# NickTravers/NeuralNetworkLibrary

Hardware: AMD Instinct MI355X
Metric: ResNet-34 224x224 training throughput (Learner.train1minibatch, fwd+loss+bwd+optimizer) (higher is better)
Workload: dtype f32; 1 GPU; DogsCats ResNet-34 classifier, 224x224, bs=64 per GPU, SGD momentum 0.9, fp32; global_batch=64, image_size=224, parallelism=dp1

## Files before the change

include/nnl.h:

```cpp
#ifndef NNL_H_
#define NNL_H_

#include <stddef.h>
#include <stdint.h>

#ifdef __cplusplus
extern "C" {
#endif

typedef enum {
  NNL_OK = 0,
  NNL_ERR_INVALID_ARG = -1,
  NNL_ERR_HIP = -2,
  NNL_ERR_UNSUPPORTED = -3,
  NNL_ERR_WORKSPACE = -4
} nnl_status_t;

int nnl_version(void);
const char* nnl_last_error(void);
int nnl_reload_env(void);

enum { NNL_PROF_CONV_FWD = 0, NNL_PROF_CONV_DGRAD = 1, NNL_PROF_CONV_WGRAD = 2, NNL_PROF_EMBDOT = 3,
       NNL_PROF_TABULAR = 4, NNL_PROF_RETINA_LOSS = 5, NNL_PROF_LSTM = 6, NNL_PROF_SOFTMAX_CE = 7,
       NNL_PROF_ELEMENTWISE = 8, NNL_PROF_GEMM = 9, NNL_PROF_OPTIM = 10, NNL_PROF_KINDS = 11 };
int nnl_prof_enable(int enable);
int nnl_prof_collect(int64_t* launches, double* total_ms, double* total_work);
int nnl_prof_collect2(int64_t* launches, double* total_ms, double* total_work, double* total_exec);
int nnl_dp_bump(int32_t* step, void* stream);
int nnl_dp_signal(int32_t* flag, const int32_t* step, void* stream);
int nnl_dp_wait(const int32_t* flag, int32_t value, int64_t timeout_us, int32_t* err, void* stream);
const char* nnl_source_stamp(void);

int nnl_embdotbias_fwd(const int64_t* x, const float* U, const float* M, const float* bu, const float* bi,
                       float* y, float* z, int64_t n, int64_t n_user, int64_t n_item, int64_t D,
                       int has_range, float lo, float hi, int32_t* err_flag, void* stream);
size_t nnl_embdotbias_bwd_workspace_bytes(int64_t n);
int nnl_embdotbias_bwd(const int64_t* x, const float* U, const float* M, const float* z, const float* dy,
                       float* dU, float* dM, float* dbu, float* dbi, int64_t n, int64_t n_user,
                       int64_t n_item, int64_t D, int has_range, float lo, float hi, void* workspace, size_t workspace_bytes, void* stream);

typedef struct {
  int32_t N, H, W, C;
  int32_t K, R, S;
  int32_t stride, pad;
  int32_t P, Q;
} nnl_conv_geom_t;

size_t nnl_conv2d_fwd_workspace_bytes(const nnl_conv_geom_t* g);
int64_t nnl_conv2d_tile_counters(void);
int nnl_conv2d_fwd(const float* x, const float* w, const float* bias, float* y, const nnl_conv_geom_t* g,
                   int relu, void* workspace, size_t workspace_bytes, int32_t* tile_counters, float* bn_partials,
                   const float* bn_pivot, int32_t* bn_rows, void* stream);
int nnl_conv2d_fwd_add_up2(const float* x, const float* w, const float* bias, const float* small, float* y,
                           const nnl_conv_geom_t* g, void* stream);
int nnl_upsample2_bwd(const float* dy, float* dsmall, int64_t N, int64_t h, int64_t w, int64_t C, void* stream);
int nnl_conv2d_weight_transpose(const float* w, float* wt, int K, int R, int S, int C, void* stream);
typedef struct {
  const float* w;
  float* wt;
  int32_t K, RS, C, first_tile;
} nnl_wt_desc_t;
int nnl_conv2d_weight_transpose_multi(const nnl_wt_desc_t* desc, const int32_t* tile_tensor, int64_t n_tiles,
                                      double total_elems, void* stream);
size_t nnl_conv2d_dgrad_workspace_bytes(const nnl_conv_geom_t* g);
int nnl_conv2d_dgrad(const float* dy, const float* wt, float* dx, const nnl_conv_geom_t* g, const float* addend,
                     void* workspace, size_t workspace_bytes, int32_t* tile_counters, void* stream);
typedef struct {
  const float* src;
  float* dst;
  int32_t rows, ch, flip, first_block;
  int32_t two_d, reserved;
} nnl_wino_desc_t;
int nnl_conv2d_wino_preferred(const nnl_conv_geom_t* g, int dgrad);
int nnl_wino_filter_multi(const nnl_wino_desc_t* desc, const int32_t* block_desc, int64_t n_blocks, void* stream);
int nnl_conv2d_fwd_pre(const float* x, const float* w, const float* bias, float* y, const nnl_conv_geom_t* g, int relu,
                       void* workspace, size_t workspace_bytes, int32_t* tile_counters, float* bn_partials, const float* bn_pivot,
                       int32_t* bn_rows, const float* u, void* stream);
int nnl_conv2d_dgrad_pre(const float* dy, const float* wt, float* dx, const nnl_conv_geom_t* g, const float* addend,
                         void* workspace, size_t workspace_bytes, int32_t* tile_counters, const float* u, void* stream);
size_t nnl_debug_conv_wino_workspace_bytes(int N, int H, int W, int C, int K);
int nnl_debug_conv_wino_fwd(const float* x, const float* filt, const float* bias, const float* add, float* y, void* ws,
                            size_t ws_bytes, int32_t* counters, long n_counters, float* bn_part, const float* bn_pivot, int N,
                            int H, int W, int C, int K, int relu, int flip, void* stream);
size_t nnl_debug_conv_wino2_workspace_bytes(int N, int H, int W, int C, int K);
int nnl_debug_conv_wino2_fwd(const float* x, const float* filt, const float* bias, const float* add, float* y, void* ws,
                            size_t ws_bytes, int32_t* counters, long n_counters, float* bn_part, const float* bn_pivot, int N,
                            int H, int W, int C, int K, int relu, int flip, void* stream);
int nnl_debug_conv_plan_times(int N, int H, int W, int C, int K, double* out);

int nnl_debug_route_record(int enable);
int nnl_debug_route_collect(char* out, size_t n);
size_t nnl_conv2d_wgrad_workspace_bytes(const nnl_conv_geom_t* g);
int nnl_conv2d_wgrad(const float* x, const float* dy, float* dw, const nnl_conv_geom_t* g, void* workspace,
                     size_t workspace_bytes, void* stream);
size_t nnl_colsum_workspace_bytes(int64_t rows, int64_t cols);
int nnl_sum_tensors(const float* const* src, int n, float* out, int64_t numel, void* stream);
int nnl_colsum(const float* a, float* out, int64_t rows, int64_t cols, void* workspace, size_t workspace_bytes,
               void* stream);
int nnl_relu_gate_colsum(const float* dy, const float* y, float* g, float* colsum, int64_t rows, int64_t cols, void* workspace,
                         size_t workspace_bytes, void* stream);
int nnl_act_gate_colsum(const float* dy, const float* y, float* g, float* colsum, int64_t rows, int64_t cols, int act,
                        void* workspace, size_t workspace_bytes, void* stream);

size_t nnl_bn_workspace_bytes(int64_t rows, int64_t C);
int nnl_bn_fwd(const float* x, const float* gamma, const float* beta, const float* residual, float* y,
               float* save_mean, float* save_invstd, float* running_mean, float* running_var, int64_t rows,
               int64_t C, float eps, float momentum, int training, int relu, int64_t* num_batches_tracked,
               uint32_t* relu_mask, const float* ext_partials, int64_t ext_rows, const float* ext_pivot, float* pivot_out,
               void* workspace, size_t workspace_bytes, void* stream);
int nnl_bn_bwd(const float* dy, const float* y, const uint32_t* relu_mask, const float* x, const float* gamma,
               const float* mean, const float* invstd, float* dx, float* dres, float* dgamma, float* dbeta, int64_t rows,
               int64_t C, int training, int relu, void* workspace, size_t workspace_bytes, void* stream);

int nnl_bn_relu_maxpool_supported(int64_t C);
int nnl_bn_relu_maxpool_fwd(const float* x, const float* gamma, const float* beta, float* y, uint8_t* idx, float* save_mean,
                            float* save_invstd, float* save_scale, float* save_shift, float* running_mean, float* running_var,
                            int64_t N, int64_t H, int64_t W, int64_t C, int64_t P, int64_t Q, int ks, int stride, int pad, float eps,
                            float momentum, int training, int64_t* num_batches_tracked, void* workspace, size_t workspace_bytes,
                            void* stream);
int nnl_bn_relu_maxpool_bwd(const float* dpool, const float* y, const uint8_t* idx, const float* x, const float* gamma,
                            const float* beta, const float* mean, const float* invstd, const float* scale, const float* shift,
                            float* dx, float* dgamma, float* dbeta,
                            int64_t N, int64_t H, int64_t W, int64_t C, int64_t P, int64_t Q, int ks, int stride, int pad,
                            int training, void* workspace, size_t workspace_bytes, void* stream);

int nnl_debug_bn_plan(int64_t rows, int64_t C, int64_t N, int64_t H, int64_t W, int64_t P, int64_t Q, int32_t* out10);

int nnl_bn_sync_stats(const float* x, float* stats, int64_t rows, int64_t C, void* workspace, size_t workspace_bytes,
                      void* stream);
int nnl_bn_sync_fwd(const float* x, const float* all_stats, int world, const float* gamma, const float* beta,
                    const float* residual, float* y, float* save_mean, float* save_invstd, float* running_mean,
                    float* running_var, int64_t rows, int64_t C, float eps, float momentum, int relu,
                    int64_t* num_batches_tracked, uint32_t* relu_mask, void* workspace, size_t workspace_bytes, void* stream);
int nnl_bn_sync_bwd_reduce(const float* dy, const float* y, const uint32_t* relu_mask, const float* x, const float* mean,
                           const float* invstd, float* sums, int64_t rows, int64_t C, int relu, void* workspace,
                           size_t workspace_bytes, void* stream);
int nnl_bn_sync_bwd(const float* dy, const float* y, const uint32_t* relu_mask, const float* x, const float* gamma,
                    const float* mean, const float* invstd, const float* local_sums, const float* global_sums,
                    const float* all_stats,
                    int world, float* dx, float* dres, float* dgamma, float* dbeta, int64_t rows, int64_t C, int relu,
                    void* workspace, size_t workspace_bytes, void* stream);

int nnl_maxpool2d_fwd(const float* x, float* y, uint8_t* idx, int64_t N, int64_t H, int64_t W, int64_t C, int64_t P,
                      int64_t Q, int ksize, int stride, int pad, void* stream);
int nnl_maxpool2d_bwd(const float* dy, const uint8_t* idx, float* dx, int64_t N, int64_t H, int64_t W, int64_t C,
                      int64_t P, int64_t Q, int ksize, int stride, int pad, void* stream);
int nnl_concat_pool_fwd(const float* x, float* out, int32_t* argmax, int64_t N, int64_t HW, int64_t C, void* stream);
int nnl_concat_pool_bwd(const float* dout, const int32_t* argmax, float* dx, int64_t N, int64_t HW, int64_t C, void* stream);

int nnl_gconv2d_fwd(const float* x, const float* w, const float* bias, float* y, int64_t N, int64_t H, int64_t W, int64_t C, int64_t K,
                    int64_t G, int R, int stride, int pad, int relu, void* stream);
int nnl_gconv2d_dgrad(const float* dy, const float* w, float* dx, int64_t N, int64_t H, int64_t W, int64_t C, int64_t K, int64_t G,
                      int R, int stride, int pad, void* stream);
size_t nnl_gconv2d_workspace_bytes(int64_t N, int64_t H, int64_t W, int64_t C, int64_t K, int64_t G, int R, int stride, int pad);
int nnl_gconv2d_wgrad(const float* x, const float* dy, float* dw, void* ws, size_t ws_bytes, int64_t N, int64_t H, int64_t W, int64_t C,
                      int64_t K, int64_t G, int R, int stride, int pad, void* stream);

int nnl_dwconv2d_fwd(const float* x, const float* w, const float* bias, float* y, int64_t N, int64_t H, int64_t W, int64_t C, int64_t P,
                     int64_t Q, int R, int stride, int pad_lo, int relu_in, void* stream);
int nnl_dwconv2d_dgrad(const float* dy, const float* w, const float* x, float* dx, int64_t N, int64_t H, int64_t W, int64_t C, int64_t P,
                       int64_t Q, int R, int stride, int pad_lo, int relu_in, void* stream);
size_t nnl_dwconv2d_wgrad_workspace_bytes(int64_t N, int64_t H, int64_t W, int64_t C, int64_t P, int64_t Q, int R, int stride, int pad_lo);
int nnl_dwconv2d_wgrad(const float* x, const float* dy, float* dw, void* ws, size_t ws_bytes, int64_t N, int64_t H, int64_t W, int64_t C,
                       int64_t P, int64_t Q, int R, int stride, int pad_lo, int relu_in, void* stream);

int nnl_avgpool2d_fwd(const float* x, float* y, int64_t N, int64_t H, int64_t W, int64_t C, int64_t P, int64_t Q, int ksize, int stride,
                      int pad_lo, int count_include_pad, void* stream);
int nnl_avgpool2d_bwd(const float* dy, float* dx, int64_t N, int64_t H, int64_t W, int64_t C, int64_t P, int64_t Q, int ksize, int stride,
                      int pad_lo, int count_include_pad, void* stream);
int nnl_subsample2d_fwd(const float* x, float* y, int64_t N, int64_t H, int64_t W, int64_t C, int64_t P, int64_t Q, int stride, int off,
                        void* stream);
int nnl_subsample2d_bwd(const float* dy, float* dx, int64_t N, int64_t H, int64_t W, int64_t C, int64_t P, int64_t Q, int stride, int off,
                        void* stream);

int nnl_se_squeeze(const float* x, float* m, int64_t N, int64_t HW, int64_t C, void* stream);
int nnl_se_excite_fwd(const float* x, const float* z, const float* residual, float* out, int64_t N, int64_t HW, int64_t C, void* stream);
int nnl_se_excite_bwd(const float* dy, const float* out, const float* x, const float* z, float* dx, float* dres, float* dz, int64_t N,
                      int64_t HW, int64_t C, void* stream);
int nnl_se_squeeze_bwd(const float* dm, float* dx, int64_t N, int64_t HW, int64_t C, void* stream);

int nnl_bbox_decode(const float* anchors, const float* reg, const float* clas, int64_t bs, int64_t A, int64_t K,
                    const float* mean4, const float* std4, float thresh, float width, float height, float* cand_boxes,
                    int32_t* cand_classes, float* cand_scores, int32_t* cand_order, int32_t* cand_count, void* stream);
int nnl_bbox_decode_window(const float* anchors, const float* reg, const float* clas, int64_t bs, int64_t A, int64_t K,
                           const float* mean4, const float* std4, float thresh, float x_min, float y_min, float x_max, float y_max,
                           float* cand_boxes, int32_t* cand_classes, float* cand_scores, int32_t* cand_order, int32_t* cand_count,
                           void* stream);
size_t nnl_nms_workspace_bytes(int64_t bs, int64_t top_k);
int nnl_nms(const float* cand_boxes, const int32_t* cand_classes, const float* cand_scores, const int32_t* cand_order,
            const int32_t* cand_count, int64_t bs, int64_t cap, int64_t top_k, float max_overlap, float* kept_boxes,
            int32_t* kept_classes, float* kept_scores, int32_t* kept_count, void* workspace, size_t workspace_bytes,
            void* stream);

typedef struct {
  float col_jit, row_jit;
  float inv;
  float cols;
  int32_t flip;
} nnl_tta_undo_t;
int nnl_tta_bbox_merge(const float* boxes, const int32_t* classes, const float* scores, const int32_t* counts,
                       const nnl_tta_undo_t* undo, int64_t L, int64_t P, int64_t M, float* cand_boxes, int32_t* cand_classes,
                       float* cand_scores, int32_t* cand_order, int32_t* cand_count, int32_t* err_flag, void* stream);

int nnl_tab_renorm(const int64_t* xcat, float* const* tables, const int32_t* card, const int32_t* dim,
                   const int32_t* row_off, const int32_t* row_table, int32_t* flags, int64_t bs, int32_t ncat,
                   int32_t total_rows, float max_norm, int32_t* err_flag, void* stream);
int nnl_tab_gather_fwd(const int64_t* xcat, const float* const* tables, const int32_t* card, const int32_t* dim,
                       const int32_t* col_off, const int32_t* col_table, const float* row_mask, const float* cont,
                       const float* cont_mask, float* out, int64_t bs, int32_t ncat, int32_t cat_width,
                       int32_t n_cont, int32_t ld_out, void* stream);
size_t nnl_tab_scatter_bwd_workspace_bytes(int64_t bs, int32_t ncat);
int nnl_tab_scatter_bwd(const int64_t* xcat, const int32_t* card, const int32_t* dim, const int32_t* col_off,
                        const int32_t* col_table, const int64_t* grad_off, const float* row_mask,
                        const float* cont_mask, const float* dout, float* dtab_flat, int64_t dtab_elems,
                        float* dcont, int64_t bs, int32_t ncat, int32_t cat_width, int32_t n_cont, int32_t ld_out,
                        void* workspace, size_t workspace_bytes, void* stream);
int nnl_tab_scan_bwd(const int64_t* xcat, const int32_t* card, const int32_t* dim, const int32_t* col_off,
                     const int64_t* grad_off, const float* row_mask, const float* cont_mask, const float* dout,
                     float* dtab_flat, float* dcont, const int32_t* blk_col, const int32_t* blk_first, int32_t n_scan_blocks,
                     int32_t max_dim, int64_t bs, int32_t ncat, int32_t cat_width, int32_t n_cont, int32_t ld_out, void* stream);

int nnl_pad_cols(const float* src, float* dst, int64_t rows, int64_t C, int64_t Cp, void* stream);
int nnl_keep_masks(const float* u, float* a, int64_t na, float keep_a, float* b, int64_t nb, float keep_b, void* stream);

int nnl_linear_small_supported(int64_t N);
int nnl_linear_small_fwd(const float* x, const float* w, const float* bias, float* y, int64_t M, int64_t K, int64_t ldx, int64_t N,
                         void* stream);
size_t nnl_linear_small_bwd_workspace_bytes(int64_t M, int64_t K, int64_t N);
int nnl_linear_small_bwd(const float* dy, const float* x, const float* w, float* dx, float* dw, float* db, int64_t M, int64_t K,
                         int64_t ldx, int64_t N, void* workspace, size_t workspace_bytes, void* stream);

size_t nnl_retina_loss_workspace_bytes(int64_t bs, int64_t A);
int nnl_retina_loss_fwd(const float* anchors, const float* reg, const float* clas, const float* boxes,
                        const int64_t* cats, int32_t* state, float* npos, float* out, int64_t bs, int64_t A,
                        int64_t K, int64_t M, float beta, float alpha, float gamma, void* workspace,
                        size_t workspace_bytes, void* stream);
int nnl_retina_loss_bwd(const float* anchors, const float* reg, const float* clas, const float* boxes,
                        const int64_t* cats, const int32_t* state, const float* npos, const float* grad_out,
                        float* dreg, float* dclas, int64_t bs, int64_t A, int64_t K, int64_t M, float beta,
                        float alpha, float gamma, void* stream);

int64_t nnl_lstm_padded_hidden(int64_t H);
int64_t nnl_lstm_padded_gates(int64_t H);
size_t nnl_lstm_workspace_bytes(int64_t T, int64_t B, int64_t H);
int nnl_lstm_fwd(const float* gx, const float* w_hh_pad, const float* h0, const float* c0, float* y, float* cy,
                 float* gates, int64_t T, int64_t B, int64_t H, void* workspace, size_t workspace_bytes, int32_t* err_flag,
                 void* stream);
int nnl_lstm_bwd(const float* dy, const float* dhT, const float* dcT, const float* gates, const float* cy,
                 const float* c0, const float* w_hh_t_pad, float* dgates_pad, float* dh0, float* dc0, int64_t T, int64_t B,
                 int64_t H, void* workspace, size_t workspace_bytes, int32_t* err_flag, void* stream);
int nnl_debug_lstm_bptt2_plan(int64_t B, int64_t H, int32_t* out5);
int nnl_debug_lstm_plan(int64_t B, int64_t H, int32_t* out14);

size_t nnl_mse_workspace_bytes(int64_t n);
int nnl_mse_fwd(const float* pred, const float* target, float* loss, int64_t n, void* workspace, size_t workspace_bytes, void* stream);
int nnl_mse_bwd(const float* pred, const float* target, const float* grad_out, float* dpred, int64_t n, void* stream);
size_t nnl_bce_logits_workspace_bytes(int64_t n);
int nnl_bce_logits_fwd(const float* logits, const float* target, float* loss, int64_t n, void* workspace, size_t workspace_bytes, void* stream);
int nnl_bce_logits_bwd(const float* logits, const float* target, const float* grad_out, float* dlogits, int64_t n, void* stream);
size_t nnl_fbeta_workspace_bytes(int64_t N, int64_t C);
int nnl_fbeta(const float* pred, const float* target, float* out, int64_t N, int64_t C, float beta2, float threshold, int use_thresh, float eps,
              void* workspace, size_t workspace_bytes, void* stream);
int nnl_scaled_sigmoid_fwd(const float* x, float* y, float* sig, int64_t n, float lo, float hi, void* stream);
int nnl_scaled_sigmoid_bwd(const float* dy, const float* sig, float* dx, int64_t n, float lo, float hi, void* stream);

int nnl_embedding_rowmask_fwd(const int64_t* x, const float* W, const float* rowmask, float* out, int64_t n,
                              int64_t V, int64_t D, int32_t* err_flag, void* stream);
size_t nnl_embedding_rowmask_bwd_workspace_bytes(int64_t n);
int nnl_embedding_rowmask_bwd(const int64_t* x, const float* rowmask, const float* dout, float* dW, int64_t n,
                              int64_t V, int64_t D, int64_t padding_idx, void* workspace, size_t workspace_bytes, void* stream);
int nnl_softmax_ce_fwd(const float* logits, const int64_t* target, float* row_stats, float* loss_rows, float* loss_mean,
                       int64_t rows, int64_t V, int32_t* err_flag, void* stream);
// ... 149 lines not shown
```

neuralnetworklibrary_amd/_lib.py:

```python
import ctypes as C
import os

import torch

_HERE = os.path.dirname(os.path.abspath(__file__))
LIB_PATH = os.environ.get('NNL_LIB_PATH') or os.path.join(_HERE, 'libnnl_hip.so')

if not os.path.exists(LIB_PATH):
    raise ImportError(
        f"{LIB_PATH} not found: build it with `python -c 'import __graft_entry__ as g; g.build()'` "
        "(or `make -C neuralnetworklibrary_amd/csrc`). There is no CPU fallback for the HIP hot path.")

lib = C.CDLL(LIB_PATH)

c_p = C.c_void_p
i32, i64, f32, f64 = C.c_int32, C.c_int64, C.c_float, C.c_double
sz = C.c_size_t


class ConvGeom(C.Structure):
    _fields_ = [('N', i32), ('H', i32), ('W', i32), ('C', i32), ('K', i32), ('R', i32), ('S', i32),
                ('stride', i32), ('pad', i32), ('P', i32), ('Q', i32)]


SIGNATURES = {
    'nnl_version': (C.c_int, []),
    'nnl_last_error': (C.c_char_p, []),
    'nnl_reload_env': (C.c_int, []),
    'nnl_prof_enable': (C.c_int, [C.c_int]),
    'nnl_prof_collect': (C.c_int, [C.POINTER(i64), C.POINTER(f64), C.POINTER(f64)]),
    'nnl_prof_collect2': (C.c_int, [C.POINTER(i64), C.POINTER(f64), C.POINTER(f64), C.POINTER(f64)]),
    'nnl_source_stamp': (C.c_char_p, []),
    'nnl_dp_bump': (C.c_int, [c_p, c_p]),
    'nnl_dp_signal': (C.c_int, [c_p, c_p, c_p]),
    'nnl_dp_wait': (C.c_int, [c_p, i32, i64, c_p, c_p]),
    'nnl_embdotbias_fwd': (C.c_int, [c_p, c_p, c_p, c_p, c_p, c_p, c_p, i64, i64, i64, i64, C.c_int, f32, f32,
                                     c_p, c_p]),
    'nnl_embdotbias_bwd_workspace_bytes': (sz, [i64]),
    'nnl_embdotbias_bwd': (C.c_int, [c_p, c_p, c_p, c_p, c_p, c_p, c_p, c_p, c_p, i64, i64, i64, i64, C.c_int,
                                     f32, f32, c_p, sz, c_p]),
    'nnl_conv2d_fwd_workspace_bytes': (sz, [C.POINTER(ConvGeom)]),
    'nnl_conv2d_dgrad_workspace_bytes': (sz, [C.POINTER(ConvGeom)]),
    'nnl_conv2d_tile_counters': (i64, []),
    'nnl_conv2d_wino_preferred': (C.c_int, [C.POINTER(ConvGeom), C.c_int]),
    'nnl_wino_filter_multi': (C.c_int, [c_p, c_p, i64, c_p]),
    'nnl_conv2d_fwd_pre': (C.c_int, [c_p, c_p, c_p, c_p, C.POINTER(ConvGeom), C.c_int, c_p, sz, c_p, c_p, c_p, C.POINTER(i32), c_p, c_p]),
    'nnl_conv2d_dgrad_pre': (C.c_int, [c_p, c_p, c_p, C.POINTER(ConvGeom), c_p, c_p, sz, c_p, c_p, c_p]),
    'nnl_debug_conv_wino_workspace_bytes': (sz, [C.c_int] * 5),
    'nnl_debug_conv_wino_fwd': (C.c_int, [c_p] * 6 + [sz, c_p, C.c_long, c_p, c_p] + [C.c_int] * 7 + [c_p]),
    'nnl_debug_conv_wino2_workspace_bytes': (sz, [C.c_int] * 5),
    'nnl_debug_conv_wino2_fwd': (C.c_int, [c_p] * 6 + [sz, c_p, C.c_long, c_p, c_p] + [C.c_int] * 7 + [c_p]),
    'nnl_debug_conv_plan_times': (C.c_int, [C.c_int] * 5 + [C.POINTER(C.c_double)]),
    'nnl_debug_route_record': (C.c_int, [C.c_int]),
    'nnl_debug_route_collect': (C.c_int, [C.c_char_p, sz]),
    'nnl_conv2d_fwd': (C.c_int, [c_p, c_p, c_p, c_p, C.POINTER(ConvGeom), C.c_int, c_p, sz, c_p, c_p, c_p, C.POINTER(i32), c_p]),
    'nnl_conv2d_weight_transpose': (C.c_int, [c_p, c_p, C.c_int, C.c_int, C.c_int, C.c_int, c_p]),
    'nnl_conv2d_weight_transpose_multi': (C.c_int, [c_p, c_p, i64, f64, c_p]),
    'nnl_conv2d_dgrad': (C.c_int, [c_p, c_p, c_p, C.POINTER(ConvGeom), c_p, c_p, sz, c_p, c_p]),
    'nnl_conv2d_wgrad_workspace_bytes': (sz, [C.POINTER(ConvGeom)]),
    'nnl_conv2d_wgrad': (C.c_int, [c_p, c_p, c_p, C.POINTER(ConvGeom), c_p, sz, c_p]),
    'nnl_colsum_workspace_bytes': (sz, [i64, i64]),
    'nnl_colsum': (C.c_int, [c_p, c_p, i64, i64, c_p, sz, c_p]),
    'nnl_relu_gate_colsum': (C.c_int, [c_p, c_p, c_p, c_p, i64, i64, c_p, sz, c_p]),
    'nnl_conv2d_fwd_add_up2': (C.c_int, [c_p, c_p, c_p, c_p, c_p, C.POINTER(ConvGeom), c_p]),
    'nnl_upsample2_bwd': (C.c_int, [c_p, c_p, i64, i64, i64, i64, c_p]),
    'nnl_act_gate_colsum': (C.c_int, [c_p, c_p, c_p, c_p, i64, i64, C.c_int, c_p, sz, c_p]),
    'nnl_maxpool2d_fwd': (C.c_int, [c_p, c_p, c_p, i64, i64, i64, i64, i64, i64, C.c_int, C.c_int, C.c_int, c_p]),
    'nnl_maxpool2d_bwd': (C.c_int, [c_p, c_p, c_p, i64, i64, i64, i64, i64, i64, C.c_int, C.c_int, C.c_int, c_p]),
    'nnl_sum_tensors': (C.c_int, [c_p, C.c_int, c_p, i64, c_p]),
    'nnl_bn_relu_maxpool_supported': (C.c_int, [i64]),
    'nnl_bn_relu_maxpool_fwd': (C.c_int, [c_p, c_p, c_p, c_p, c_p, c_p, c_p, c_p, c_p, c_p, c_p, i64, i64, i64, i64, i64, i64,
                                          C.c_int, C.c_int, C.c_int, f32, f32, C.c_int, c_p, c_p, sz, c_p]),
    'nnl_bn_relu_maxpool_bwd': (C.c_int, [c_p, c_p, c_p, c_p, c_p, c_p, c_p, c_p, c_p, c_p, c_p, c_p, c_p, i64, i64, i64, i64, i64, i64,
                                          C.c_int, C.c_int, C.c_int, C.c_int, c_p, sz, c_p]),
    'nnl_concat_pool_fwd': (C.c_int, [c_p, c_p, c_p, i64, i64, i64, c_p]),
    'nnl_concat_pool_bwd': (C.c_int, [c_p, c_p, c_p, i64, i64, i64, c_p]),
    'nnl_gconv2d_fwd': (C.c_int, [c_p, c_p, c_p, c_p, i64, i64, i64, i64, i64, i64, C.c_int, C.c_int, C.c_int, C.c_int, c_p]),
    'nnl_gconv2d_dgrad': (C.c_int, [c_p, c_p, c_p, i64, i64, i64, i64, i64, i64, C.c_int, C.c_int, C.c_int, c_p]),
    'nnl_gconv2d_workspace_bytes': (sz, [i64, i64, i64, i64, i64, i64, C.c_int, C.c_int, C.c_int]),
    'nnl_gconv2d_wgrad': (C.c_int, [c_p, c_p, c_p, c_p, sz, i64, i64, i64, i64, i64, i64, C.c_int, C.c_int, C.c_int, c_p]),
    'nnl_dwconv2d_fwd': (C.c_int, [c_p, c_p, c_p, c_p, i64, i64, i64, i64, i64, i64, C.c_int, C.c_int, C.c_int, C.c_int, c_p]),
    'nnl_dwconv2d_dgrad': (C.c_int, [c_p, c_p, c_p, c_p, i64, i64, i64, i64, i64, i64, C.c_int, C.c_int, C.c_int, C.c_int, c_p]),
    'nnl_dwconv2d_wgrad_workspace_bytes': (sz, [i64, i64, i64, i64, i64, i64, C.c_int, C.c_int, C.c_int]),
    'nnl_dwconv2d_wgrad': (C.c_int, [c_p, c_p, c_p, c_p, sz, i64, i64, i64, i64, i64, i64, C.c_int, C.c_int, C.c_int, C.c_int, c_p]),
    'nnl_avgpool2d_fwd': (C.c_int, [c_p, c_p, i64, i64, i64, i64, i64, i64, C.c_int, C.c_int, C.c_int, C.c_int, c_p]),
    'nnl_avgpool2d_bwd': (C.c_int, [c_p, c_p, i64, i64, i64, i64, i64, i64, C.c_int, C.c_int, C.c_int, C.c_int, c_p]),
    'nnl_subsample2d_fwd': (C.c_int, [c_p, c_p, i64, i64, i64, i64, i64, i64, C.c_int, C.c_int, c_p]),
    'nnl_subsample2d_bwd': (C.c_int, [c_p, c_p, i64, i64, i64, i64, i64, i64, C.c_int, C.c_int, c_p]),
    'nnl_se_squeeze': (C.c_int, [c_p, c_p, i64, i64, i64, c_p]),
    'nnl_se_excite_fwd': (C.c_int, [c_p, c_p, c_p, c_p, i64, i64, i64, c_p]),
    'nnl_se_excite_bwd': (C.c_int, [c_p, c_p, c_p, c_p, c_p, c_p, c_p, i64, i64, i64, c_p]),
    'nnl_se_squeeze_bwd': (C.c_int, [c_p, c_p, i64, i64, i64, c_p]),
    'nnl_bbox_decode': (C.c_int, [c_p, c_p, c_p, i64, i64, i64, c_p, c_p, f32, f32, f32, c_p, c_p, c_p, c_p, c_p, c_p]),
    'nnl_bbox_decode_window': (C.c_int, [c_p, c_p, c_p, i64, i64, i64, c_p, c_p, f32, f32, f32, f32, f32, c_p, c_p, c_p, c_p, c_p, c_p]),
    'nnl_nms_workspace_bytes': (sz, [i64, i64]),
    'nnl_nms': (C.c_int, [c_p, c_p, c_p, c_p, c_p, i64, i64, i64, f32, c_p, c_p, c_p, c_p, c_p, sz, c_p]),
    'nnl_tta_bbox_merge': (C.c_int, [c_p, c_p, c_p, c_p, c_p, i64, i64, i64, c_p, c_p, c_p, c_p, c_p, c_p, c_p]),
    'nnl_tab_renorm': (C.c_int, [c_p, c_p, c_p, c_p, c_p, c_p, c_p, i64, i32, i32, f32, c_p, c_p]),
    'nnl_tab_gather_fwd': (C.c_int, [c_p, c_p, c_p, c_p, c_p, c_p, c_p, c_p, c_p, c_p, i64, i32, i32, i32, i32, c_p]),
    'nnl_tab_scatter_bwd_workspace_bytes': (sz, [i64, i32]),
    'nnl_tab_scatter_bwd': (C.c_int, [c_p, c_p, c_p, c_p, c_p, c_p, c_p, c_p, c_p, c_p, i64, c_p, i64, i32, i32, i32, i32, c_p, sz, c_p]),
    'nnl_tab_scan_bwd': (C.c_int, [c_p] * 12 + [i32, i32, i64, i32, i32, i32, i32, c_p]),
    'nnl_pad_cols': (C.c_int, [c_p, c_p, i64, i64, i64, c_p]),
    'nnl_keep_masks': (C.c_int, [c_p, c_p, i64, f32, c_p, i64, f32, c_p]),
    'nnl_linear_small_supported': (C.c_int, [i64]),
    'nnl_linear_small_fwd': (C.c_int, [c_p, c_p, c_p, c_p, i64, i64, i64, i64, c_p]),
    'nnl_linear_small_bwd_workspace_bytes': (sz, [i64, i64, i64]),
    'nnl_linear_small_bwd': (C.c_int, [c_p, c_p, c_p, c_p, c_p, c_p, i64, i64, i64, i64, c_p, sz, c_p]),
    'nnl_retina_loss_workspace_bytes': (sz, [i64, i64]),
    'nnl_retina_loss_fwd': (C.c_int, [c_p, c_p, c_p, c_p, c_p, c_p, c_p, c_p, i64, i64, i64, i64, f32, f32, f32, c_p, sz, c_p]),
    'nnl_retina_loss_bwd': (C.c_int, [c_p, c_p, c_p, c_p, c_p, c_p, c_p, c_p, c_p, c_p, i64, i64, i64, i64, f32, f32, f32, c_p]),
    'nnl_lstm_padded_hidden': (i64, [i64]),
    'nnl_lstm_padded_gates': (i64, [i64]),
    'nnl_lstm_workspace_bytes': (sz, [i64, i64, i64]),
    'nnl_lstm_fwd': (C.c_int, [c_p, c_p, c_p, c_p, c_p, c_p, c_p, i64, i64, i64, c_p, sz, c_p, c_p]),
    'nnl_lstm_bwd': (C.c_int, [c_p, c_p, c_p, c_p, c_p, c_p, c_p, c_p, c_p, c_p, i64, i64, i64, c_p, sz, c_p, c_p]),
    'nnl_debug_lstm_bptt2_plan': (C.c_int, [i64, i64, c_p]),
    'nnl_debug_lstm_plan': (C.c_int, [i64, i64, C.POINTER(i32)]),
    'nnl_embedding_rowmask_fwd': (C.c_int, [c_p, c_p, c_p, c_p, i64, i64, i64, c_p, c_p]),
    'nnl_embedding_rowmask_bwd_workspace_bytes': (sz, [i64]),
    'nnl_embedding_rowmask_bwd': (C.c_int, [c_p, c_p, c_p, c_p, i64, i64, i64, i64, c_p, sz, c_p]),
    'nnl_softmax_ce_fwd': (C.c_int, [c_p, c_p, c_p, c_p, c_p, i64, i64, c_p, c_p]),
    'nnl_softmax_ce_bwd': (C.c_int, [c_p, c_p, c_p, c_p, c_p, i64, i64, i64, c_p]),
    'nnl_mse_workspace_bytes': (sz, [i64]),
    'nnl_mse_fwd': (C.c_int, [c_p, c_p, c_p, i64, c_p, sz, c_p]),
    'nnl_mse_bwd': (C.c_int, [c_p, c_p, c_p, c_p, i64, c_p]),
    'nnl_bce_logits_workspace_bytes': (sz, [i64]),
    'nnl_bce_logits_fwd': (C.c_int, [c_p, c_p, c_p, i64, c_p, sz, c_p]),
    'nnl_bce_logits_bwd': (C.c_int, [c_p, c_p, c_p, c_p, i64, c_p]),
    'nnl_fbeta_workspace_bytes': (sz, [i64, i64]),
    'nnl_fbeta': (C.c_int, [c_p, c_p, c_p, i64, i64, C.c_float, C.c_float, C.c_int, C.c_float, c_p, sz, c_p]),
    'nnl_scaled_sigmoid_fwd': (C.c_int, [c_p, c_p, c_p, i64, C.c_float, C.c_float, c_p]),
    'nnl_scaled_sigmoid_bwd': (C.c_int, [c_p, c_p, c_p, i64, C.c_float, C.c_float, c_p]),
    'nnl_seq_reg_workspace_bytes': (sz, [i64, i64]),
    'nnl_seq_reg_fwd': (C.c_int, [c_p, c_p, i64, i64, C.c_float, C.c_float, c_p, sz, c_p]),
    'nnl_seq_reg_bwd': (C.c_int, [c_p, c_p, c_p, i64, i64, C.c_float, C.c_float, c_p]),
    'nnl_weight_drop': (C.c_int, [c_p, i64, c_p, c_p, i64, i64, i64, C.c_uint64, C.c_float, c_p]),
    'nnl_lstm_cell_b1': (C.c_int, [c_p, i64, c_p, i64, c_p, c_p, c_p, i64, c_p, i64, i64, c_p, c_p, c_p, c_p, i64, i64, c_p]),
    'nnl_lm_next_token_workspace_bytes': (sz, [i64, i64]),
    'nnl_lm_next_token': (C.c_int, [c_p, i64, c_p, i64, i64, i64, i64, c_p, i64, c_p, i64, c_p, c_p, c_p, c_p, sz, c_p]),
    'nnl_attn_pool_workspace_bytes': (sz, [i64, i64, i64, i64]),
    'nnl_attn_pool_fwd': (C.c_int, [c_p, c_p, c_p, c_p, c_p, i64, c_p, c_p, i64, i64, i64, i64, c_p, sz, c_p, i64, c_p]),
    'nnl_attn_pool_bwd': (C.c_int, [c_p, c_p, c_p, c_p, c_p, c_p, c_p, c_p, c_p, c_p, i64, i64, i64, i64, c_p, sz, c_p, i64, c_p]),
    'nnl_image_aug_workspace_bytes': (sz, [i64, i64, i64]),
    'nnl_image_aug': (C.c_int, [c_p, i64, c_p, i64, c_p, i64, i64, i64, C.POINTER(f32), C.c_int, c_p, c_p, sz, c_p]),
    'nnl_detect_aug': (C.c_int, [c_p, i64, c_p, i64, c_p, c_p, c_p, i64, c_p, i64, i64, i64, i64, i64, i64, f64, C.POINTER(f32),
                                 c_p, c_p, c_p, c_p]),
    'nnl_image_stats': (C.c_int, [c_p, i64, c_p, i64, i64, i64, c_p, c_p]),
    'nnl_image_resize_u8': (C.c_int, [c_p, i64, c_p, c_p, i64, c_p, i64, c_p]),
    'nnl_optim_chunk_elems': (i64, []),
    'nnl_optim_patch': (C.c_int, [c_p, c_p, c_p, i64, c_p]),
    'nnl_optim_step': (C.c_int, [c_p, c_p, c_p, i64, C.c_int, c_p, C.c_int, c_p, c_p]),
    'nnl_bn_workspace_bytes': (sz, [i64, i64]),
    'nnl_bn_fwd': (C.c_int, [c_p, c_p, c_p, c_p, c_p, c_p, c_p, c_p, c_p, i64, i64, f32, f32, C.c_int, C.c_int, c_p, c_p, c_p, i64,
                             c_p, c_p, c_p, sz, c_p]),
    'nnl_debug_bn_plan': (C.c_int, [i64] * 7 + [C.POINTER(i32)]),
    'nnl_bn_sync_stats': (C.c_int, [c_p, c_p, i64, i64, c_p, sz, c_p]),
    'nnl_bn_sync_fwd': (C.c_int, [c_p, c_p, C.c_int, c_p, c_p, c_p, c_p, c_p, c_p, c_p, c_p, i64, i64, f32, f32, C.c_int, c_p,
                                  c_p, c_p, sz, c_p]),
    'nnl_bn_sync_bwd_reduce': (C.c_int, [c_p, c_p, c_p, c_p, c_p, c_p, c_p, i64, i64, C.c_int, c_p, sz, c_p]),
    'nnl_bn_sync_bwd': (C.c_int, [c_p, c_p, c_p, c_p, c_p, c_p, c_p, c_p, c_p, c_p, C.c_int, c_p, c_p, c_p, c_p, i64, i64,
                                  C.c_int, c_p, sz, c_p]),
    'nnl_bn_bwd': (C.c_int, [c_p, c_p, c_p, c_p, c_p, c_p, c_p, c_p, c_p, c_p, c_p, i64, i64, C.c_int, C.c_int, c_p, sz, c_p]),
    'nnl_seg_event_gaps': (C.c_int, [c_p, c_p, c_p, i64, f64, c_p, c_p, c_p, c_p, c_p]),
    'nnl_seg_rolling': (C.c_int, [c_p, c_p, c_p, c_p, i64, i64, i64, i64, C.c_int, C.c_int, c_p, c_p]),
    'nnl_assoc_contingency': (C.c_int, [c_p, c_p, i64, i64, c_p, c_p, c_p, i64, c_p, c_p]),
    'nnl_assoc_table_stats': (C.c_int, [c_p, c_p, i64, c_p, c_p, c_p, i64, c_p, c_p]),
    'nnl_assoc_cat_cont_workspace_bytes': (sz, [c_p, i64, c_p, i64]),
    'nnl_assoc_cat_cont': (C.c_int, [c_p, c_p, i64, c_p, c_p, i64, i64, c_p, c_p, i64, c_p, sz, c_p, c_p]),
    'nnl_assoc_cont_cont_workspace_bytes': (sz, [i64, i64]),
    'nnl_assoc_cont_cont': (C.c_int, [c_p, c_p, i64, i64, c_p, c_p, i64, C.c_int, c_p, sz, c_p, c_p]),
    'nnl_det_coco_match': (C.c_int, [c_p] * 7 + [i64, i64, i64, c_p, i64, c_p, i64, c_p, sz, c_p, c_p, c_p, c_p, c_p]),
    'nnl_det_coco_accumulate': (C.c_int, [c_p] * 8 + [i64, i64, i64, i64, i64, c_p, i64, c_p, i64, c_p, c_p, c_p, c_p]),
    'nnl_det_map_match': (C.c_int, [c_p, c_p, c_p, c_p, i64, i64, i64, c_p, i64, c_p, c_p]),
    'nnl_det_map_integrate_workspace_bytes': (sz, [i64, i64]),
    'nnl_det_map_integrate': (C.c_int, [c_p, c_p, c_p, c_p, c_p, i64, i64, i64, c_p, sz, c_p, c_p]),
    'nnl_text_token_count': (C.c_int, [c_p, i64, c_p, i64, C.c_int, c_p, c_p]),
    'nnl_text_token_fill': (C.c_int, [c_p, i64, c_p, i64, C.c_int, c_p, i64, c_p, c_p, c_p, c_p]),
    'nnl_text_token_hash': (C.c_int, [c_p, i64, c_p, c_p, i64, C.c_int, C.c_uint64, C.c_uint64, c_p, c_p]),
    'nnl_text_vocab_insert': (C.c_int, [c_p, i64, c_p, c_p, c_p, i64, C.c_int, c_p, c_p, c_p]),
    'nnl_text_vocab_verify': (C.c_int, [c_p, i64, c_p, c_p, c_p, i64, C.c_int, c_p, i64, c_p, c_p, i64, C.c_int, c_p, i64, c_p, c_p]),
    'nnl_text_vocab_compact': (C.c_int, [c_p, c_p, c_p, i64, c_p, c_p, i64, c_p, i64, c_p, c_p]),
    'nnl_text_vocab_assign': (C.c_int, [c_p, c_p, i64, c_p, i64, c_p]),
    'nnl_text_vocab_lookup': (C.c_int, [c_p, i64, c_p, c_p, c_p, i64, C.c_int, c_p, i64, c_p, c_p, i64, c_p, c_p, i64, c_p, c_p]),
    'nnl_text_ids_write': (C.c_int, [c_p, c_p, i64, c_p, i64, i64, C.c_int, c_p, c_p]),
}

for _name, (_res, _args) in SIGNATURES.items():
    try:
        _fn = getattr(lib, _name)
    except AttributeError as e:
        raise ImportError(f"libnnl_hip.so does not export {_name}; rebuild it") from e
    _fn.restype = _res
    _fn.argtypes = _args

PROF_KINDS = ['conv_fwd', 'conv_dgrad', 'conv_wgrad', 'embdot', 'tabular', 'retina_loss', 'lstm',
              'softmax_ce', 'elementwise', 'gemm', 'optim']


class NnlError(RuntimeError):
    pass


def check(status):
    if status != 0:
        raise NnlError(f"nnl error {status}: {lib.nnl_last_error().decode()}")


def ptr(t):
    return None if t is None else C.c_void_p(t.data_ptr())


def stream():
    return C.c_void_p(torch.cuda.current_stream().cuda_stream)


def require_cuda(*tensors):
    for t in tensors:
        if t is not None and not t.is_cuda:
            raise NnlError("nnl HIP op called with a non-CUDA tensor: the MI355X path has no CPU fallback")


def prof_enable(flag=True):
    check(lib.nnl_prof_enable(1 if flag else 0))

# ... 23 lines not shown
```

neuralnetworklibrary_amd/csrc/batchnorm.hip:

```cpp
#include "nnl_common.h"

namespace {

typedef float f32x4 __attribute__((ext_vector_type(4)));

template <int VEC> struct VecT;
template <> struct VecT<4> { typedef f32x4 type; };
template <> struct VecT<1> { typedef float type; };

template <int VEC> __device__ __forceinline__ float vget(const typename VecT<VEC>::type& v, int i);
template <> __device__ __forceinline__ float vget<4>(const f32x4& v, int i) { return v[i]; }
template <> __device__ __forceinline__ float vget<1>(const float& v, int i) { return v; }
template <int VEC> __device__ __forceinline__ void vset(typename VecT<VEC>::type& v, int i, float x);
template <> __device__ __forceinline__ void vset<4>(f32x4& v, int i, float x) { v[i] = x; }
template <> __device__ __forceinline__ void vset<1>(float& v, int i, float x) { v = x; }

constexpr int kBlock = 256;
constexpr int kMaxRowBlocks = 1024;
constexpr float kCentreAbove = 16.f;
constexpr int kFinLanes = 64;

struct Shape {
  int L;
  int rpb;
// ... 661 lines not shown
      const uchar4 id = reinterpret_cast<const uchar4*>(idx)[o];
      const f32x4 d = reinterpret_cast<const f32x4*>(dpool)[o];
      if (id.x == t) acc[0] += d[0];
      if (id.y == t) acc[1] += d[1];
      if (id.z == t) acc[2] += d[2];
      if (id.w == t) acc[3] += d[3];
    }
  }
  const f32x4 z = bnpool_affine(xv, sc, sh);
#pragma unroll
  for (int e = 0; e < 4; ++e) if (!(z[e] > 0.f)) acc[e] = 0.f;
  return acc;
}

constexpr int kPoolRedBlock = 1024;

__device__ __forceinline__ void store_pool_block_partials(const float (&s1)[4], const float (&s2)[4], float* __restrict__ part, int C,
                                                          int C4) {
  __shared__ float red[kPoolRedBlock][8];
#pragma unroll
  for (int e = 0; e < 4; ++e) { red[threadIdx.x][e * 2] = s1[e]; red[threadIdx.x][e * 2 + 1] = s2[e]; }
  __syncthreads();
  if ((int)threadIdx.x < C4) {
#pragma unroll
    for (int e = 0; e < 4; ++e) {
      float a = 0.f, b = 0.f;
      for (int j = threadIdx.x; j < kPoolRedBlock; j += C4) { a += red[j][e * 2]; b += red[j][e * 2 + 1]; }
      const long c = (long)threadIdx.x * 4 + e;
      part[((long)blockIdx.x * C + c) * 2 + 0] = a;
      part[((long)blockIdx.x * C + c) * 2 + 1] = b;
    }
  }
}

__global__ __launch_bounds__(kPoolRedBlock) void bnpool_bwd_reduce_kernel(const float* __restrict__ dpool, const uint8_t* __restrict__ idx,
                                                                   const float* __restrict__ x, const float* __restrict__ scale,
                                                                   const float* __restrict__ shift, const float* __restrict__ mean,
                                                                   const float* __restrict__ invstd, float* __restrict__ part,
                                                                   int N, int C, PoolGeom g) {
  const long total = (long)N * g.H * g.W * g.C4;
  const long i0 = (long)blockIdx.x * blockDim.x + threadIdx.x;
  const int c4 = (int)(i0 % g.C4);
  const f32x4 sc = reinterpret_cast<const f32x4*>(scale)[c4], sh = reinterpret_cast<const f32x4*>(shift)[c4];
  const f32x4 mu = reinterpret_cast<const f32x4*>(mean)[c4], is = reinterpret_cast<const f32x4*>(invstd)[c4];
  float s1[4] = {0.f, 0.f, 0.f, 0.f}, s2[4] = {0.f, 0.f, 0.f, 0.f};
  for (long i = i0; i < total; i += (long)gridDim.x * blockDim.x) {
    long r = i / g.C4;
    const int w = (int)(r % g.W); r /= g.W;
    const int h = (int)(r % g.H);
    const int n = (int)(r / g.H);
    const f32x4 xv = reinterpret_cast<const f32x4*>(x)[i];
    const f32x4 gg = bnpool_grad(dpool, idx, xv, sc, sh, n, h, w, c4, g);
#pragma unroll
    for (int e = 0; e < 4; ++e) { s1[e] += gg[e]; s2[e] += gg[e] * ((xv[e] - mu[e]) * is[e]); }
  }
  store_pool_block_partials(s1, s2, part, C, g.C4);
}

__global__ __launch_bounds__(kPoolRedBlock) void bnpool_bwd_reduce_out_kernel(const float* __restrict__ dpool, const float* __restrict__ y,
                                                                       const uint8_t* __restrict__ idx, const float* __restrict__ x,
                                                                       const float* __restrict__ gamma, const float* __restrict__ beta,
                                                                       const float* __restrict__ mean, const float* __restrict__ invstd,
                                                                       float* __restrict__ part, int N, int C, PoolGeom g) {
  const long total = (long)N * g.P * g.Q * g.C4;
  const long i0 = (long)blockIdx.x * blockDim.x + threadIdx.x;
  const int c4 = (int)(i0 % g.C4);
  float bt[4], rg[4], mu[4], is[4];
  bool fast[4];
#pragma unroll
  for (int e = 0; e < 4; ++e) {
    const int c = c4 * 4 + e;
    const float gm = gamma ? gamma[c] : 1.f;
    bt[e] = beta ? beta[c] : 0.f;
    fast[e] = fabsf(gm) > 1e-2f;
    rg[e] = fast[e] ? 1.f / gm : 0.f;
    mu[e] = mean[c]; is[e] = invstd[c];
  }
  float s1[4] = {0.f, 0.f, 0.f, 0.f}, s2[4] = {0.f, 0.f, 0.f, 0.f};
  for (long i = i0; i < total; i += (long)gridDim.x * blockDim.x) {
    const f32x4 d = reinterpret_cast<const f32x4*>(dpool)[i];
    const f32x4 yv = reinterpret_cast<const f32x4*>(y)[i];
    const uchar4 id = reinterpret_cast<const uchar4*>(idx)[i];
    const unsigned char t[4] = {id.x, id.y, id.z, id.w};
#pragma unroll
    for (int e = 0; e < 4; ++e) {
      if (!(yv[e] > 0.f)) continue;
      float xh;
      if (fast[e]) {
        xh = (yv[e] - bt[e]) * rg[e];
      } else {
        long r = i / g.C4;
        const int q = (int)(r % g.Q); r /= g.Q;
        const int p = (int)(r % g.P);
        const int n = (int)(r / g.P);
        const int h = p * g.stride - g.pad + t[e] / g.ks, w = q * g.stride - g.pad + t[e] % g.ks;
        xh = (x[((long)(n * g.H + h) * g.W + w) * C + c4 * 4 + e] - mu[e]) * is[e];
      }
      s1[e] += d[e];
      s2[e] += d[e] * xh;
    }
  }
  store_pool_block_partials(s1, s2, part, C, g.C4);
}

__global__ __launch_bounds__(kBlock) void bnpool_bwd_apply_kernel(const float* __restrict__ dpool, const uint8_t* __restrict__ idx,
                                                                  const float* __restrict__ x, const float* __restrict__ scale,
                                                                  const float* __restrict__ shift, const float* __restrict__ coef,
                                                                  float* __restrict__ dx, int N, int C, PoolGeom g) {
  const long total = (long)N * g.H * g.W * g.C4;
  const long i0 = (long)blockIdx.x * blockDim.x + threadIdx.x;
  const int c4 = (int)(i0 % g.C4);
  const f32x4 sc = reinterpret_cast<const f32x4*>(scale)[c4], sh = reinterpret_cast<const f32x4*>(shift)[c4];
  const f32x4 ca = reinterpret_cast<const f32x4*>(coef)[c4], cb = *reinterpret_cast<const f32x4*>(coef + C + c4 * 4),
              cc = *reinterpret_cast<const f32x4*>(coef + 2 * C + c4 * 4);
  for (long i = i0; i < total; i += (long)gridDim.x * blockDim.x) {
    long r = i / g.C4;
    const int w = (int)(r % g.W); r /= g.W;
    const int h = (int)(r % g.H);
    const int n = (int)(r / g.H);
    const f32x4 xv = reinterpret_cast<const f32x4*>(x)[i];
    const f32x4 gg = bnpool_grad(dpool, idx, xv, sc, sh, n, h, w, c4, g);
    f32x4 out;
#pragma unroll
    for (int e = 0; e < 4; ++e) out[e] = ca[e] * gg[e] + cb[e] * xv[e] + cc[e];
    reinterpret_cast<f32x4*>(dx)[i] = out;
  }
}

bool bnpool_ok(long C) { return C % 4 == 0 && C >= 4 && C <= 1024 && (kBlock % (C / 4)) == 0; }
unsigned bnpool_grid(long total) {
  long g = nnl_cdiv(total, (long)kPoolRedBlock * 4);
  if (g > kMaxRowBlocks) g = kMaxRowBlocks;
  return (unsigned)(g < 1 ? 1 : g);
}

int check_stem_geometry(const char* who, long N, long H, long W, long C, long P, long Q, int ks, int stride, int pad) {
  NNL_CHECK_ARG(N > 0 && H > 0 && W > 0 && P > 0 && Q > 0 && ks > 0 && ks * ks <= 255 && stride > 0 && pad >= 0 && 2 * pad <= ks,
                "%s: bad geometry", who);
  NNL_CHECK_ARG(P == (H + 2 * pad - ks) / stride + 1 && Q == (W + 2 * pad - ks) / stride + 1, "%s: P/Q do not match", who);
  NNL_CHECK_ARG(bnpool_ok(C), "%s: C=%ld needs C %% 4 == 0 and C/4 dividing 256", who, C);
  NNL_CHECK_ARG(N * H * W * C < (1L << 31) * 4, "%s: tensor too large", who);
  return NNL_OK;
}

}

extern "C" int nnl_bn_relu_maxpool_supported(int64_t C) { return bnpool_ok(C) ? 1 : 0; }

extern "C" int nnl_bn_relu_maxpool_fwd(const float* x, const float* gamma, const float* beta, float* y, uint8_t* idx,
                                       float* save_mean, float* save_invstd, float* save_scale, float* save_shift,
                                       float* running_mean, float* running_var, int64_t N, int64_t H, int64_t W, int64_t C,
                                       int64_t P, int64_t Q, int ks, int stride, int pad, float eps, float momentum, int training,
                                       int64_t* num_batches_tracked, void* workspace, size_t workspace_bytes, void* stream) {
  NNL_TRY(check_stem_geometry("bn_relu_maxpool_fwd", N, H, W, C, P, Q, ks, stride, pad));
  NNL_CHECK_ARG(x && y && idx && save_mean && save_invstd && save_scale && save_shift, "bn_relu_maxpool_fwd: null pointer");
  NNL_CHECK_ARG(training || (running_mean && running_var), "bn_relu_maxpool_fwd: eval mode needs running statistics");
  const long rows = (long)N * H * W, CG = C / 4;
  Workspace ws;
  NNL_TRY(bind_workspace(workspace, workspace_bytes, rows, C, "bn_relu_maxpool_fwd", ws));
  hipStream_t s = (hipStream_t)stream;
  NnlProfScope prof(NNL_PROF_ELEMENTWISE, s, (double)rows * C * (training ? 8.0 : 4.0) + (double)N * P * Q * C * 5.0);
  const ChannelStats cs{gamma, beta, save_mean, save_invstd, running_mean, running_var, save_scale, save_shift,  nullptr,
                         nullptr, num_batches_tracked, eps, momentum};
  NNL_TRY(launch_channel_affine(x, ws.part, cs, rows, C, training, s));
  const long total = (long)N * P * Q * CG;
  hipLaunchKernelGGL(bnpool_fwd_kernel, dim3((unsigned)nnl_cdiv(total, kBlock)), dim3(kBlock), 0, s, x, save_scale, save_shift, y, idx,
                     (int)N, (int)H, (int)W, (int)CG, (int)P, (int)Q, ks, stride, pad);
  NNL_CHECK_LAUNCH();
  return NNL_OK;
}

extern "C" int nnl_bn_relu_maxpool_bwd(const float* dpool, const float* y, const uint8_t* idx, const float* x, const float* gamma,
                                       const float* beta, const float* mean, const float* invstd, const float* scale,
                                       const float* shift, float* dx, float* dgamma, float* dbeta, int64_t N,
                                       int64_t H, int64_t W, int64_t C, int64_t P, int64_t Q, int ks, int stride, int pad,
                                       int training, void* workspace, size_t workspace_bytes, void* stream) {
  NNL_TRY(check_stem_geometry("bn_relu_maxpool_bwd", N, H, W, C, P, Q, ks, stride, pad));
  NNL_CHECK_ARG(dpool && idx && x && mean && invstd && scale && shift && dx, "bn_relu_maxpool_bwd: null pointer");
  const long rows = (long)N * H * W;
  Workspace ws;
  NNL_TRY(bind_workspace(workspace, workspace_bytes, rows, C, "bn_relu_maxpool_bwd", ws));
  hipStream_t s = (hipStream_t)stream;
  const PoolGeom g{(int)H, (int)W, (int)(C / 4), (int)P, (int)Q, ks, stride, pad};
  const long total = rows * (C / 4);
  NnlProfScope prof(NNL_PROF_ELEMENTWISE, s, (double)rows * C * 12.0 + (double)N * P * Q * C * 10.0);
  unsigned grid;
  if (y != nullptr) {
    grid = bnpool_grid((long)N * P * Q * (C / 4));
    hipLaunchKernelGGL(bnpool_bwd_reduce_out_kernel, dim3(grid), dim3(kPoolRedBlock), 0, s, dpool, y, idx, x, gamma, beta, mean, invstd,
                       ws.part, (int)N, (int)C, g);
  } else {
    grid = bnpool_grid(total);
    hipLaunchKernelGGL(bnpool_bwd_reduce_kernel, dim3(grid), dim3(kPoolRedBlock), 0, s, dpool, idx, x, scale, shift, mean, invstd, ws.part,
                       (int)N, (int)C, g);
  }
  NNL_CHECK_LAUNCH();
  NNL_TRY(launch_bwd_finalize(ws.part, (int)grid, gamma, mean, invstd, dgamma, dbeta, ws.coef, rows, C, training, s));
  hipLaunchKernelGGL(bnpool_bwd_apply_kernel, dim3((unsigned)nnl_cdiv(total, kBlock)), dim3(kBlock), 0, s, dpool, idx, x, scale, shift,
                     ws.coef, dx, (int)N, (int)C, g);
  NNL_CHECK_LAUNCH();
  return NNL_OK;
}

extern "C" int nnl_bn_sync_stats(const float* x, float* stats, int64_t rows, int64_t C, void* workspace,
                                 size_t workspace_bytes, void* stream) {
  NNL_CHECK_ARG(rows > 0 && C > 0 && C < (1 << 24) && x && stats, "bn_sync_stats: bad arguments");
  Workspace ws;
  NNL_TRY(bind_workspace(workspace, workspace_bytes, rows, C, "bn_sync_stats", ws));
  hipStream_t s = (hipStream_t)stream;
  NnlProfScope prof(NNL_PROF_ELEMENTWISE, s, (double)rows * C * 4.0);
  int nparts;
  NNL_TRY(launch_stats(x, ws.part, rows, C, s, nparts));
  hipLaunchKernelGGL(bn_sync_local_kernel, dim3((unsigned)nnl_cdiv(C, 4)), dim3(256), 0, s, x, (const float*)ws.part, nparts, stats,
                     (long)rows, (int)C);
  NNL_CHECK_LAUNCH();
  return NNL_OK;
}

extern "C" int nnl_bn_sync_fwd(const float* x, const float* all_stats, int world, const float* gamma, const float* beta,
                               const float* residual, float* y, float* save_mean, float* save_invstd, float* running_mean,
                               float* running_var, int64_t rows, int64_t C, float eps, float momentum, int relu,
                               int64_t* num_batches_tracked, uint32_t* relu_mask, void* workspace, size_t workspace_bytes,
                               void* stream) {
  NNL_CHECK_ARG(rows > 0 && C > 0 && C < (1 << 24) && world > 0, "bn_sync_fwd: bad sizes");
  NNL_CHECK_ARG(x && y && all_stats && save_mean && save_invstd, "bn_sync_fwd: null pointer");
  Workspace ws;
  NNL_TRY(bind_workspace(workspace, workspace_bytes, rows, C, "bn_sync_fwd", ws));
  hipStream_t s = (hipStream_t)stream;
  NnlProfScope prof(NNL_PROF_ELEMENTWISE, s, (double)rows * C * 8.0 + (residual ? 4.0 * rows * C : 0.0));
  hipLaunchKernelGGL(bn_sync_merge_kernel, dim3((unsigned)nnl_cdiv(C, 256)), dim3(256), 0, s, all_stats, world, gamma, beta,
                     save_mean, save_invstd, running_mean, running_var, ws.scale, ws.shift, (int)C, eps, momentum,
                     (long long*)num_batches_tracked, ws.apply_pivot);
  NNL_CHECK_LAUNCH();
  return launch_apply(x, ws, residual, y, rows, C, relu, relu_mask, s);
}

extern "C" int nnl_bn_sync_bwd_reduce(const float* dy, const float* y, const uint32_t* relu_mask, const float* x,
                                      const float* mean, const float* invstd, float* sums, int64_t rows, int64_t C, int relu,
                                      void* workspace, size_t workspace_bytes, void* stream) {
  NNL_CHECK_ARG(rows > 0 && C > 0 && C < (1 << 24), "bn_sync_bwd_reduce: bad sizes");
  NNL_CHECK_ARG(dy && x && mean && invstd && sums && (y || relu_mask || !relu), "bn_sync_bwd_reduce: null pointer");
  Workspace ws;
  NNL_TRY(bind_workspace(workspace, workspace_bytes, rows, C, "bn_sync_bwd_reduce", ws));
  hipStream_t s = (hipStream_t)stream;
  NnlProfScope prof(NNL_PROF_ELEMENTWISE, s, (double)rows * C * (relu ? 12.0 : 8.0));
  int nparts;
  NNL_TRY(launch_bwd_reduce(dy, y, relu_mask, x, mean, invstd, ws.part, rows, C, relu, s, nparts));
  hipLaunchKernelGGL(bn_sync_bwd_sums_kernel, dim3((unsigned)nnl_cdiv(C, 4)), dim3(256), 0, s, (const float*)ws.part, nparts, sums, (int)C);
  NNL_CHECK_LAUNCH();
  return NNL_OK;
}

extern "C" int nnl_bn_sync_bwd(const float* dy, const float* y, const uint32_t* relu_mask, const float* x, const float* gamma,
                               const float* mean,
                               const float* invstd, const float* local_sums, const float* global_sums, const float* all_stats,
                               int world, float* dx, float* dres, float* dgamma, float* dbeta, int64_t rows, int64_t C, int relu,
                               void* workspace, size_t workspace_bytes, void* stream) {
  NNL_CHECK_ARG(rows > 0 && C > 0 && C < (1 << 24) && world > 0, "bn_sync_bwd: bad sizes");
  NNL_CHECK_ARG(dy && x && mean && invstd && dx && local_sums && global_sums && all_stats && (y || relu_mask || !relu),
                "bn_sync_bwd: null pointer");
  Workspace ws;
  NNL_TRY(bind_workspace(workspace, workspace_bytes, rows, C, "bn_sync_bwd", ws));
  hipStream_t s = (hipStream_t)stream;
  NnlProfScope prof(NNL_PROF_ELEMENTWISE, s, (double)rows * C * (relu ? 16.0 : 12.0) + (dres ? 4.0 * rows * C : 0.0));
  hipLaunchKernelGGL(bn_sync_bwd_coef_kernel, dim3((unsigned)nnl_cdiv(C, 256)), dim3(256), 0, s, local_sums, global_sums, all_stats,
                     world, gamma, mean, invstd, dgamma, dbeta, ws.coef, (int)C);
  NNL_CHECK_LAUNCH();
  return launch_bwd_apply(dy, y, relu_mask, x, ws.coef, dx, dres, rows, C, relu, s);
}

extern "C" int nnl_debug_bn_plan(int64_t rows, int64_t C, int64_t N, int64_t H, int64_t W, int64_t P, int64_t Q, int32_t* out10) {
  if (rows <= 0 || C <= 0 || C >= (1 << 24) || out10 == nullptr) return 0;
  const int VEC = vec_of(C);
  const long CG = C / VEC;
  const Shape sh = make_shape(rows, CG);
  out10[0] = VEC; out10[1] = sh.L; out10[2] = sh.rpb; out10[3] = sh.gx; out10[4] = sh.gy; out10[5] = sh.capped ? 1 : 0;
  out10[6] = ew_grid(rows * CG, CG);
  out10[7] = kMaxRowBlocks;
  const bool stem = N > 0 && H > 0 && W > 0 && P > 0 && Q > 0 && bnpool_ok(C);
  out10[8] = stem ? (int32_t)bnpool_grid((long)N * H * W * (C / 4)) : -1;
  out10[9] = stem ? (int32_t)bnpool_grid((long)N * P * Q * (C / 4)) : -1;
  return 1;
}
```

neuralnetworklibrary_amd/csrc/conv2d.hip:

```cpp
#include "igemm_kernels.h"
#include "igemm_taps.h"
#include "split_plan.h"
#include "wino.h"
#include "igemm_wgrad.h"
#include "igemm_wgrad2d.h"

#ifdef NNL_TAPS_TIMING
static void* g_wgrad_dbg = nullptr;
extern "C" void* nnl_debug_wgrad_stamps(void) { return g_wgrad_dbg; }
#endif

namespace {

int check_geom(const nnl_conv_geom_t* g, const char* who) {
  if (!g) return nnl_set_error(NNL_ERR_INVALID_ARG, "%s: null geometry", who);
  if (g->N <= 0 || g->H <= 0 || g->W <= 0 || g->C <= 0 || g->K <= 0 || g->R <= 0 || g->S <= 0 || g->stride <= 0 ||
      g->pad < 0)
    return nnl_set_error(NNL_ERR_INVALID_ARG, "%s: non-positive dimension", who);
  if (g->H + 2L * g->pad < g->R || g->W + 2L * g->pad < g->S)
    return nnl_set_error(NNL_ERR_INVALID_ARG, "%s: the %d x %d filter is larger than the padded input (%d x %d, pad %d)", who, g->R, g->S,
                         g->H, g->W, g->pad);
  const int P = (g->H + 2 * g->pad - g->R) / g->stride + 1, Q = (g->W + 2 * g->pad - g->S) / g->stride + 1;
  if (P != g->P || Q != g->Q || P <= 0 || Q <= 0)
    return nnl_set_error(NNL_ERR_INVALID_ARG, "%s: P,Q=(%d,%d) do not match the geometry (%d,%d)", who, g->P, g->Q, P, Q);
// ... 453 lines not shown
    f32x4* dst = reinterpret_cast<f32x4*>(dw) + (k * 9 + r * 3) * C4 + c4;
    const f32x4 h = 0.5f * (u1 + u2);
    dst[0] = u0 + h;
    dst[C4] = 0.5f * (u1 - u2);
    dst[2L * C4] = h + u3;
  }
}

bool wgrad_wino_ok(const nnl_conv_geom_t* g) {
  const int mode = NNL_ENV_INT("NNL_WGRAD_WINO", 1);
  if (mode == 0) return false;
  if (g->R != 3 || g->S != 3 || g->stride != 1 || g->pad != 1 || g->Q % 2 != 0 || g->C % 64 != 0 || g->K % 4 != 0) return false;
  const long pairs = (long)g->N * g->P * (g->Q / 2);
  if (pairs < 1024 || !wgrad_v2_ok(2 * pairs * g->K, (long)g->N * g->H * g->W * g->C, pairs)) return false;
  if (mode == 2) return true;
  if (g->C == 64) return pairs >= 65536;
  return pairs >= 2048;
}

WgradPlan plan_wgrad_wino(const nnl_conv_geom_t* g) {
  return plan_wgrad(g->K, 12 * g->C, (long)g->N * g->P * (g->Q / 2), 3 * g->C);
}

int launch_wgrad_wino(const float* dy, const float* x, float* slabs, const nnl_conv_geom_t* g, const WgradPlan& pl, hipStream_t s) {
  IgemmWgradParams q{};
  const long pairs = (long)g->N * g->P * (g->Q / 2);
  q.a = dy; q.b = x; q.y = slabs;
  q.a_bytes = (unsigned)(2 * pairs * g->K * 4); q.b_bytes = (unsigned)((long)g->N * g->H * g->W * g->C * 4);
  q.H = g->H; q.W = g->W; q.C = g->C; q.P = g->P; q.Q = g->Q / 2; q.R = 3; q.S = 3; q.stride = 1; q.pad = 1;
  q.Mc = g->K; q.Nc = 12 * g->C; q.Kp = (int)pairs;
  q.splits = pl.splits; q.k_per_split = pl.k_per_split; q.grid_m = pl.grid_m; q.grid_n = pl.grid_n;
  q.n_fast = 1;
  if (pl.kg != 1 || (pl.bm == 64 && pl.k_per_split % 32 != 0))
    return nnl_set_error(NNL_ERR_UNSUPPORTED, "wgrad_wino1d: no kernel for the plan <%d> kg=%d k_per_split=%d", pl.bm, pl.kg, pl.k_per_split);
  const auto note = [&] { NNL_ROUTE("wgrad_wino1d<%d,%d,kg1>@splits=%d", pl.bm, pl.bm == 128 ? 16 : 32, pl.splits); };
  if (pl.bm == 128) return launch_wave_groups<igemm_wgrad_kernel<128, 128, 16, 2, 2, true, 1, true>>(q, 1, wgrad_lds_bytes(256, 16, 1), s, note);
  return launch_wave_groups<igemm_wgrad_kernel<64, 64, 32, 2, 2, true, 1, true>>(q, 1, wgrad_lds_bytes(128, 32, 1), s, note);
}

__global__ __launch_bounds__(256) void wino2d_wgrad_finish_kernel(const float* __restrict__ part, float* __restrict__ dw, long n_items, int C4,
                                                                   int splits, long slab4) {
  __shared__ f32x4 du[16][16];
  const int it = threadIdx.x >> 4, pos = threadIdx.x & 15;
  const long i = (long)blockIdx.x * 16 + it;
  const long c4 = i % C4, k = i / C4;
  f32x4 u = {0.f, 0.f, 0.f, 0.f};
  if (i < n_items) {
    const f32x4* src = reinterpret_cast<const f32x4*>(part) + (k * 16 + pos) * C4 + c4;
    for (int s0 = 0; s0 < splits; s0 += 8) {
      f32x4 v[8];
#pragma unroll
      for (int e = 0; e < 8; ++e) if (s0 + e < splits) v[e] = src[(long)(s0 + e) * slab4];
#pragma unroll
      for (int e = 0; e < 8; ++e) if (s0 + e < splits) u += v[e];
    }
  }
  du[it][pos] = u;
  __syncthreads();
  if (pos < 9 && i < n_items) {
    const int r = pos / 3, sx = pos - r * 3;
    const float gr[4] = {r == 0 ? 1.f : 0.f, 0.5f, r == 1 ? -0.5f : 0.5f, r == 2 ? 1.f : 0.f};
    const float gs[4] = {sx == 0 ? 1.f : 0.f, 0.5f, sx == 1 ? -0.5f : 0.5f, sx == 2 ? 1.f : 0.f};
    f32x4 acc = {0.f, 0.f, 0.f, 0.f};
#pragma unroll
    for (int a = 0; a < 4; ++a) {
      f32x4 row = {0.f, 0.f, 0.f, 0.f};
#pragma unroll
      for (int b = 0; b < 4; ++b) row += gs[b] * du[it][a * 4 + b];
      acc += gr[a] * row;
    }
    reinterpret_cast<f32x4*>(dw)[(k * 9 + pos) * C4 + c4] = acc;
  }
}

bool wgrad_wino2d_ok(const nnl_conv_geom_t* g) {
  const int mode = NNL_ENV_INT("NNL_WGRAD_WINO2D", 1);
  if (mode == 0 || NNL_ENV_INT("NNL_WGRAD_WINO", 1) == 0) return false;
  if (g->R != 3 || g->S != 3 || g->stride != 1 || g->pad != 1 || g->C % 64 != 0 || g->K % 4 != 0 || g->H < 2 || g->W < 2) return false;
  const long quads = (long)g->N * ((g->H + 1) / 2) * ((g->W + 1) / 2);
  if (quads < 512 || !wgrad_v2_ok((long)g->N * g->H * g->W * g->K, (long)g->N * g->H * g->W * g->C, quads)) return false;
  if (mode == 2) return true;
  return quads >= 1024;
}

WgradPlan plan_wgrad_wino2d(const nnl_conv_geom_t* g) {
  const long quads = (long)g->N * ((g->H + 1) / 2) * ((g->W + 1) / 2);
  WgradPlan pl = plan_wgrad(g->K, 16 * g->C, quads, g->C);
  auto with_tile = [&](int bt, int splits_target) {
    WgradPlan q{};
    q.bm = q.bn = bt; q.grid_m = (int)nnl_cdiv(g->K, bt); q.grid_n = (int)nnl_cdiv(16L * g->C, bt); q.kg = 1;
    const long tiles = (long)q.grid_m * q.grid_n;
    long sp = splits_target > 0 ? splits_target : (256L * 4 + tiles - 1) / tiles;
    const long max_sp = quads / 256 > 0 ? quads / 256 : 1;
    if (sp > max_sp) sp = max_sp;
    if (sp < 1) sp = 1;
    const long k1 = nnl_cdiv(nnl_cdiv(quads, sp), 32) * 32;
    q.k_per_split = (int)k1; q.splits = (int)nnl_cdiv(quads, k1);
    return q;
  };
  const bool big = g->K >= 128 && g->C % 128 == 0;
  if (big && (double)quads * g->K * g->C >= 500e6) return pl.bm == 128 ? pl : with_tile(128, 0);
  WgradPlan p64 = pl.bm == 64 ? pl : with_tile(64, 0);
  if (p64.splits >= 4) {
    const long sp = nnl_cdiv(p64.splits, 4);
    const long k1 = nnl_cdiv(nnl_cdiv(quads, sp), 128L) * 128L;
    if (k1 / 4 >= 700) {
      p64.kg = 4; p64.k_per_split = (int)k1; p64.splits = (int)nnl_cdiv(quads, k1);
      return p64;
    }
    return pl;
  }
  if (big) return pl.bm == 128 ? pl : with_tile(128, 0);
  return p64;
}

int launch_wgrad_wino2d(const float* dy, const float* x, float* slabs, const nnl_conv_geom_t* g, const WgradPlan& pl, hipStream_t s) {
  IgemmWgrad2dParams q{};
  q.a = dy; q.b = x; q.y = slabs;
  q.a_bytes = (unsigned)((long)g->N * g->H * g->W * g->K * 4); q.b_bytes = (unsigned)((long)g->N * g->H * g->W * g->C * 4);
  q.H = g->H; q.W = g->W; q.C = g->C; q.H2 = (g->H + 1) / 2; q.W2 = (g->W + 1) / 2;
  q.Mc = g->K; q.Nc = 16 * g->C; q.Kp = (int)((long)g->N * q.H2 * q.W2);
  q.splits = pl.splits; q.k_per_split = pl.k_per_split; q.grid_m = pl.grid_m; q.grid_n = pl.grid_n;
  q.n_fast = 1;
  if (!(pl.kg == 1 || (pl.kg == 4 && pl.bm == 64)) || (pl.bm == 64 && pl.k_per_split % 32 != 0))
    return nnl_set_error(NNL_ERR_UNSUPPORTED, "wgrad_wino2d: no kernel for the plan <%d> kg=%d k_per_split=%d", pl.bm, pl.kg, pl.k_per_split);
  const auto note = [&] { NNL_ROUTE("wgrad_wino2d<%d,%d,kg%d>@splits=%d", pl.bm, pl.bm == 128 ? 16 : 32, pl.kg, pl.splits); };
  if (pl.bm == 128) return launch_wave_groups<igemm_wgrad2d_kernel<128, 16, 1>>(q, 1, wgrad_lds_bytes(256, 16, 1), s, note);
  if (pl.kg == 4) return launch_wave_groups<igemm_wgrad2d_kernel<64, 32, 4>>(q, 4, wgrad_lds_bytes(128, 32, 4), s, note);
  return launch_wave_groups<igemm_wgrad2d_kernel<64, 32, 1>>(q, 1, wgrad_lds_bytes(128, 32, 1), s, note);
}

int launch_wgrad_direct(IgemmKmajorParams p, const WgradPlan& pl, float* ws, float* dw, hipStream_t s) {
  p.grid_m = pl.grid_m; p.grid_n = pl.grid_n; p.splits = pl.splits; p.k_per_split = pl.k_per_split;
  p.y = pl.splits > 1 ? ws : dw;
  const long a_elems = p.Kp * p.Mc, b_elems = (long)p.N * p.H * p.W * p.C;
  if (wgrad_v2_ok(a_elems, b_elems, p.Kp)) {
    const int st = launch_wgrad_v2(p, a_elems, b_elems, pl, s);
    if (st) return st;
  } else {
    const dim3 grid(pl.grid_m * pl.grid_n * pl.splits), block(256);
    NNL_ROUTE("wgrad_kmajor<%d,%d>%s@splits=%d", pl.bm, pl.bn, pl.splits > 1 ? ":splitk" : "", pl.splits);
    if (pl.bm == 128 && pl.bn == 128)
      hipLaunchKernelGGL((igemm_kmajor_kernel<128, 128, 16, 2, 2>), grid, block, 0, s, p);
    else if (pl.bm == 128)
      hipLaunchKernelGGL((igemm_kmajor_kernel<128, 64, 16, 2, 2>), grid, block, 0, s, p);
    else if (pl.bn == 128)
      hipLaunchKernelGGL((igemm_kmajor_kernel<64, 128, 16, 2, 2>), grid, block, 0, s, p);
    else
      hipLaunchKernelGGL((igemm_kmajor_kernel<64, 64, 16, 2, 2>), grid, block, 0, s, p);
    NNL_CHECK_LAUNCH();
  }
  if (pl.splits > 1) {
    const long n4 = (long)p.Mc * p.Nc / 4;
    NNL_ROUTE("splitk_reduce");
    hipLaunchKernelGGL(splitk_reduce_kernel, dim3((unsigned)nnl_cdiv(n4, 32)), dim3(256), 0, s, (const float*)ws, dw, n4, pl.splits);
    NNL_CHECK_LAUNCH();
  }
  return NNL_OK;
}

IgemmTapsParams fwd_taps_params(const nnl_conv_geom_t* g, const float* x, const float* w, float* y, const float* bias, int relu) {
  IgemmTapsParams q{};
  q.a = x; q.b = w; q.y = y; q.bias = bias; q.add = nullptr;
  q.a_bytes = (unsigned)((long)g->N * g->H * g->W * g->C * 4); q.b_bytes = (unsigned)((long)g->K * g->R * g->S * g->C * 4);
  q.H = g->H; q.W = g->W; q.C = g->C; q.P = g->P; q.Q = g->Q;
  q.in_stride = g->stride; q.ih0 = -g->pad; q.iw0 = -g->pad;
  q.OH = g->P; q.OW = g->Q; q.out_stride = 1; q.oh0 = 0; q.ow0 = 0;
  q.M = g->N * g->P * g->Q; q.Nc = g->K; q.b_row_stride = g->R * g->S * g->C; q.relu = relu;
  q.ntaps = g->R * g->S;
  for (int r = 0; r < g->R; ++r)
    for (int ss = 0; ss < g->S; ++ss) {
      const int t = r * g->S + ss;
      q.tap_dh[t] = (signed char)r; q.tap_dw[t] = (signed char)ss;
      q.tap_aoff[t] = (r * g->W + ss) * g->C; q.tap_woff[t] = t * g->C;
    }
  q.tap_affine = affine_taps_ok(g->S); q.tap_R = g->R; q.tap_S = g->S; q.tap_dh0 = 0; q.tap_dw0 = 0; q.tap_dstep = 1;
  return q;
}

IgemmTapsParams gemm_taps_params(const float* a, const float* b, float* y, int M, int N, int K) {
  IgemmTapsParams q{};
  q.a = a; q.b = b; q.y = y;
  q.a_bytes = (unsigned)((long)M * K * 4); q.b_bytes = (unsigned)((long)N * K * 4);
  q.H = 1; q.W = 1; q.C = K; q.P = 1; q.Q = 1; q.in_stride = 1; q.ih0 = 0; q.iw0 = 0;
  q.OH = 1; q.OW = 1; q.out_stride = 1; q.oh0 = 0; q.ow0 = 0;
  q.M = M; q.Nc = N; q.b_row_stride = K; q.ntaps = 1;
  q.tap_dh[0] = 0; q.tap_dw[0] = 0; q.tap_aoff[0] = 0; q.tap_woff[0] = 0;
  q.tap_affine = 1; q.tap_R = 1; q.tap_S = 1; q.tap_dstep = 1;
  return q;
}

}

int nnl_internal_gemm_nt(const float* a, const float* b, float* y, const float* bias, const float* add, int M, int N,
                         int K, int relu, hipStream_t s) {
  if (M <= 0 || N <= 0 || K <= 0 || K % 4 != 0) return nnl_set_error(NNL_ERR_INVALID_ARG, "gemm_nt: bad sizes");
  IgemmRowkParams p{};
  p.a = a; p.b = b; p.y = y; p.bias = bias; p.add = add;
  p.N = M; p.H = 1; p.W = 1; p.C = K; p.P = 1; p.Q = 1; p.R = 1; p.S = 1; p.stride = 1; p.pad = 0;
  p.M = M; p.Nc = N; p.Kg = K; p.relu = relu;
  if (taps_ok((long)M * K, (long)N * K, K, 1)) {
    IgemmTapsParams q = gemm_taps_params(a, b, y, M, N, K);
    q.bias = bias; q.add = add; q.relu = relu;
    return dispatch_taps(q, s);
  }
  return dispatch_rowk<IGEMM_MODE_FWD>(p, s);
}

int nnl_internal_gemm_nt_splitk(const float* a, const float* b, float* y_slabs, int M, int N, int K, int splits, hipStream_t s) {
  if (M <= 0 || N <= 0 || K <= 0 || K % 32 != 0 || splits < 1 || !taps_ok((long)M * K, (long)N * K, K, 1))
    return nnl_set_error(NNL_ERR_INVALID_ARG, "gemm_nt_splitk: bad sizes M=%d N=%d K=%d", M, N, K);
  IgemmTapsParams q = gemm_taps_params(a, b, y_slabs, M, N, K);
  q.ksplit = splits; q.slab_stride = (long)M * N;
  return launch_taps<64, 64, 32>(q, s);
}

int nnl_internal_lstm_step(IgemmTapsParams q, int epi, hipStream_t s) {
  if ((epi != 1 && epi != 2) || q.M <= 0 || q.C % 32 != 0 || q.lstm.H <= 0 || q.lstm.counters == nullptr)
    return nnl_set_error(NNL_ERR_INVALID_ARG, "lstm_step: bad arguments");
  q.grid_m = (int)nnl_cdiv(q.M, 64);
  q.grid_n = epi == 1 ? (int)nnl_cdiv(q.lstm.H, 16) : (int)nnl_cdiv(q.lstm.H, 64);
  q.bal = 0;
  const dim3 grid(q.grid_m * q.grid_n, q.ksplit > 1 ? q.ksplit : 1), block(256);
  if (epi == 1)
    hipLaunchKernelGGL((igemm_taps_kernel<64, 64, 32, 2, 2, 1>), grid, block, 0, s, q);
  else
    hipLaunchKernelGGL((igemm_taps_kernel<64, 64, 32, 2, 2, 2>), grid, block, 0, s, q);
  NNL_CHECK_LAUNCH();
  return NNL_OK;
}

size_t nnl_internal_gemm_tn_workspace_bytes(int Mc, int Nc, long Kp) {
  const WgradPlan pl = plan_wgrad(Mc, Nc, Kp);
  return pl.splits > 1 ? (size_t)pl.splits * Mc * Nc * sizeof(float) : 0;
}

int nnl_internal_gemm_tn(const float* a, const float* b, float* y, int Mc, int Nc, long Kp, void* ws, size_t ws_bytes,
                         hipStream_t s) {
  if (Mc <= 0 || Nc <= 0 || Kp <= 0 || Mc % 4 != 0 || Nc % 4 != 0) return nnl_set_error(NNL_ERR_INVALID_ARG, "gemm_tn: bad sizes");
  IgemmKmajorParams p{};
  p.a = a; p.b = b;
  p.N = (int)Kp; p.H = 1; p.W = 1; p.C = Nc; p.P = 1; p.Q = 1; p.R = 1; p.S = 1; p.stride = 1; p.pad = 0;
  p.Mc = Mc; p.Nc = Nc; p.Kp = Kp;
  const size_t need = nnl_internal_gemm_tn_workspace_bytes(Mc, Nc, Kp);
  if (need > 0 && (ws == nullptr || ws_bytes < need)) return nnl_set_error(NNL_ERR_WORKSPACE, "gemm_tn: workspace too small");
  return launch_wgrad_direct(p, plan_wgrad(Mc, Nc, Kp), (float*)ws, y, s);
}

static int wino_mode(int N, int H, int W, int Cin, int Nc, int R, int S, int stride, int pad) {
  if (!nnl_wino_ok(N, H, W, Cin, Nc, R, S, stride, pad)) return 0;
  const int e = NNL_ENV_INT("NNL_CONV_WINO", 1);
  const bool two_ok = nnl_wino2_ok(N, H, W, Cin, Nc, R, S, stride, pad);
  if (e >= 3) return two_ok ? 2 : 1;
  if (e == 2) return 1;
  const double t_d = plan_balance((long)N * H * W, Nc, Cin, 9).t_us + 6.0;
  const double t_w = nnl_wino_plan_time_us(N, H, W, Cin, Nc) + 6.0 + 3.0 + 21.0 * Cin * Nc * 4.0 / 4.0e6;
  const bool two_on = two_ok && NNL_ENV_INT("NNL_CONV_WINO2", 1) != 0;
  if (!(t_w < 0.97 * t_d)) {
    if (two_on && nnl_wino2_plan_is_pos(N, H, W, Cin, Nc) && nnl_wino2_plan_time_us(N, H, W, Cin, Nc) < 0.9 * t_d) return 2;
    return 0;
  }
  if (two_on && nnl_wino2_plan_time_us(N, H, W, Cin, Nc) < 0.9 * t_w) return 2;
  return 1;
}
static size_t wino_mode_workspace(int mode, int N, int H, int W, int Cin, int Nc) {
  return kWinoFamily[mode - 1].workspace_bytes(N, H, W, Cin, Nc);
}
static int wino_mode_launch(int mode, const WinoProblem& q, void* ws, size_t ws_bytes, int* counters, long n_counters, hipStream_t s) {
  nnl_prof_exec_frac(mode >= 2 ? 1.0 / 2.25 : 1.0 / 1.5);
  return kWinoFamily[mode - 1].launch(q, ws, ws_bytes, counters, n_counters, s);
}

extern "C" int nnl_debug_conv_plan_times(int N, int H, int W, int Cin, int Nc, double* out) {
  out[0] = plan_balance((long)N * H * W, Nc, Cin, 9).t_us;
  out[1] = nnl_wino_plan_time_us(N, H, W, Cin, Nc);
  out[2] = nnl_wino2_plan_time_us(N, H, W, Cin, Nc);
  out[3] = -1.0;
  return wino_mode(N, H, W, Cin, Nc, 3, 3, 1, 1);
}

extern "C" size_t nnl_conv2d_fwd_workspace_bytes(const nnl_conv_geom_t* g) {
  if (!g || check_geom(g, "conv2d_fwd_workspace_bytes")) return 0;
  const long a_elems = (long)g->N * g->H * g->W * g->C, b_elems = (long)g->K * g->R * g->S * g->C;
  const int tk = taps_kind(a_elems, b_elems, g->C, g->R * g->S);
  if (!tk) return 0;
  if (tk == 2) return balance_workspace_bytes((long)g->N * g->P * g->Q, g->K, (int)nnl_cdiv(g->C, 32) * 32, 1);
  size_t b = balance_workspace_bytes((long)g->N * g->P * g->Q, g->K, g->C, g->R * g->S);
  if (const int wm = wino_mode(g->N, g->H, g->W, g->C, g->K, g->R, g->S, g->stride, g->pad)) {
    const size_t wb = wino_mode_workspace(wm, g->N, g->H, g->W, g->C, g->K);
    if (wb > b) b = wb;
  }
  return b;
}

extern "C" size_t nnl_conv2d_dgrad_workspace_bytes(const nnl_conv_geom_t* g) {
  if (!g || check_geom(g, "conv2d_dgrad_workspace_bytes") || g->stride != 1) return 0;
  const long a_elems = (long)g->N * g->P * g->Q * g->K, b_elems = (long)g->C * g->R * g->S * g->K;
  const int tk = taps_kind(a_elems, b_elems, g->K, g->R * g->S);
  if (!tk) return 0;
  if (tk == 2) return balance_workspace_bytes((long)g->N * g->H * g->W, g->C, (int)nnl_cdiv(g->K, 32) * 32, 1);
  size_t b = balance_workspace_bytes((long)g->N * g->H * g->W, g->C, g->K, g->R * g->S);
  if (const int wm = wino_mode(g->N, g->P, g->Q, g->K, g->C, g->R, g->S, g->stride, g->pad)) {
    const size_t wb = wino_mode_workspace(wm, g->N, g->P, g->Q, g->K, g->C);
    if (wb > b) b = wb;
  }
  return b;
}

extern "C" int64_t nnl_conv2d_tile_counters(void) { return kTileCounters; }

extern "C" int nnl_conv2d_wino_preferred(const nnl_conv_geom_t* g, int dgrad) {
  if (!g) return 0;
  return dgrad ? wino_mode(g->N, g->P, g->Q, g->K, g->C, g->R, g->S, g->stride, g->pad)
               : wino_mode(g->N, g->H, g->W, g->C, g->K, g->R, g->S, g->stride, g->pad);
}

extern "C" int nnl_conv2d_fwd(const float* x, const float* w, const float* bias, float* y, const nnl_conv_geom_t* g,
                              int relu, void* workspace, size_t workspace_bytes, int32_t* tile_counters, float* bn_partials,
                              const float* bn_pivot, int32_t* bn_rows, void* stream) {
  return nnl_conv2d_fwd_pre(x, w, bias, y, g, relu, workspace, workspace_bytes, tile_counters, bn_partials, bn_pivot, bn_rows, nullptr, stream);
}

extern "C" int nnl_conv2d_fwd_pre(const float* x, const float* w, const float* bias, float* y, const nnl_conv_geom_t* g,
                                  int relu, void* workspace, size_t workspace_bytes, int32_t* tile_counters, float* bn_partials,
                                  const float* bn_pivot, int32_t* bn_rows, const float* u, void* stream) {
  if (bn_rows) *bn_rows = 0;
  int st = check_geom(g, "conv2d_fwd");
  if (st) return st;
  NNL_CHECK_ARG(x && w && y, "conv2d_fwd: null pointer");
  NNL_CHECK_ARG(relu >= 0 && relu <= 2, "conv2d_fwd: relu (activation) must be 0 none, 1 ReLU or 2 sigmoid");
  hipStream_t s = (hipStream_t)stream;
  IgemmRowkParams p{};
  p.a = x; p.b = w; p.y = y; p.bias = bias;
  p.N = g->N; p.H = g->H; p.W = g->W; p.C = g->C; p.P = g->P; p.Q = g->Q;
  p.R = g->R; p.S = g->S; p.stride = g->stride; p.pad = g->pad;
  p.M = g->N * g->P * g->Q; p.Nc = g->K; p.Kg = g->R * g->S * g->C; p.relu = relu;
  NnlProfScope prof(NNL_PROF_CONV_FWD, s, 2.0 * p.M * (double)p.Nc * p.Kg);
  const long a_elems = (long)g->N * g->H * g->W * g->C, b_elems = (long)g->K * g->R * g->S * g->C;
  const int wmode = (relu != 2 && workspace != nullptr) ? wino_mode(g->N, g->H, g->W, g->C, g->K, g->R, g->S, g->stride, g->pad) : 0;
  if (wmode && workspace_bytes >= wino_mode_workspace(wmode, g->N, g->H, g->W, g->C, g->K)) {
    WinoProblem wq{};
    wq.in = x; wq.filt = w; wq.out = y; wq.bias = bias; wq.add = nullptr;
    wq.N = g->N; wq.H = g->H; wq.W = g->W; wq.Cin = g->C; wq.Nc = g->K; wq.relu = relu; wq.flip = 0;
    const bool stats = bn_partials && bn_pivot && bn_rows;
// ... 307 lines not shown
```

neuralnetworklibrary_amd/csrc/igemm.h:

```cpp
#pragma once
#include "nnl_common.h"

typedef float f32x16 __attribute__((ext_vector_type(16)));
typedef float f32x4 __attribute__((ext_vector_type(4)));

struct IgemmRowkParams {
  const float* a;
  const float* b;
  float* y;
  const float* bias;
  const float* add;
  int N, H, W, C;
  int P, Q;
  int R, S, stride, pad;
  int M, Nc, Kg;
  int relu;
  int grid_m, grid_n;
};

struct IgemmKmajorParams {
  const float* a;
  const float* b;
  float* y;
  int N, H, W, C;
  int P, Q;
  int R, S, stride, pad;
  int Mc, Nc;
  long Kp;
  int splits, k_per_split;
  int grid_m, grid_n;
};

int nnl_internal_gemm_nt(const float* a, const float* b, float* y, const float* bias, const float* add, int M, int N,
                         int K, int relu, hipStream_t s);
int nnl_internal_gemm_nt_splitk(const float* a, const float* b, float* y_slabs, int M, int N, int K, int splits, hipStream_t s);
size_t nnl_internal_gemm_tn_workspace_bytes(int Mc, int Nc, long Kp);
int nnl_internal_gemm_tn(const float* a, const float* b, float* y, int Mc, int Nc, long Kp, void* ws, size_t ws_bytes,
                         hipStream_t s);

__device__ __forceinline__ int nnl_xcd_remap(int bid, int nblk) {
  const int q = nblk >> 3, r = nblk & 7;
  const int xcd = bid & 7, idx = bid >> 3;
  const int base = (xcd < r) ? xcd * (q + 1) : r * (q + 1) + (xcd - r) * q;
  return base + idx;
}
```

neuralnetworklibrary_amd/csrc/igemm_taps.h:

```cpp
#pragma once
#include "igemm.h"
#include "split_tile.h"

#define IGEMM_MAX_TAPS 49

struct LstmEpi {
  int H, Hp, Gp;
  int* counters;
  const float* gx;
  const float* c_prev;
  float* gates;
  float* c;
  float* h;
  float* hpad;
  const float* dy;
  float* dc;
  float* dgates;
};

struct IgemmTapsParams {
  const float* a; const float* b; float* y; const float* bias; const float* add;
  unsigned a_bytes, b_bytes;
  int H, W, C;
  int P, Q;
// ... 245 lines not shown
    if (nk > 0) {
      set_tap(t_nx);
      load_tile(c_nx);
      store_tile(0);
      if (nk > 1) advance();
      load_tile(c_nx);
    }
    __syncthreads();
    NNL_TSTAMP(1);
    int cur = 0, kt = 0;
    for (; kt + 1 < nk; kt += 2) {
      if (kt + 2 < nk) advance();
      load_tile2(c_nx);
      __builtin_amdgcn_sched_barrier(0);
      compute(cur);
      __builtin_amdgcn_sched_barrier(0);
      store_tile(cur ^ 1);
      __syncthreads();
      cur ^= 1;
      if (kt + 3 < nk) advance();
      load_tile(c_nx);
      __builtin_amdgcn_sched_barrier(0);
      compute(cur);
      __builtin_amdgcn_sched_barrier(0);
      store_tile2(cur ^ 1);
      __syncthreads();
      cur ^= 1;
    }
    if (kt < nk) {
      compute(cur);
      __syncthreads();
    }
  } else {
  if (nk > 0) {
    set_tap(t_nx);
    load_tile(c_nx);
    store_tile(0);
  }
  __syncthreads();
  NNL_TSTAMP(1);
  int cur = 0;
  for (int kt = 0; kt < nk; ++kt) {
    if (kt + 1 < nk) advance();
    load_tile(c_nx);
    __builtin_amdgcn_sched_barrier(0);
    compute(cur);
    __builtin_amdgcn_sched_barrier(0);
    store_tile(cur ^ 1);
    __syncthreads();
    cur ^= 1;
  }
  }

  NNL_TSTAMP(2);
  if constexpr (kTwoAcc) {
#pragma unroll
    for (int e = 0; e < 16; ++e) acc[0][0][e] += acc2[e];
  }
  if constexpr (EPI != 0) {
    constexpr int LDT = 68;
    float* tl = &lds[0][0];
    const int Nlog = p.grid_n * 64;
    const int cl = wn * 32 + (lane & 31);
    if (nslices > 1) {
      const __amdgpu_buffer_rsrc_t rs = __builtin_amdgcn_make_buffer_rsrc(p.y, 0, (int)((long)nslices * p.slab_stride * 4), 0x00020000);
#pragma unroll
      for (int e = 0; e < 16; ++e) {
        const int rl = wm * 32 + (e & 3) + 8 * (e >> 2) + (lane >> 5) * 4;
        const long off = (long)kslice * p.slab_stride + (long)(m0 + rl) * Nlog + n0 + cl;
        __builtin_amdgcn_raw_buffer_store_b32(__float_as_uint(acc[0][0][e]), rs, (m0 + rl < p.M) ? (int)(off * 4) : -1, 0, kSc1);
      }
      if (!split_tile_handover<false>(&p.lstm.counters[logical], nslices, tid)) return;
      for (int k4 = 0; k4 < 4; ++k4) {
        const int idx4 = tid + k4 * 256, rl = idx4 >> 4, c4 = (idx4 & 15) * 4;
        f32x4 v = {0.f, 0.f, 0.f, 0.f};
        if (m0 + rl < p.M) v = slab_sum4(rs, (long)(m0 + rl) * Nlog + n0 + c4, p.slab_stride, nslices);
        *reinterpret_cast<f32x4*>(tl + rl * LDT + c4) = v;
      }
    } else {
#pragma unroll
      for (int e = 0; e < 16; ++e) {
        const int rl = wm * 32 + (e & 3) + 8 * (e >> 2) + (lane >> 5) * 4;
        tl[rl * LDT + cl] = acc[0][0][e];
      }
    }
    __syncthreads();
    const LstmEpi& L = p.lstm;
    const int H = L.H;
    if constexpr (EPI == 1) {
      for (int idx = tid; idx < 64 * 16; idx += 256) {
        const int rl = idx >> 4, j = idx & 15;
        const int b = m0 + rl, u = tile_n * 16 + j;
        if (b >= p.M || u >= H) continue;
        const long g0 = (long)b * 4 * H + u, bu = (long)b * H + u;
        const float gi = nnl_sigmoid(L.gx[g0] + tl[rl * LDT + j]);
        const float gf = nnl_sigmoid(L.gx[g0 + H] + tl[rl * LDT + 16 + j]);
        const float gg = tanhf(L.gx[g0 + 2L * H] + tl[rl * LDT + 32 + j]);
        const float go = nnl_sigmoid(L.gx[g0 + 3L * H] + tl[rl * LDT + 48 + j]);
        const float cn = gf * L.c_prev[bu] + gi * gg;
        const float hn = go * tanhf(cn);
        L.gates[g0] = gi; L.gates[g0 + H] = gf; L.gates[g0 + 2L * H] = gg; L.gates[g0 + 3L * H] = go;
        L.c[bu] = cn;
        L.h[bu] = hn;
        L.hpad[(long)b * L.Hp + u] = hn;
      }
    } else {
      for (int idx = tid; idx < 64 * 64; idx += 256) {
        const int rl = idx >> 6, j = idx & 63;
        const int b = m0 + rl, u = n0 + j;
        if (b >= p.M || u >= H) continue;
        const long g0 = (long)b * 4 * H + u, bu = (long)b * H + u;
        const float gi = L.gates[g0], gf = L.gates[g0 + H], gg = L.gates[g0 + 2L * H], go = L.gates[g0 + 3L * H];
        const float dh = (L.dy ? L.dy[bu] : 0.f) + tl[rl * LDT + j];
        const float tc = tanhf(L.c[bu]);
        const float dcn = L.dc[bu] + dh * go * (1.f - tc * tc);
        float* dg = L.dgates + (long)b * L.Gp;
        dg[u] = dcn * gg * (gi * (1.f - gi));
        dg[H + u] = dcn * L.c_prev[bu] * (gf * (1.f - gf));
        dg[2 * H + u] = dcn * gi * (1.f - gg * gg);
        dg[3 * H + u] = dh * tc * (go * (1.f - go));
        L.dc[bu] = dcn * gf;
      }
    }
    return;
  }
  const int col_l = lane & 31, row_h = (lane >> 5) * 4;
  const bool dense_out = (p.out_stride == 1) && (p.OH == p.P) && (p.OW == p.Q) && (oh0 == 0) && (ow0 == 0);
  if (EPI == 0 && BM == 64 && BN == 64 && p.bal && partial && p.tile_counters != nullptr) {
    float* const base = in_tail ? p.tail_out : p.main_out;
    const long sstride = in_tail ? p.tail_slab_stride : p.main_slab_stride;
    const __amdgpu_buffer_rsrc_t rs = __builtin_amdgcn_make_buffer_rsrc(base, 0, (int)((long)nslices * sstride * 4), 0x00020000);
    const int cl = n0 + wn * 32 + col_l;
#pragma unroll
    for (int e = 0; e < 16; ++e) {
      const int row = m0 + wm * 32 + (e & 3) + 8 * (e >> 2) + row_h;
      const long off = (long)kslice * sstride + (long)(row - row0) * p.Nc + cl;
      __builtin_amdgcn_raw_buffer_store_b32(__float_as_uint(acc[0][0][e]), rs, (row < p.M && cl < p.Nc) ? (int)(off * 4) : -1, 0, kSc1);
    }
    if (!split_tile_handover<true>(&p.tile_counters[logical], nslices, tid)) return;
    float fs1[4] = {0.f, 0.f, 0.f, 0.f}, fs2[4] = {0.f, 0.f, 0.f, 0.f};
    for (int k4 = 0; k4 < 4; ++k4) {
      const int idx4 = tid + k4 * 256, rl = idx4 >> 4, c4 = n0 + (idx4 & 15) * 4;
      const int row = m0 + rl;
      if (row >= p.M || c4 >= p.Nc) continue;
      const f32x4 v = slab_sum4(rs, (long)(row - row0) * p.Nc + c4, sstride, nslices);
      const long o = (long)row * p.Nc + c4;
      finish_piece<true>(p, v, c4, o, fs1, fs2);
    }
    bn_partials_write(p, fs1, fs2, &lds[0][0], tid, tile_m, n0);
    return;
  }
  if constexpr (EPI == 0 && BM == 64 && BN == 64) {
    if (dense_out && !p.add_up2 && !partial && p.Nc % 4 == 0) {
      constexpr int LDT = 68;
      float* tl = &lds[0][0];
#pragma unroll
      for (int e = 0; e < 16; ++e) tl[(wm * 32 + (e & 3) + 8 * (e >> 2) + row_h) * LDT + wn * 32 + col_l] = acc[0][0][e];
      __syncthreads();
      float fs1[4] = {0.f, 0.f, 0.f, 0.f}, fs2[4] = {0.f, 0.f, 0.f, 0.f};
#pragma unroll
      for (int k4 = 0; k4 < 4; ++k4) {
        const int idx4 = tid + k4 * 256, rl = idx4 >> 4, c4 = n0 + (idx4 & 15) * 4;
        const int row = m0 + rl;
        if (row >= p.M || c4 >= p.Nc) continue;
        f32x4 v = *reinterpret_cast<const f32x4*>(tl + rl * LDT + (idx4 & 15) * 4);
        const long o = (long)row * p.Nc + c4;
        finish_piece<true>(p, v, c4, o, fs1, fs2);
      }
      bn_partials_write(p, fs1, fs2, &lds[0][0], tid, tile_m, n0);
      return;
    }
  }
#pragma unroll
  for (int j = 0; j < TN; ++j) {
    const int col = n0 + wn * WTN + j * 32 + col_l;
    const bool cok = col < p.Nc;
    const float bv = (p.bias != nullptr && cok && !partial) ? p.bias[col] : 0.f;
#pragma unroll
    for (int i = 0; i < TM; ++i) {
#pragma unroll
      for (int e = 0; e < 16; ++e) {
        const int row = m0 + wm * WTM + i * 32 + (e & 3) + 8 * (e >> 2) + row_h;
        if (cok && row < p.M) {
          long pix = row, apix = row;
          if (!dense_out || p.add_up2) {
            const int n = row / PQ;
            const int rem = row - n * PQ;
            const int pp = rem / p.Q;
            const int qq = rem - pp * p.Q;
            const int oh = pp * p.out_stride + oh0, ow = qq * p.out_stride + ow0;
            pix = ((long)n * p.OH + oh) * p.OW + ow;
            apix = p.add_up2 ? ((long)n * (p.OH >> 1) + (oh >> 1)) * (p.OW >> 1) + (ow >> 1) : pix;
          }
          float v = acc[i][j][e] + bv;
          if (!partial) {
            if (p.add) v += p.add[apix * p.Nc + col];
            if (p.relu == 1) v = fmaxf(v, 0.f);
            else if (p.relu == 2) v = nnl_sigmoid(v);
          }
          yout[(pix - row0) * p.Nc + col] = v;
        }
      }
    }
  }
  if (EPI == 0 && BM == 64 && BN == 64 && p.bn_part != nullptr && !partial) {
    const int col = n0 + wn * 32 + col_l;
    const bool cok = col < p.Nc;
    const float piv = cok ? p.bn_pivot[col] : 0.f, bv = (p.bias != nullptr && cok) ? p.bias[col] : 0.f;
    float s1 = 0.f, s2 = 0.f;
#pragma unroll
    for (int e = 0; e < 16; ++e) {
      const int row = m0 + wm * 32 + (e & 3) + 8 * (e >> 2) + row_h;
      if (row < p.M) {
        float v = acc[0][0][e] + bv;
        if (p.relu == 1) v = fmaxf(v, 0.f);
        else if (p.relu == 2) v = nnl_sigmoid(v);
        const float d = v - piv;
        s1 += d; s2 += d * d;
      }
    }
    s1 += __shfl_xor(s1, 32, 64);
    s2 += __shfl_xor(s2, 32, 64);
    float* red = &lds[0][0];
    if (lane < 32) { red[((wm * 64) + wn * 32 + lane) * 2] = s1; red[((wm * 64) + wn * 32 + lane) * 2 + 1] = s2; }
    __syncthreads();
    if (tid < 64 && n0 + tid < p.Nc) {
      p.bn_part[((long)tile_m * p.Nc + n0 + tid) * 2 + 0] = red[tid * 2] + red[(64 + tid) * 2];
      p.bn_part[((long)tile_m * p.Nc + n0 + tid) * 2 + 1] = red[tid * 2 + 1] + red[(64 + tid) * 2 + 1];
    }
  }
#ifdef NNL_TAPS_TIMING
  asm volatile("s_waitcnt vmcnt(0)" ::: "memory");
  NNL_TSTAMP(3);
#endif
}

int nnl_internal_lstm_step(IgemmTapsParams q, int epi, hipStream_t s);
```

neuralnetworklibrary_amd/csrc/split_tile.h:

```cpp
#pragma once
#include "igemm.h"

typedef int i32x4 __attribute__((ext_vector_type(4)));

constexpr int kSc1 = 1 << 4;

template <int POL>
__device__ __forceinline__ f32x4 buf_load4_policy(__amdgpu_buffer_rsrc_t rsrc, unsigned voff) {
  const i32x4 v = __builtin_bit_cast(i32x4, __builtin_amdgcn_raw_buffer_load_b128(rsrc, (int)voff, 0, POL));
  return __builtin_bit_cast(f32x4, v);
}
#define buf_load4_pol(rsrc, voff, pol) buf_load4_policy<pol>(rsrc, voff)


struct SplitTile {
  int logical, kslice, nslices, row0;
  bool in_tail;
};

template <class Params>
__device__ __forceinline__ SplitTile split_tile_decode(const Params& p) {
  SplitTile t{0, 0, 1, 0, false};
  if (p.bal) {
    const int nmb = p.n_main_tiles * p.main_ks;
    if ((int)blockIdx.x < nmb) {
      const int u = nnl_xcd_remap(blockIdx.x, nmb);
      t.logical = u / p.main_ks;
      t.kslice = u - t.logical * p.main_ks;
      t.nslices = p.main_ks;
    } else {
      const int tb = (int)blockIdx.x - nmb;
      const int tt = tb / p.tail_slices;
      t.kslice = tb - tt * p.tail_slices;
      t.logical = p.n_main_tiles + tt;
      t.nslices = p.tail_slices;
      if (t.nslices > 1) { t.row0 = p.tail_row0; t.in_tail = true; }
    }
  } else {
    t.logical = nnl_xcd_remap(blockIdx.x, gridDim.x);
  }
  return t;
}

template <bool RESET>
__device__ __forceinline__ bool split_tile_handover(int* counter, int nslices, int tid) {
  __shared__ int ticket;
  asm volatile("s_waitcnt vmcnt(0)" ::: "memory");
  __syncthreads();
  if (tid == 0) ticket = __hip_atomic_fetch_add(counter, 1, __ATOMIC_RELAXED, __HIP_MEMORY_SCOPE_AGENT);
  __syncthreads();
  if (ticket != nslices - 1) return false;
  if (RESET && tid == 0) __hip_atomic_store(counter, 0, __ATOMIC_RELAXED, __HIP_MEMORY_SCOPE_AGENT);
  return true;
}

__device__ __forceinline__ f32x4 slab_sum4(__amdgpu_buffer_rsrc_t rs, long off, long sstride, int nslices) {
  f32x4 v = {0.f, 0.f, 0.f, 0.f};
  for (int sl0 = 0; sl0 < nslices; sl0 += 8) {
    f32x4 part[8];
#pragma unroll
    for (int sl = 0; sl < 8; ++sl)
      if (sl0 + sl < nslices) part[sl] = buf_load4_pol(rs, (unsigned)(((long)(sl0 + sl) * sstride + off) * 4), kSc1);
#pragma unroll
    for (int sl = 0; sl < 8; ++sl)
      if (sl0 + sl < nslices) v += part[sl];
  }
  return v;
}

template <bool SIG>
__device__ __forceinline__ f32x4 finish4(f32x4 v, const float* bias, long boff, const float* add, long aoff, int relu) {
  if (bias) v += *reinterpret_cast<const f32x4*>(bias + boff);
  if (add) v += *reinterpret_cast<const f32x4*>(add + aoff);
  if (relu == 1) { v[0] = fmaxf(v[0], 0.f); v[1] = fmaxf(v[1], 0.f); v[2] = fmaxf(v[2], 0.f); v[3] = fmaxf(v[3], 0.f); }
  else if (SIG && relu == 2) { v[0] = nnl_sigmoid(v[0]); v[1] = nnl_sigmoid(v[1]); v[2] = nnl_sigmoid(v[2]); v[3] = nnl_sigmoid(v[3]); }
  return v;
}

template <bool SIG, class Params>
__device__ __forceinline__ void finish_piece(const Params& p, f32x4 v, int c4, long o, float (&fs1)[4], float (&fs2)[4]) {
  v = finish4<SIG>(v, p.bias, c4, p.add, o, p.relu);
  *reinterpret_cast<f32x4*>(p.y + o) = v;
  if (p.bn_part) {
    const f32x4 pv = *reinterpret_cast<const f32x4*>(p.bn_pivot + c4);
#pragma unroll
    for (int e = 0; e < 4; ++e) { const float d = v[e] - pv[e]; fs1[e] += d; fs2[e] += d * d; }
  }
}

template <class Params>
__device__ __forceinline__ void bn_partials_write(const Params& p, const float (&fs1)[4], const float (&fs2)[4], float* red, int tid,
                                                  int tile_m, int n0) {
  if (!p.bn_part) return;
  __syncthreads();
#pragma unroll
  for (int e = 0; e < 4; ++e) {
    red[(((tid >> 4) * 64) + (tid & 15) * 4 + e) * 2 + 0] = fs1[e];
    red[(((tid >> 4) * 64) + (tid & 15) * 4 + e) * 2 + 1] = fs2[e];
  }
  __syncthreads();
  if (tid < 64 && n0 + tid < p.Nc) {
    float a = 0.f, b = 0.f;
    for (int r = 0; r < 16; ++r) { a += red[(r * 64 + tid) * 2]; b += red[(r * 64 + tid) * 2 + 1]; }
    p.bn_part[((long)tile_m * p.Nc + n0 + tid) * 2 + 0] = a;
    p.bn_part[((long)tile_m * p.Nc + n0 + tid) * 2 + 1] = b;
  }
}
```

neuralnetworklibrary_amd/ops.py:

```python
import collections
import contextlib
import ctypes
import os
import weakref

import numpy as np
import torch

from . import _lib
from ._lib import check, lib, ptr, require_cuda, stream

__all__ = ['mse_loss', 'bce_with_logits', 'fbeta', 'scaled_sigmoid', 'embdotbias', 'index_error_flag', 'raise_if_index_error', 'conv2d', 'to_nhwc', 'from_nhwc', 'linear', 'bn_act', 'concat_pool2d', 'TabularPlan', 'tab_embed_concat', 'embedding_renorm_drop', 'retina_loss', 'image_aug', 'grouped_conv2d', 'se_excite']

_ERR_FLAGS = {}


def _flags(device):
    key = (device.type, device.index)
    if key not in _ERR_FLAGS:
        _ERR_FLAGS[key] = torch.zeros(2, dtype=torch.int32, device=device)
    return _ERR_FLAGS[key]


def index_error_flag(device):
# ... 314 lines not shown
        return u if u is not None and u.numel() == _wino_u_numel(rows, ch, mode) else None


_CLOSED = _Filters(torch.nn.Module())


def _filters(model):
    if getattr(model, '_nnl_filters', None) is None:
        object.__setattr__(model, '_nnl_filters', _Filters(model))
    return model._nnl_filters


def prepare_forward(model):
    _filters(model).prepare_forward()


def prepare_backward(model):
    _filters(model).prepare_backward()


def finish_backward():
    global _OPEN
    if _OPEN is not None:
        for views in (*_OPEN.u, _OPEN.wt, _OPEN.wt_padded):
            views.clear()
        _OPEN = None


def prepared_batches(model):
    return tuple(_filters(model).batches.values())


def prepared_filter_counts():
    f = _OPEN or _CLOSED
    return len(f.u[0]), len(f.u[1]), len(f.wt)


@contextlib.contextmanager
def filter_window(model):
    def backward(loss):
        prepare_backward(model)
        loss.backward()
    prepare_forward(model)
    try:
        yield backward
    finally:
        finish_backward()


_PADDED_GRADS = {}


def register_padded_grad(base, ld):
    if len(_PADDED_GRADS) > 64:
        for k in [k for k, (r, _) in _PADDED_GRADS.items() if r() is None]:
            del _PADDED_GRADS[k]
    _PADDED_GRADS[id(base)] = (weakref.ref(base), int(ld))


def _padded_rows(dy, K):
    base = dy._base if dy._is_view() else None
    ent = _PADDED_GRADS.get(id(base)) if base is not None else None
    if ent is None or ent[0]() is not base or dy.dim() != 4 or dy.shape[2] != 1 or dy.shape[3] != 1:
        return None
    ld = ent[1]
    if dy.dtype != torch.float32 or dy.stride(1) != 1 or dy.stride(0) != ld or ld < K or ld % 16 != 0 or dy.storage_offset() % ld != 0:
        return None
    if dy.storage_offset() + dy.shape[0] * ld > base.numel():
        return None
    return torch.as_strided(base, (dy.shape[0], 1, 1, ld), (ld, ld, ld, 1), dy.storage_offset())


_TILE_COUNTERS = {}


def _tile_counters(device):
    t = _TILE_COUNTERS.get(device.index)
    if t is None:
        if torch.cuda.is_current_stream_capturing():
            return None
        t = _TILE_COUNTERS[device.index] = torch.zeros(int(lib.nnl_conv2d_tile_counters()), dtype=torch.int32, device=device)
    return t


class GradSlot:
    __slots__ = ('tensor', 'closed')

    def __init__(self):
        self.tensor = None
        self.closed = False



_FAN = {}


class _FanOut(torch.autograd.Function):
    @staticmethod
    def forward(ctx, p, n):
        ctx.n = n
        return tuple(p.detach().view(p.shape) for _ in range(n))

    @staticmethod
    def backward(ctx, *grads):
        have = [g for g in grads if g is not None]
        if not have:
            return None, None
        if len(have) == 1:
            return have[0], None
        g0 = have[0]
        dense = all(g.is_cuda and g.dtype == torch.float32 and g.shape == g0.shape and g.stride() == g0.stride() and g.data_ptr() % 16 == 0
                    and (g.is_contiguous() or (g.dim() == 4 and g.is_contiguous(memory_format=torch.channels_last))) for g in have)
        if not dense or len(have) > 8:
            out = have[0]
            for g in have[1:]:
                out = out + g
            return out, None
        out = torch.empty_like(g0)
        arr = (ctypes.c_void_p * len(have))(*[g.data_ptr() for g in have])
        check(lib.nnl_sum_tensors(arr, len(have), ptr(out), g0.numel(), stream()))
        return out, None


class shared_params:

    def __init__(self, modules, n):
        self.modules, self.n, self.keys = modules, int(n), []

    def __enter__(self):
        if self.n > 1 and torch.is_grad_enabled():
            for m in self.modules:
                for p in m.parameters():
                    if p.requires_grad and p.is_cuda and id(p) not in _FAN:
                        _FAN[id(p)] = list(_FanOut.apply(p, self.n))
                        self.keys.append(id(p))
        return self

    def __exit__(self, *exc):
        for k in self.keys:
            _FAN.pop(k, None)
        return False


def fan_param(p):
    if p is None or not _FAN:
        return p
    lst = _FAN.get(id(p))
    return lst.pop(0) if lst else p


_ConvState = collections.namedtuple('_ConvState', 'g relu has_bias c_in w_layout slot give_slot grad_dst uses')


def _conv_operands(x, weight, bias, stride, pad):
    xn = _pad_c4(to_nhwc(_f32c(x) if x.dim() != 4 else x.float()))
    wn = _pad_c4(to_nhwc(weight.float()))
    N, H, W, C = xn.shape
    K, R, S, _ = wn.shape
    g = _geom(N, H, W, C, K, R, S, stride, pad)
    y = torch.empty((N, g.P, g.Q, K), dtype=torch.float32, device=x.device)
    return xn, wn, (None if bias is None else _f32c(bias)), g, y


def _conv_state(x, weight, bias, g, relu, slot=None, give_slot=None):
    uses = getattr(weight, '_nnl_uses', None)
    if uses is not None:
        uses[0] += 1
    return _ConvState(g, relu, bias is not None, x.shape[1], (tuple(weight.shape), tuple(weight.stride())), slot, give_slot,
                      getattr(weight, '_nnl_grad_dst', None), uses)


def _with_k(g, K):
    return _geom(g.N, g.H, g.W, g.C, K, g.R, g.S, g.stride, g.pad)


def _conv_backward(st, xn, wn, y, dy, needs):
    if dy is None:
        return None, None, None
    g, K = st.g, st.g.K
    want_db = st.has_bias and needs[2]
    db = None
    pre = _padded_rows(dy, K) if (not st.relu and g.R == 1 and g.S == 1 and g.H == 1 and g.W == 1) else None
    if pre is not None and pre.shape[-1] != K:
        dy4 = pre
    else:
        dy4 = to_nhwc(dy.float())
        if st.relu:
            dy4, db = _conv_act_gate(y, dy4, g, st.relu, want_db)
        if K % 4 != 0:
            dy4 = _pad_c4(dy4)
    w4, g4 = wn, g
    if dy4.shape[-1] != K:
        w4, g4 = torch.nn.functional.pad(wn, (0, 0, 0, 0, 0, 0, 0, dy4.shape[-1] - K)), _with_k(g, dy4.shape[-1])
    dx = dw = None
    if needs[0]:
        dx = _conv_dgrad(st, dy4, w4, g4, K)
    elif st.slot is not None:
        st.slot.tensor, st.slot.closed = None, True
    if needs[1]:
        dw = _conv_wgrad(st, xn, dy4, g4, K)
    if db is None and want_db:
        db = _conv_bias_grad(dy4, g4, K)
    return dx, dw, db


def _conv_act_gate(y, dyn, g, relu, want_db):
    rows = g.N * g.P * g.Q
    gated = torch.empty_like(dyn)
    cb = int(lib.nnl_colsum_workspace_bytes(rows, g.K)) if want_db else 0
    cws = _workspace(cb, dyn.device, floor=True) if want_db else None
    db = torch.empty(g.K, dtype=torch.float32, device=dyn.device) if want_db else None
    check(lib.nnl_act_gate_colsum(ptr(dyn), ptr(y), ptr(gated), ptr(db), rows, g.K, int(relu), ptr(cws), cb, stream()))
    return gated, db


def _conv_dgrad_operands(dy4, w4, g4, K):
    ktail = g4.R == 1 and g4.S == 1 and g4.K % 4 == 0
    dyd, gd, padk, wkey = dy4, g4, 0, None
    f = _OPEN or _CLOSED
    if g4.K % 16 != 0 and g4.K >= 32 and not ktail:
        padk = 16 - g4.K % 16
        dyd, gd = torch.nn.functional.pad(dy4, (0, padk)), _with_k(g4, g4.K + padk)
        wkey = (w4.data_ptr(), tuple(w4.shape), padk)
        wt = f.wt_padded.get(wkey) if f.wt else None
    else:
        wt = f.wt.get(w4.data_ptr()) if g4.K == K else None
        if wt is not None and tuple(wt.shape) != (g4.C, g4.R, g4.S, g4.K):
            wt = None
    if wt is None:
        wd = torch.nn.functional.pad(w4, (0, 0, 0, 0, 0, 0, 0, padk)) if padk else w4
        wt = torch.empty((gd.C, gd.R, gd.S, gd.K), dtype=torch.float32, device=dy4.device)
        check(lib.nnl_conv2d_weight_transpose(ptr(wd), ptr(wt), gd.K, gd.R, gd.S, gd.C, stream()))
        if wkey is not None and f.wt:
            f.wt_padded[wkey] = wt
    return dyd, wt, gd


def _conv_dgrad(st, dy4, w4, g4, K):
    dyd, wt, g = _conv_dgrad_operands(dy4, w4, g4, K)
    dxn = torch.empty((g.N, g.H, g.W, g.C), dtype=torch.float32, device=dyd.device)
    wsb = int(lib.nnl_conv2d_dgrad_workspace_bytes(g))
    dws = _workspace(wsb, dyd.device)
    shortcut = None
    if st.slot is not None:
        shortcut, st.slot.tensor, st.slot.closed = st.slot.tensor, None, True
    fuse = shortcut is not None and g.K % 16 == 0 and g.R * g.S <= 49 and shortcut.numel() == dxn.numel() \
        and ((g.stride == 1 and (g.S <= 32 or g.pad <= 127)) or (g.stride == 2 and g.R == 3 and g.S == 3 and g.pad == 1))
    u = (_OPEN or _CLOSED).wino(w4.data_ptr() if g.K == K else 0, 1, g)
    check(lib.nnl_conv2d_dgrad_pre(ptr(dyd), ptr(wt), ptr(dxn), g, ptr(shortcut) if fuse else None, ptr(dws), wsb,
                                   ptr(_tile_counters(dyd.device) if wsb else None), ptr(u), stream()))
    if shortcut is not None and not fuse:
        dxn += shortcut.view_as(dxn)
    give = st.give_slot
    if give is not None and not give.closed and st.c_in == g.C:
        give.tensor = dxn
        return None
    return from_nhwc(dxn[..., :st.c_in] if st.c_in != g.C else dxn)


def _conv_wgrad(st, xn, dy4, g4, K):
    dst = st.grad_dst
    if dst is not None and st.uses is not None and st.uses[0] == 1 and dst.dim() == 4 and g4.K == K and st.c_in == g4.C \
            and dst.permute(0, 2, 3, 1).is_contiguous() and tuple(dst.shape) == (g4.K, g4.C, g4.R, g4.S):
        dwn = dst.permute(0, 2, 3, 1)
    else:
        dwn = torch.empty((g4.K, g4.R, g4.S, g4.C), dtype=torch.float32, device=dy4.device)
    wsb = int(lib.nnl_conv2d_wgrad_workspace_bytes(g4))
    ws = _workspace(wsb, dy4.device, floor=True)
    check(lib.nnl_conv2d_wgrad(ptr(xn), ptr(dy4), ptr(dwn), g4, ptr(ws), wsb, stream()))
    dw = from_nhwc(dwn[:K, :, :, :st.c_in])
    wshape, wstride = st.w_layout
    if (g4.R == 1 and g4.S == 1 and wshape == tuple(dw.shape) and wstride != tuple(dw.stride()) and dw.is_contiguous(memory_format=torch.channels_last)
            and wstride[1] == 1 and wstride[0] == dw.shape[1]):
        dw = dw.as_strided(wshape, wstride)
    return dw


def _conv_bias_grad(dy4, g4, K):
    rows = g4.N * g4.P * g4.Q
    db_full = torch.empty(g4.K, dtype=torch.float32, device=dy4.device)
    cb = int(lib.nnl_colsum_workspace_bytes(rows, g4.K))
    cws = _workspace(cb, dy4.device, floor=True)
    check(lib.nnl_colsum(ptr(dy4), ptr(db_full), rows, g4.K, ptr(cws), cb, stream()))
    return db_full[:K]


class _Conv2d(torch.autograd.Function):

    @staticmethod
    def forward(ctx, x, weight, bias, stride, pad, relu, slot=None, bn_pivot=None, give_slot=None):
        require_cuda(x, weight, bias)
        xn, wn, b, g, y = _conv_operands(x, weight, bias, stride, pad)
        N, K = g.N, g.K
        ctx.st = _conv_state(x, weight, bias, g, relu, slot, give_slot)
        wsb = int(lib.nnl_conv2d_fwd_workspace_bytes(g))
        ws = _workspace(wsb, x.device)
        part, rows = None, _lib.i32(0)
        if bn_pivot is not None:
            part = torch.empty(((N * g.P * g.Q + 63) // 64) * K * 2, dtype=torch.float32, device=x.device)
        u = (_OPEN or _CLOSED).wino(wn.data_ptr(), 0, g)
        check(lib.nnl_conv2d_fwd_pre(ptr(xn), ptr(wn), ptr(b), ptr(y), g, int(relu), ptr(ws), wsb, ptr(_tile_counters(x.device) if wsb else None),
                                     ptr(part), ptr(bn_pivot), ctypes.byref(rows) if part is not None else None, ptr(u), stream()))
        if part is None or rows.value == 0:
            part = torch.empty(0, dtype=torch.float32, device=x.device)
        else:
            part = part[:rows.value * K * 2]
        ctx.mark_non_differentiable(part)
        ctx.set_materialize_grads(False)
        ctx.save_for_backward(xn, wn, y if relu else None)
        return from_nhwc(y), part

    @staticmethod
    def backward(ctx, dy, _dpart=None):
        xn, wn, y = ctx.saved_tensors
        return _conv_backward(ctx.st, xn, wn, y, dy, ctx.needs_input_grad[:3]) + (None,) * 6


def _conv(x, weight, bias, *, stride=1, pad=0, relu=0, slot=None, bn_pivot=None, give_slot=None):
    return _Conv2d.apply(x, weight, bias, int(stride), int(pad), int(relu), slot, bn_pivot, give_slot)


def conv2d(x, weight, bias=None, stride=1, pad=0, relu=False, grad_slot=None, give_slot=None):
    return _conv(x, weight, bias, stride=stride, pad=pad, relu=relu, slot=grad_slot, give_slot=give_slot)[0]


class _ConvAddUp2(torch.autograd.Function):

    @staticmethod
    def forward(ctx, x, weight, bias, small, stride, pad):
        require_cuda(x, weight, bias, small)
        xn, wn, b, g, y = _conv_operands(x, weight, bias, stride, pad)
        sn = to_nhwc(small.float())
        ctx.small_shape = (g.N, g.P // 2, g.Q // 2, g.K)
        if tuple(sn.shape) != ctx.small_shape or g.P % 2 or g.Q % 2:
            raise _lib.NnlError('conv_add_upsampled: `small` %s is not [N, K, P/2, Q/2] of the %dx%d output' % (tuple(small.shape), g.P, g.Q))
        ctx.st = _conv_state(x, weight, bias, g, 0)
        check(lib.nnl_conv2d_fwd_add_up2(ptr(xn), ptr(wn), ptr(b), ptr(sn), ptr(y), g, stream()))
        ctx.save_for_backward(xn, wn)
        return from_nhwc(y)

    @staticmethod
    def backward(ctx, dy):
        dsmall = None
        if ctx.needs_input_grad[3]:
            dyn = to_nhwc(dy.float())
            N, h, w, K = ctx.small_shape
            ds = torch.empty(ctx.small_shape, dtype=torch.float32, device=dy.device)
            check(lib.nnl_upsample2_bwd(ptr(dyn), ptr(ds), N, h, w, K, stream()))
            dsmall = from_nhwc(ds)
        xn, wn = ctx.saved_tensors
        return _conv_backward(ctx.st, xn, wn, None, dy, ctx.needs_input_grad[:3]) + (dsmall, None, None)


def conv_add_upsampled(x, weight, bias, small, stride=1, pad=0):
    return _ConvAddUp2.apply(x, weight, bias, small, int(stride), int(pad))


def conv2d_with_bn_stats(x, weight, bias, stride, pad, bn_pivot, grad_slot=None, give_slot=None):
    return _conv(x, weight, bias, stride=stride, pad=pad, slot=grad_slot, bn_pivot=bn_pivot, give_slot=give_slot)


def _rows_in_place(x):
    return x.dtype == torch.float32 and x.dim() == 2 and x.stride(1) == 1 and x.stride(0) >= x.shape[1]


class _LinearSmall(torch.autograd.Function):

    @staticmethod
    def forward(ctx, x, weight, bias):
        require_cuda(x, weight, bias)
        x = x if _rows_in_place(x) else _f32c(x)
        w = _f32c(weight)
        b = None if bias is None else _f32c(bias)
        M, K = x.shape
        N = w.shape[0]
        y = torch.empty(M, N, dtype=torch.float32, device=x.device)
        check(lib.nnl_linear_small_fwd(ptr(x), ptr(w), ptr(b), ptr(y), M, K, x.stride(0) if M > 1 else K, N, stream()))
        ctx.save_for_backward(x, w)
        ctx.has_bias = bias is not None
        return y

    @staticmethod
    def backward(ctx, dy):
        x, w = ctx.saved_tensors
        M, K = x.shape
        N = w.shape[0]
        dy = _f32c(dy)
        dev = dy.device
        dx = torch.empty(M, K, dtype=torch.float32, device=dev) if ctx.needs_input_grad[0] else None
        dw = torch.empty(N, K, dtype=torch.float32, device=dev) if ctx.needs_input_grad[1] else None
        db = torch.empty(N, dtype=torch.float32, device=dev) if (ctx.has_bias and ctx.needs_input_grad[2]) else None
        wsb = int(lib.nnl_linear_small_bwd_workspace_bytes(M, K, N)) if (dw is not None or db is not None) else 0
        ws = _workspace(wsb, dev)
        check(lib.nnl_linear_small_bwd(ptr(dy), ptr(x), ptr(w), ptr(dx), ptr(dw), ptr(db), M, K, x.stride(0) if M > 1 else K, N, ptr(ws), wsb,
                                       stream()))
        return dx, dw, db


def linear(x, weight, bias=None, relu=False):
    lead = x.shape[:-1]
    x2 = x.reshape(-1, x.shape[-1])
    if not relu and weight.shape[0] <= 4 and x2.is_cuda and x2.shape[0] > 0:
        return _LinearSmall.apply(x2, weight, bias).reshape(*lead, weight.shape[0])
    y = _conv(x2[:, :, None, None], weight[:, :, None, None], bias, relu=relu)[0]
    return y.reshape(*lead, weight.shape[0])


def _rows_view(x):
    if x.dim() == 4:
        xn = to_nhwc(x.float())
        N, H, W, C = xn.shape
        return xn.view(-1, C), (lambda m: from_nhwc(m.view(N, H, W, C)))
    if x.dim() == 2:
        return _f32c(x), (lambda m: m)
    if x.dim() == 3:
        xn = x.float().permute(0, 2, 1).contiguous()
        N, L, C = xn.shape
        return xn.view(-1, C), (lambda m: m.view(N, L, C).permute(0, 2, 1))
    raise ValueError('bn_act: unsupported input rank %d' % x.dim())


def _relu_mask(rows, C, device):
    return torch.empty((rows * C + 31) // 32 + 2, dtype=torch.int32, device=device)


def _bn_grad_buffers(ctx, xm, gamma, has_res):
    dx = torch.empty_like(xm)
    dres = torch.empty_like(xm) if (has_res and ctx.needs_input_grad[1]) else None
    dgamma = torch.empty(xm.shape[1], dtype=torch.float32, device=xm.device) if gamma is not None else None
    dbeta = torch.empty(xm.shape[1], dtype=torch.float32, device=xm.device) if gamma is not None else None
    return dx, dres, dgamma, dbeta


def _bn_grads(ctx, back, dx, dres, dgamma, dbeta):
    if ctx.slot is not None and dres is not None:
        ctx.slot.tensor, dres = dres, None
    return back(dx), None if dres is None else back(dres), dgamma, dbeta


class _BNAct(torch.autograd.Function):
    @staticmethod
    def forward(ctx, x, residual, gamma, beta, running_mean, running_var, training, momentum, eps, relu, nbt, slot=None, ext=None,
                pivot_out=None):
        require_cuda(x, residual, gamma, beta)
        ctx.slot = slot
        xm, back = _rows_view(x)
        rows, C = xm.shape
        rm = None if residual is None else _rows_view(residual)[0]
        y = torch.empty_like(xm)
        mean = torch.empty(C, dtype=torch.float32, device=xm.device)
        invstd = torch.empty(C, dtype=torch.float32, device=xm.device)
        wsb = int(lib.nnl_bn_workspace_bytes(rows, C))
        ws = _workspace(wsb, xm.device)
        mask = _relu_mask(rows, C, xm.device) if relu else None
        check(lib.nnl_bn_fwd(ptr(xm), ptr(gamma), ptr(beta), ptr(rm), ptr(y), ptr(mean), ptr(invstd), ptr(running_mean),
# ... 52 lines not shown
        dym = _rows_view(dy)[0]
        rows, C = xm.shape
        dev = xm.device
        wsb = int(lib.nnl_bn_workspace_bytes(rows, C))
        ws = _workspace(wsb, dev)
        sums = torch.empty(2 * C, dtype=torch.float32, device=dev)
        check(lib.nnl_bn_sync_bwd_reduce(ptr(dym), None, ptr(mask), ptr(xm), ptr(mean), ptr(invstd), ptr(sums), rows, C, int(relu),
                                         ptr(ws), wsb, stream()))
        total = comm.all_reduce_sum(sums, group)
        dx, dres, dgamma, dbeta = _bn_grad_buffers(ctx, xm, gamma, has_res)
        check(lib.nnl_bn_sync_bwd(ptr(dym), None, ptr(mask), ptr(xm), ptr(gamma), ptr(mean), ptr(invstd), ptr(sums), ptr(total),
                                  ptr(all_stats), int(all_stats.shape[0]), ptr(dx), ptr(dres), ptr(dgamma), ptr(dbeta), rows, C,
                                  int(relu), ptr(ws), wsb, stream()))
        return _bn_grads(ctx, back, dx, dres, dgamma, dbeta) + (None,) * 9


class DistComm:

    @staticmethod
    def all_gather(t, group):
        import torch.distributed as dist
        w = dist.get_world_size(group)
        out = torch.empty((w,) + tuple(t.shape), dtype=t.dtype, device=t.device)
        dist.all_gather(list(out.unbind(0)), t, group=group)
        return out

    @staticmethod
    def all_reduce_sum(t, group):
        import torch.distributed as dist
        out = t.clone()
        dist.all_reduce(out, op=dist.ReduceOp.SUM, group=group)
        return out


def _bn_mode(bn):
    training = bn.training or (bn.running_mean is None)
    momentum, nbt = 0.0, None
    if bn.training and bn.track_running_stats:
        nbt, momentum = bn.num_batches_tracked, bn.momentum
    stats = not training or bn.track_running_stats
    return training, momentum, nbt, (bn.running_mean if stats else None), (bn.running_var if stats else None)


def bn_act(bn, x, residual=None, relu=True, grad_slot=None, ext_stats=None, pivot_out=None):
    training, momentum, nbt, rmean, rvar = _bn_mode(bn)
    if momentum is None:
        nbt.add_(1)
        momentum, nbt = 1.0 / float(nbt.item()), None
    sync = getattr(bn, 'nnl_sync', None)
    if sync is not None and training:
        return _SyncBNAct.apply(x, residual, bn.weight, bn.bias, rmean, rvar, momentum, bn.eps, relu, nbt, sync[0], sync[1],
                                grad_slot)
    ext = ext_stats if (ext_stats is not None and training and ext_stats[0].numel() > 0) else None
    return _BNAct.apply(x, residual, bn.weight, bn.bias, rmean, rvar, training, momentum, bn.eps, relu, nbt, grad_slot, ext,
                        pivot_out if training else None)


class _ConcatPool(torch.autograd.Function):
    @staticmethod
    def forward(ctx, x):
        require_cuda(x)
        xn = to_nhwc(x.float())
        N, H, W, C = xn.shape
        out = torch.empty(N, 2 * C, dtype=torch.float32, device=x.device)
        am = torch.empty(N, C, dtype=torch.int32, device=x.device)
        check(lib.nnl_concat_pool_fwd(ptr(xn), ptr(out), ptr(am), N, H * W, C, stream()))
        ctx.save_for_backward(am)
        ctx.shape = (N, H, W, C)
        return out.view(N, 2 * C, 1, 1)

    @staticmethod
    def backward(ctx, dout):
        (am,) = ctx.saved_tensors
        N, H, W, C = ctx.shape
        dx = torch.empty(N, H, W, C, dtype=torch.float32, device=dout.device)
        check(lib.nnl_concat_pool_bwd(ptr(_f32c(dout.reshape(N, 2 * C))), ptr(am), ptr(dx), N, H * W, C, stream()))
        return from_nhwc(dx)


def conv_bn_act(conv, bn, x, residual=None, relu=True, conv_slot=None, bn_slot=None, conv_give=None):
    fuse = (bn.training and bn.track_running_stats and bn.running_mean is not None and bn.momentum is not None
            and getattr(bn, 'nnl_sync', None) is None and x.is_cuda and conv.bias is None and not conv.fuse_relu
            and torch.is_grad_enabled() and os.environ.get('NNL_BN_EPI_STATS', '1') != '0')

    def unfused(**kw):
        return bn_act(bn, conv(x, grad_slot=conv_slot, give_slot=conv_give), residual=residual, relu=relu, grad_slot=bn_slot, **kw)
    if not fuse:
        return unfused()
    pivot = getattr(bn, '_nnl_pivot', None)
    if pivot is None or pivot.device != x.device or pivot.numel() != bn.num_features:
        if torch.cuda.is_current_stream_capturing():
            return unfused()
        pivot = torch.empty(bn.num_features, dtype=torch.float32, device=x.device)
        object.__setattr__(bn, '_nnl_pivot', pivot)
        return unfused(pivot_out=pivot)
    y, part = conv2d_with_bn_stats(x, conv.weight, None, conv.stride[0], conv.padding[0], pivot, conv_slot, conv_give)
    return bn_act(bn, y, residual=residual, relu=relu, grad_slot=bn_slot, ext_stats=(part, pivot), pivot_out=pivot)


def linear_relu_bn(lin, bn, x):
    fuse = (bn.training and bn.track_running_stats and bn.running_mean is not None and bn.momentum is not None
            and getattr(bn, 'nnl_sync', None) is None and x.is_cuda and x.dim() == 2 and torch.is_grad_enabled()
            and os.environ.get('NNL_BN_EPI_STATS', '1') != '0')
    pivot = getattr(bn, '_nnl_pivot', None) if fuse else None
    if not fuse or pivot is None or pivot.device != x.device or pivot.numel() != bn.num_features:
        y = linear(x, lin.weight, lin.bias, relu=True)
        if not fuse or torch.cuda.is_current_stream_capturing():
            return bn_act(bn, y, relu=False)
        pivot = torch.empty(bn.num_features, dtype=torch.float32, device=x.device)
        object.__setattr__(bn, '_nnl_pivot', pivot)
        return bn_act(bn, y, relu=False, pivot_out=pivot)
    y, part = _conv(x[:, :, None, None], lin.weight[:, :, None, None], lin.bias, relu=1, bn_pivot=pivot)
    return bn_act(bn, y.reshape(x.shape[0], lin.weight.shape[0]), relu=False, ext_stats=(part, pivot), pivot_out=pivot)


def concat_pool2d(x):
    return _ConcatPool.apply(x)


def pool_out_size(H, ksize, stride, pad, ceil_mode=False):
    if not ceil_mode:
        return (H + 2 * pad - ksize) // stride + 1
    out = -((H + 2 * pad - ksize) // -stride) + 1
    return out - 1 if (out - 1) * stride >= H + pad else out


class _MaxPool2d(torch.autograd.Function):
    @staticmethod
    def forward(ctx, x, ksize, stride, pad, ceil_mode=False):
        require_cuda(x)
        xn = to_nhwc(x.float())
        N, H, W, C = xn.shape
        P, Q = pool_out_size(H, ksize, stride, pad, ceil_mode), pool_out_size(W, ksize, stride, pad, ceil_mode)
        y = torch.empty(N, P, Q, C, dtype=torch.float32, device=x.device)
        idx = torch.empty(N, P, Q, C, dtype=torch.uint8, device=x.device)
        check(lib.nnl_maxpool2d_fwd(ptr(xn), ptr(y), ptr(idx), N, H, W, C, P, Q, ksize, stride, pad, stream()))
        ctx.save_for_backward(idx)
        ctx.cfg = (N, H, W, C, P, Q, ksize, stride, pad)
        return from_nhwc(y)

    @staticmethod
    def backward(ctx, dy):
        (idx,) = ctx.saved_tensors
        N, H, W, C, P, Q, ksize, stride, pad = ctx.cfg
        dyn = to_nhwc(dy.float())
        dx = torch.empty(N, H, W, C, dtype=torch.float32, device=dy.device)
        check(lib.nnl_maxpool2d_bwd(ptr(dyn), ptr(idx), ptr(dx), N, H, W, C, P, Q, ksize, stride, pad, stream()))
        return from_nhwc(dx), None, None, None, None


class _BNReLUMaxPool(torch.autograd.Function):

    @staticmethod
    def forward(ctx, x, gamma, beta, running_mean, running_var, training, momentum, eps, nbt, ksize, stride, pad):
        require_cuda(x, gamma, beta)
        xn = to_nhwc(x.float())
        N, H, W, C = xn.shape
        P, Q = (H + 2 * pad - ksize) // stride + 1, (W + 2 * pad - ksize) // stride + 1
        dev = x.device
        y = torch.empty(N, P, Q, C, dtype=torch.float32, device=dev)
        idx = torch.empty(N, P, Q, C, dtype=torch.uint8, device=dev)
        stats = torch.empty(4, C, dtype=torch.float32, device=dev)
        wsb = int(lib.nnl_bn_workspace_bytes(N * H * W, C))
        ws = _workspace(wsb, dev)
        check(lib.nnl_bn_relu_maxpool_fwd(ptr(xn), ptr(gamma), ptr(beta), ptr(y), ptr(idx), ptr(stats[0]), ptr(stats[1]),
                                          ptr(stats[2]), ptr(stats[3]), ptr(running_mean), ptr(running_var), N, H, W, C, P, Q,
                                          ksize, stride, pad, float(eps), float(momentum), int(training), ptr(nbt), ptr(ws), wsb,
                                          stream()))
        ctx.save_for_backward(xn, idx, gamma, beta, stats, y)
        ctx.cfg = (N, H, W, C, P, Q, ksize, stride, pad, training)
        return from_nhwc(y)

    @staticmethod
    def backward(ctx, dy):
        xn, idx, gamma, beta, stats, y = ctx.saved_tensors
        N, H, W, C, P, Q, ksize, stride, pad, training = ctx.cfg
        dyn = to_nhwc(dy.float())
        dx = torch.empty_like(xn)
        dgamma = torch.empty(C, dtype=torch.float32, device=xn.device) if gamma is not None else None
        dbeta = torch.empty(C, dtype=torch.float32, device=xn.device) if gamma is not None else None
        wsb = int(lib.nnl_bn_workspace_bytes(N * H * W, C))
        ws = _workspace(wsb, xn.device)
        check(lib.nnl_bn_relu_maxpool_bwd(ptr(dyn), ptr(y), ptr(idx), ptr(xn), ptr(gamma), ptr(beta), ptr(stats[0]), ptr(stats[1]),
                                          ptr(stats[2]), ptr(stats[3]), ptr(dx), ptr(dgamma), ptr(dbeta), N, H, W, C, P, Q, ksize, stride, pad,
                                          int(training), ptr(ws), wsb, stream()))
        return (from_nhwc(dx), dgamma, dbeta) + (None,) * 9


def conv_bn_relu_maxpool(conv, bn, pool, x):
    k, s, p = pool.kernel_size, pool.stride, pool.padding
    fuse = (x.is_cuda and isinstance(pool, torch.nn.MaxPool2d) and all(isinstance(v, int) for v in (k, s, p))
            and pool.dilation == 1 and not pool.ceil_mode and not pool.return_indices and 2 * p <= k and k * k <= 255
            and not (bn.training and getattr(bn, 'nnl_sync', None) is not None)
            and (bn.running_mean is not None or bn.training)
            and not (bn.training and bn.track_running_stats and bn.momentum is None)
            and bool(lib.nnl_bn_relu_maxpool_supported(bn.num_features)))
    if not fuse:
        return pool(conv_bn_act(conv, bn, x, relu=True))
    y = conv(x)
    training, momentum, nbt, rmean, rvar = _bn_mode(bn)
    return _BNReLUMaxPool.apply(y, bn.weight, bn.bias, rmean, rvar, training, momentum, bn.eps, nbt, k, s, p)


def maxpool2d(x, ksize=3, stride=2, pad=1, ceil_mode=False):
    return _MaxPool2d.apply(x, int(ksize), int(stride), int(pad), bool(ceil_mode))


def _gconv_check(x_shape, w_shape, stride, pad, groups):
    if len(x_shape) != 4 or len(w_shape) != 4:
        raise NotImplementedError('grouped_conv2d: x %s and weight %s must be 4-D' % (tuple(x_shape), tuple(w_shape)))
    C, (K, Cg, R, S) = x_shape[1], w_shape
    if R != S or R not in (1, 3):
        raise NotImplementedError('grouped_conv2d: kernel_size %dx%d is not supported (1x1 or 3x3)' % (R, S))
    if stride not in (1, 2):
        raise NotImplementedError('grouped_conv2d: stride %r is not supported (1 or 2)' % (stride,))
    if pad not in (0, 1) or pad > R // 2:
        raise NotImplementedError('grouped_conv2d: padding %r is not supported (0 .. kernel_size // 2)' % (pad,))
    if groups < 1 or C % groups or K % groups or C // groups != Cg:
        raise NotImplementedError('grouped_conv2d: groups %r must divide the %d input and %d output channels (weight holds %d inputs per group)'
                                  % (groups, C, K, Cg))


class _GroupedConv2d(torch.autograd.Function):

    @staticmethod
    def forward(ctx, x, weight, bias, stride, pad, groups, relu):
        _gconv_check(x.shape, weight.shape, stride, pad, groups)
        require_cuda(x, weight, bias)
        xn, wn = to_nhwc(x.float()), to_nhwc(weight.float())
        b = None if bias is None else _f32c(bias)
        N, H, W, C = xn.shape
        K, R = wn.shape[0], wn.shape[1]
        g = _geom(N, H, W, C, K, R, R, stride, pad)
        y = torch.empty((N, g.P, g.Q, K), dtype=torch.float32, device=x.device)
        check(lib.nnl_gconv2d_fwd(ptr(xn), ptr(wn), ptr(b), ptr(y), N, H, W, C, K, groups, R, stride, pad, int(relu), stream()))
        ctx.cfg = (g, groups, bool(relu), bias is not None)
        ctx.save_for_backward(xn, wn, y if relu else None)
        return from_nhwc(y)

    @staticmethod
    def backward(ctx, dy):
        xn, wn, y = ctx.saved_tensors
        g, groups, relu, has_bias = ctx.cfg
        dims = (g.N, g.H, g.W, g.C, g.K, groups, g.R, g.stride, g.pad)
        want_db = has_bias and ctx.needs_input_grad[2]
        dyn, db = to_nhwc(dy.float()), None
        if relu:
            dyn, db = _conv_act_gate(y, dyn, g, 1, want_db)
        dx = dw = None
        if ctx.needs_input_grad[0]:
            dx = torch.empty_like(xn)
            check(lib.nnl_gconv2d_dgrad(ptr(dyn), ptr(wn), ptr(dx), *dims, stream()))
            dx = from_nhwc(dx)
        if ctx.needs_input_grad[1]:
            dw = torch.empty_like(wn)
            wsb = int(lib.nnl_gconv2d_workspace_bytes(*dims))
            ws = _workspace(wsb, dyn.device)
            check(lib.nnl_gconv2d_wgrad(ptr(xn), ptr(dyn), ptr(dw), ptr(ws), wsb, *dims, stream()))
            dw = from_nhwc(dw)
        if db is None and want_db:
            db = _conv_bias_grad(dyn, g, g.K)
        return dx, dw, db, None, None, None, None


def grouped_conv2d(x, weight, bias, stride, pad, groups, relu=False):
    return _GroupedConv2d.apply(x, weight, bias, int(stride), int(pad), int(groups), bool(relu))


class _SEExcite(torch.autograd.Function):

    @staticmethod
    def forward(ctx, x, residual, w1, b1, w2, b2):
        require_cuda(x, residual, w1, b1, w2, b2)
        xn = to_nhwc(x.float())
        rn = None if residual is None else to_nhwc(residual.float())
        N, H, W, C = xn.shape
        if rn is not None and rn.shape != xn.shape:
            raise _lib.NnlError('se_excite: residual %s does not match x %s' % (tuple(residual.shape), tuple(x.shape)))
        m = torch.empty(N, C, dtype=torch.float32, device=x.device)
        check(lib.nnl_se_squeeze(ptr(xn), ptr(m), N, H * W, C, stream()))
        track = any(ctx.needs_input_grad)
        with torch.enable_grad() if track else contextlib.nullcontext():
            if track:
                m.requires_grad_(True)
            z = linear(linear(m, w1.reshape(w1.shape[0], C), b1, relu=True), w2.reshape(C, w2.shape[1]), b2)
        zd = _f32c(z.detach())
        out = torch.empty_like(xn)
        check(lib.nnl_se_excite_fwd(ptr(xn), ptr(zd), ptr(rn), ptr(out), N, H * W, C, stream()))
        ctx.fc = (m, z, (w1, b1, w2, b2)) if track else None
        ctx.has_res = rn is not None
        ctx.save_for_backward(xn, zd, out)
        return from_nhwc(out)

    @staticmethod
    def backward(ctx, dy):
        xn, zd, out = ctx.saved_tensors
        N, H, W, C = xn.shape
        dyn = to_nhwc(dy.float())
        dx, dz = torch.empty_like(xn), torch.empty_like(zd)
        dres = torch.empty_like(xn) if (ctx.has_res and ctx.needs_input_grad[1]) else None
        check(lib.nnl_se_excite_bwd(ptr(dyn), ptr(out), ptr(xn), ptr(zd), ptr(dx), ptr(dres), ptr(dz), N, H * W, C, stream()))
        m, z, params = ctx.fc
        ctx.fc = None
        live = [p is not None and p.requires_grad for p in params]
        grads = iter(torch.autograd.grad(z, [m] + [p for p, on in zip(params, live) if on], dz, allow_unused=True))
        dm = next(grads)
        if ctx.needs_input_grad[0]:
            check(lib.nnl_se_squeeze_bwd(ptr(_f32c(dm)), ptr(dx), N, H * W, C, stream()))
        dparams = tuple(next(grads) if on else None for on in live)
        return ((from_nhwc(dx) if ctx.needs_input_grad[0] else None), (None if dres is None else from_nhwc(dres))) + dparams


def se_excite(x, fc1, fc2, residual=None):
    return _SEExcite.apply(x, residual, fc1.weight, fc1.bias, fc2.weight, fc2.bias)


def fold_zero_pad(H, R, stride, pad, z):
    return pad + z - stride, (H + z + 2 * pad - R) // stride


def _window_args(H, W, R, stride, pad, pad_lo, out_size):
    if pad_lo is None:
        pad_lo = pad
    if out_size is None:
        P, Q = (H + 2 * pad - R) // stride + 1, (W + 2 * pad - R) // stride + 1
    else:
        P, Q = (out_size, out_size) if isinstance(out_size, int) else out_size
    return int(pad_lo), int(P), int(Q)


def _window_check(who, x_shape, R, rmax_text, r_ok, stride, stride_ok, pad, pad_lo, out_size):
    if len(x_shape) != 4:
        raise NotImplementedError('%s: x %s must be 4-D' % (who, tuple(x_shape)))
    if not r_ok:
        raise NotImplementedError('%s: kernel_size %r is not supported (%s)' % (who, R, rmax_text))
    if not stride_ok:
        raise NotImplementedError('%s: stride %r is not supported' % (who, stride))
    if not isinstance(pad, int) or pad < 0 or pad > R // 2:
        raise NotImplementedError('%s: padding %r is not supported (0 .. kernel_size // 2)' % (who, pad))
    H, W = x_shape[2], x_shape[3]
    lo, P, Q = _window_args(H, W, R, stride, pad, pad_lo, out_size)
    if lo < 0 or lo > R - 1:
        raise NotImplementedError('%s: pad_lo %r is not supported (0 .. kernel_size - 1)' % (who, lo))
    if P < 1 or Q < 1 or (P - 1) * stride - lo > H - 1 or (Q - 1) * stride - lo > W - 1:
        raise NotImplementedError('%s: out_size %r is not supported: every window must touch the %d x %d input' % (who, (P, Q), H, W))
    return lo, P, Q


def _dwconv_check(x_shape, w_shape, stride, pad, pad_lo, out_size):
    if len(w_shape) != 4:
        raise NotImplementedError('depthwise_conv2d: weight %s must be 4-D' % (tuple(w_shape),))
    K, Cg, R, S = w_shape
    if len(x_shape) == 4 and (K != x_shape[1] or Cg != 1):
        raise NotImplementedError('depthwise_conv2d: weight %s is not depthwise for %d input channels (groups == in_channels == '
# ... 897 lines not shown
```

Baseline: 5535 images/s.

## Add run-based stem conv kernels for small-channel inputs with fused BN stats

Adds dedicated forward and weight-gradient kernels for the ResNet stem conv when input channels are fewer than four. They treat each filter row of contiguous (S*C) input as one unpadded run, avoiding the pad-to-4-channels path and the wasted MACs that padding brings. The forward kernel emits BatchNorm partial statistics in its epilogue, and the fused BN-ReLU-maxpool then finalises from those partials instead of re-reading the activation. The cost is new kernel code, extra per-element buffer loads with bounds masks, and a first-call path that allocates the pivot buffer.

Result: no change. 5587 images/s, median of 6 (+0.9%).

```diff
diff --git a/include/nnl.h b/include/nnl.h
--- a/include/nnl.h
+++ b/include/nnl.h
@@ -93,6 +93,13 @@
 size_t nnl_conv2d_wgrad_workspace_bytes(const nnl_conv_geom_t* g);
 int nnl_conv2d_wgrad(const float* x, const float* dy, float* dw, const nnl_conv_geom_t* g, void* workspace,
                      size_t workspace_bytes, void* stream);
+int nnl_conv2d_runs_ok(const nnl_conv_geom_t* g);
+size_t nnl_conv2d_runs_workspace_bytes(const nnl_conv_geom_t* g, int wgrad);
+int nnl_conv2d_runs_fwd(const float* x, const float* w, const float* bias, float* y, const nnl_conv_geom_t* g, int relu,
+                        void* workspace, size_t workspace_bytes, float* bn_partials, const float* bn_pivot, int32_t* bn_rows,
+                        void* stream);
+int nnl_conv2d_runs_wgrad(const float* x, const float* dy, float* dw, const nnl_conv_geom_t* g, void* workspace,
+                          size_t workspace_bytes, void* stream);
 size_t nnl_colsum_workspace_bytes(int64_t rows, int64_t cols);
 int nnl_sum_tensors(const float* const* src, int n, float* out, int64_t numel, void* stream);
 int nnl_colsum(const float* a, float* out, int64_t rows, int64_t cols, void* workspace, size_t workspace_bytes,
@@ -118,6 +125,11 @@
                             int64_t N, int64_t H, int64_t W, int64_t C, int64_t P, int64_t Q, int ks, int stride, int pad, float eps,
                             float momentum, int training, int64_t* num_batches_tracked, void* workspace, size_t workspace_bytes,
                             void* stream);
+int nnl_bn_relu_maxpool_fwd_pre(const float* x, const float* gamma, const float* beta, float* y, uint8_t* idx, float* save_mean,
+                                float* save_invstd, float* save_scale, float* save_shift, float* running_mean, float* running_var,
+                                int64_t N, int64_t H, int64_t W, int64_t C, int64_t P, int64_t Q, int ks, int stride, int pad, float eps,
+                                float momentum, int training, int64_t* num_batches_tracked, void* workspace, size_t workspace_bytes,
+                                const float* bn_partials, const float* bn_pivot, int64_t bn_rows, float* pivot_out, void* stream);
 int nnl_bn_relu_maxpool_bwd(const float* dpool, const float* y, const uint8_t* idx, const float* x, const float* gamma,
                             const float* beta, const float* mean, const float* invstd, const float* scale, const float* shift,
                             float* dx, float* dgamma, float* dbeta,
diff --git a/neuralnetworklibrary_amd/_lib.py b/neuralnetworklibrary_amd/_lib.py
--- a/neuralnetworklibrary_amd/_lib.py
+++ b/neuralnetworklibrary_amd/_lib.py
@@ -59,6 +59,10 @@
     'nnl_conv2d_dgrad': (C.c_int, [c_p, c_p, c_p, C.POINTER(ConvGeom), c_p, c_p, sz, c_p, c_p]),
     'nnl_conv2d_wgrad_workspace_bytes': (sz, [C.POINTER(ConvGeom)]),
     'nnl_conv2d_wgrad': (C.c_int, [c_p, c_p, c_p, C.POINTER(ConvGeom), c_p, sz, c_p]),
+    'nnl_conv2d_runs_ok': (C.c_int, [C.POINTER(ConvGeom)]),
+    'nnl_conv2d_runs_workspace_bytes': (sz, [C.POINTER(ConvGeom), C.c_int]),
+    'nnl_conv2d_runs_fwd': (C.c_int, [c_p, c_p, c_p, c_p, C.POINTER(ConvGeom), C.c_int, c_p, sz, c_p, c_p, C.POINTER(i32), c_p]),
+    'nnl_conv2d_runs_wgrad': (C.c_int, [c_p, c_p, c_p, C.POINTER(ConvGeom), c_p, sz, c_p]),
     'nnl_colsum_workspace_bytes': (sz, [i64, i64]),
     'nnl_colsum': (C.c_int, [c_p, c_p, i64, i64, c_p, sz, c_p]),
     'nnl_relu_gate_colsum': (C.c_int, [c_p, c_p, c_p, c_p, i64, i64, c_p, sz, c_p]),
@@ -71,6 +75,8 @@
     'nnl_bn_relu_maxpool_supported': (C.c_int, [i64]),
     'nnl_bn_relu_maxpool_fwd': (C.c_int, [c_p, c_p, c_p, c_p, c_p, c_p, c_p, c_p, c_p, c_p, c_p, i64, i64, i64, i64, i64, i64,
                                           C.c_int, C.c_int, C.c_int, f32, f32, C.c_int, c_p, c_p, sz, c_p]),
+    'nnl_bn_relu_maxpool_fwd_pre': (C.c_int, [c_p, c_p, c_p, c_p, c_p, c_p, c_p, c_p, c_p, c_p, c_p, i64, i64, i64, i64, i64, i64,
+                                              C.c_int, C.c_int, C.c_int, f32, f32, C.c_int, c_p, c_p, sz, c_p, c_p, i64, c_p, c_p]),
     'nnl_bn_relu_maxpool_bwd': (C.c_int, [c_p, c_p, c_p, c_p, c_p, c_p, c_p, c_p, c_p, c_p, c_p, c_p, c_p, i64, i64, i64, i64, i64, i64,
                                           C.c_int, C.c_int, C.c_int, C.c_int, c_p, sz, c_p]),
     'nnl_concat_pool_fwd': (C.c_int, [c_p, c_p, c_p, i64, i64, i64, c_p]),
diff --git a/neuralnetworklibrary_amd/csrc/batchnorm.hip b/neuralnetworklibrary_amd/csrc/batchnorm.hip
--- a/neuralnetworklibrary_amd/csrc/batchnorm.hip
+++ b/neuralnetworklibrary_amd/csrc/batchnorm.hip
@@ -837,6 +837,18 @@
                                        float* running_mean, float* running_var, int64_t N, int64_t H, int64_t W, int64_t C,
                                        int64_t P, int64_t Q, int ks, int stride, int pad, float eps, float momentum, int training,
                                        int64_t* num_batches_tracked, void* workspace, size_t workspace_bytes, void* stream) {
+  return nnl_bn_relu_maxpool_fwd_pre(x, gamma, beta, y, idx, save_mean, save_invstd, save_scale, save_shift, running_mean, running_var, N, H, W,
+                                     C, P, Q, ks, stride, pad, eps, momentum, training, num_batches_tracked, workspace, workspace_bytes,
+                                     nullptr, nullptr, 0, nullptr, stream);
+}
+
+extern "C" int nnl_bn_relu_maxpool_fwd_pre(const float* x, const float* gamma, const float* beta, float* y, uint8_t* idx,
+                                           float* save_mean, float* save_invstd, float* save_scale, float* save_shift,
+                                           float* running_mean, float* running_var, int64_t N, int64_t H, int64_t W, int64_t C,
+                                           int64_t P, int64_t Q, int ks, int stride, int pad, float eps, float momentum, int training,
+                                           int64_t* num_batches_tracked, void* workspace, size_t workspace_bytes,
+                                           const float* bn_partials, const float* bn_pivot, int64_t bn_rows, float* pivot_out,
+                                           void* stream) {
   NNL_TRY(check_stem_geometry("bn_relu_maxpool_fwd", N, H, W, C, P, Q, ks, stride, pad));
   NNL_CHECK_ARG(x && y && idx && save_mean && save_invstd && save_scale && save_shift, "bn_relu_maxpool_fwd: null pointer");
   NNL_CHECK_ARG(training || (running_mean && running_var), "bn_relu_maxpool_fwd: eval mode needs running statistics");
@@ -846,8 +858,11 @@
   hipStream_t s = (hipStream_t)stream;
   NnlProfScope prof(NNL_PROF_ELEMENTWISE, s, (double)rows * C * (training ? 8.0 : 4.0) + (double)N * P * Q * C * 5.0);
   const ChannelStats cs{gamma, beta, save_mean, save_invstd, running_mean, running_var, save_scale, save_shift,  nullptr,
-                         nullptr, num_batches_tracked, eps, momentum};
-  NNL_TRY(launch_channel_affine(x, ws.part, cs, rows, C, training, s));
+                        training ? pivot_out : nullptr, num_batches_tracked, eps, momentum};
+  if (training && bn_partials != nullptr && bn_pivot != nullptr && bn_rows > 0)
+    NNL_TRY(launch_finalize(bn_pivot, bn_partials, (int)bn_rows, true, cs, rows, C, s));
+  else
+    NNL_TRY(launch_channel_affine(x, ws.part, cs, rows, C, training, s));
   const long total = (long)N * P * Q * CG;
   hipLaunchKernelGGL(bnpool_fwd_kernel, dim3((unsigned)nnl_cdiv(total, kBlock)), dim3(kBlock), 0, s, x, save_scale, save_shift, y, idx,
                      (int)N, (int)H, (int)W, (int)CG, (int)P, (int)Q, ks, stride, pad);
diff --git a/neuralnetworklibrary_amd/csrc/conv2d.hip b/neuralnetworklibrary_amd/csrc/conv2d.hip
--- a/neuralnetworklibrary_amd/csrc/conv2d.hip
+++ b/neuralnetworklibrary_amd/csrc/conv2d.hip
@@ -629,9 +629,7 @@
   }
   if (pl.splits > 1) {
     const long n4 = (long)p.Mc * p.Nc / 4;
-    NNL_ROUTE("splitk_reduce");
-    hipLaunchKernelGGL(splitk_reduce_kernel, dim3((unsigned)nnl_cdiv(n4, 32)), dim3(256), 0, s, (const float*)ws, dw, n4, pl.splits);
-    NNL_CHECK_LAUNCH();
+    return nnl_internal_splitk_reduce(ws, dw, n4, pl.splits, s);
   }
   return NNL_OK;
 }
@@ -667,6 +665,13 @@
   return q;
 }
 
+}
+
+int nnl_internal_splitk_reduce(const float* slabs, float* out, long n4, int splits, hipStream_t s) {
+  NNL_ROUTE("splitk_reduce");
+  hipLaunchKernelGGL(splitk_reduce_kernel, dim3((unsigned)nnl_cdiv(n4, 32)), dim3(256), 0, s, slabs, out, n4, splits);
+  NNL_CHECK_LAUNCH();
+  return NNL_OK;
 }
 
 int nnl_internal_gemm_nt(const float* a, const float* b, float* y, const float* bias, const float* add, int M, int N,
diff --git a/neuralnetworklibrary_amd/csrc/conv_runs.hip b/neuralnetworklibrary_amd/csrc/conv_runs.hip
--- /dev/null
+++ b/neuralnetworklibrary_amd/csrc/conv_runs.hip
@@ -0,0 +1,386 @@
+#include "igemm.h"
+#include "split_tile.h"
+
+namespace {
+
+constexpr unsigned kRunsOob = 0x80000000u;
+
+struct RunsParams {
+  const float* a;
+  const float* b;
+  float* y;
+  const float* bias; const float* add;
+  float* bn_part; const float* bn_pivot;
+  unsigned a_bytes, b_bytes;
+  int H, W, C, P, Q, R, stride, pad;
+  int RUN;
+  int M, Nc;
+  int relu, grid_m, grid_n;
+  int splits, k_per_split;
+};
+
+__device__ __forceinline__ float buf_load1(__amdgpu_buffer_rsrc_t rsrc, unsigned voff, unsigned soff) {
+  return __uint_as_float(__builtin_amdgcn_raw_buffer_load_b32(rsrc, (int)voff, (int)soff, 0));
+}
+
+__global__ __launch_bounds__(256) void conv_runs_repack_kernel(const float* __restrict__ w, float* __restrict__ wp, int rows, int RUN, int RUNP) {
+  const int i = blockIdx.x * 256 + threadIdx.x;
+  if (i >= rows * RUNP) return;
+  const int row = i / RUNP, f = i - row * RUNP;
+  wp[i] = f < RUN ? w[row * RUN + f] : 0.f;
+}
+
+template <int RUNP>
+__global__ __launch_bounds__(256) void conv_runs_fwd_kernel(const RunsParams p) {
+  static_assert(RUNP % 8 == 0 && RUNP >= 8 && RUNP <= 64, "run length");
+  constexpr int BKP = RUNP + 4, NE = RUNP / 4, BUF = 128 * BKP;
+  constexpr int LDS_FLOATS = 2 * BUF > 64 * 68 ? 2 * BUF : 64 * 68;
+  __shared__ __attribute__((aligned(16))) float lds[LDS_FLOATS];
+
+  const int tid = threadIdx.x, lane = tid & 63, wave = tid >> 6;
+  const int wm = wave >> 1, wn = wave & 1;
+  const int logical = nnl_xcd_remap(blockIdx.x, gridDim.x);
+  const int tile_m = logical / p.grid_n, tile_n = logical - tile_m * p.grid_n;
+  const int m0 = tile_m * 64, n0 = tile_n * 64;
+  const int srow = tid >> 2, j = tid & 3;
+
+  const __amdgpu_buffer_rsrc_t ra_src = __builtin_amdgcn_make_buffer_rsrc(const_cast<float*>(p.a), 0, (int)p.a_bytes, 0x00020000);
+  const __amdgpu_buffer_rsrc_t rb_src = __builtin_amdgcn_make_buffer_rsrc(const_cast<float*>(p.b), 0, (int)p.b_bytes, 0x00020000);
+
+  int a_base, hchk;
+  unsigned colmask = 0;
+  {
+    const int m = m0 + srow;
+    const bool valid = m < p.M;
+    const int mm = valid ? m : 0;
+    const int PQ = p.P * p.Q;
+    const int n = mm / PQ;
+    const int rem = mm - n * PQ;
+    const int pp = rem / p.Q;
+    const int qq = rem - pp * p.Q;
+    const int h0 = pp * p.stride - p.pad, w0 = qq * p.stride - p.pad;
+    a_base = (((n * p.H + h0) * p.W + w0) * p.C + j) * 4;
+    hchk = valid ? h0 : -(1 << 28);
+#pragma unroll
+    for (int i = 0; i < NE; ++i) {
+      const int f = j + 4 * i;
+      if (f < p.RUN && (unsigned)(w0 + f / p.C) < (unsigned)p.W) colmask |= 1u << i;
+    }
+  }
+  const int nr = n0 + srow;
+  const unsigned b_off = nr < p.Nc ? (unsigned)((nr * p.R * RUNP + j) * 4) : kRunsOob;
+  const int rowb = p.W * p.C * 4;
+
+  float ra[NE], rb[NE];
+  auto load_tile = [&](int r) {
+    const bool rowok = (unsigned)(hchk + r) < (unsigned)p.H;
+    const unsigned arow = (unsigned)(a_base + r * rowb);
+    const unsigned bsoff = (unsigned)(r * RUNP * 4);
+#pragma unroll
+    for (int i = 0; i < NE; ++i) ra[i] = buf_load1(ra_src, (rowok && ((colmask >> i) & 1u)) ? arow + 16u * i : kRunsOob, 0);
+#pragma unroll
+    for (int i = 0; i < NE; ++i) rb[i] = buf_load1(rb_src, b_off + 16u * i, bsoff);
+  };
+  auto store_tile = [&](int buf) {
+    float* As = lds + buf * BUF + srow * BKP + j;
+    float* Bs = As + 64 * BKP;
+#pragma unroll
+    for (int i = 0; i < NE; ++i) As[4 * i] = ra[i];
+#pragma unroll
+    for (int i = 0; i < NE; ++i) Bs[4 * i] = rb[i];
+  };
+
+  f32x16 acc, acc2;
+#pragma unroll
+  for (int e = 0; e < 16; ++e) { acc[e] = 0.f; acc2[e] = 0.f; }
+  const int frag_off = (lane & 31) * BKP + (lane >> 5) * 4;
+  auto compute = [&](int buf) {
+    const float* As = lds + buf * BUF + wm * 32 * BKP + frag_off;
+    const float* Bs = lds + buf * BUF + 64 * BKP + wn * 32 * BKP + frag_off;
+    f32x4 af[RUNP / 8], bf[RUNP / 8];
+#pragma unroll
+    for (int kk = 0; kk < RUNP / 8; ++kk) {
+      af[kk] = *reinterpret_cast<const f32x4*>(As + kk * 8);
+      bf[kk] = *reinterpret_cast<const f32x4*>(Bs + kk * 8);
+    }
+#pragma unroll
+    for (int kk = 0; kk < RUNP / 8; ++kk) {
+#pragma unroll
+      for (int t = 0; t < 4; ++t) {
+        if (kk & 1) acc2 = __builtin_amdgcn_mfma_f32_32x32x2f32(af[kk][t], bf[kk][t], acc2, 0, 0, 0);
+        else acc = __builtin_amdgcn_mfma_f32_32x32x2f32(af[kk][t], bf[kk][t], acc, 0, 0, 0);
+      }
+    }
+  };
+
+  load_tile(0);
+  store_tile(0);
+  __syncthreads();
+  int cur = 0;
+  for (int r = 0; r < p.R; ++r) {
+    load_tile(r + 1 < p.R ? r + 1 : r);
+    __builtin_amdgcn_sched_barrier(0);
+    compute(cur);
+    __builtin_amdgcn_sched_barrier(0);
+    store_tile(cur ^ 1);
+    __syncthreads();
+    cur ^= 1;
+  }
+
+#pragma unroll
+  for (int e = 0; e < 16; ++e) acc[e] += acc2[e];
+  tile64_finish_rows<false>(p, acc, lds, tid, wm, wn, tile_m, m0, n0);
+}
+
+template <int RUNP>
+__global__ __launch_bounds__(256, 4) void conv_runs_wgrad_kernel(const RunsParams p) {
+  constexpr int BK = 16, BM = 64, BN = 192, BNS = 208, NE = BN / 16, BUF = BK * (BM + BNS);
+  __shared__ __attribute__((aligned(16))) float lds[2 * BUF];
+
+  const int tid = threadIdx.x, lane = tid & 63, wave = tid >> 6;
+  const int wm = wave >> 1, wn = wave & 1;
+  const int tiles = p.grid_m * p.grid_n;
+  const int split = blockIdx.x / tiles;
+  const int t_id = blockIdx.x - split * tiles;
+  const int tile_n = t_id / p.grid_m, tile_m = t_id - tile_n * p.grid_m;
+  const int m0 = tile_m * BM, n0 = tile_n * BN;
+  const int ncol = p.R * RUNP;
+
+  const int k_begin = split * p.k_per_split;
+  const int k_end = min(k_begin + p.k_per_split, p.M);
+
+  const __amdgpu_buffer_rsrc_t ra_src = __builtin_amdgcn_make_buffer_rsrc(const_cast<float*>(p.a), 0, (int)p.a_bytes, 0x00020000);
+  const __amdgpu_buffer_rsrc_t rb_src = __builtin_amdgcn_make_buffer_rsrc(const_cast<float*>(p.b), 0, (int)p.b_bytes, 0x00020000);
+
+  const int pix = tid >> 4, j = tid & 15;
+  int k = k_begin + pix;
+  const bool a_cok = m0 + j * 4 < p.Nc;
+  unsigned a_off = ((unsigned)k * (unsigned)p.Nc + (unsigned)(m0 + j * 4)) * 4u;
+  const unsigned a_step = (unsigned)(BK * p.Nc * 4);
+  int e_off[NE], e_r[NE], e_c[NE];
+#pragma unroll
+  for (int i = 0; i < NE; ++i) {
+    const int col = n0 + j + 16 * i;
+    const int r = col / RUNP, f = col - r * RUNP;
+    const bool ok = col < ncol && f < p.RUN;
+    e_r[i] = ok ? r : (1 << 28);
+    e_c[i] = ok ? f / p.C : 0;
+    e_off[i] = ok ? (r * p.W * p.C + f) * 4 : 0;
+  }
+  int n, pp, qq;
+  {
+    const int PQ = p.P * p.Q;
+    const int kk = k < p.M ? k : 0;
+    n = kk / PQ;
+    const int rem = kk - n * PQ;
+    pp = rem / p.Q;
+    qq = rem - pp * p.Q;
+  }
+
+  f32x4 ra;
+  float rb[NE];
+  auto load_tile = [&]() {
+    const bool kv = k < k_end;
+    const int h0 = pp * p.stride - p.pad, w0 = qq * p.stride - p.pad;
+    const int hc = kv ? h0 : -(1 << 29);
+    const unsigned base = ((unsigned)(n * p.H + h0) * (unsigned)p.W + (unsigned)w0) * (unsigned)p.C * 4u;
+    ra = buf_load4_policy<0>(ra_src, (kv && a_cok) ? a_off : kRunsOob);
+#pragma unroll
+    for (int i = 0; i < NE; ++i) {
+      const bool ok = (unsigned)(hc + e_r[i]) < (unsigned)p.H && (unsigned)(w0 + e_c[i]) < (unsigned)p.W;
+      rb[i] = buf_load1(rb_src, ok ? base + (unsigned)e_off[i] : kRunsOob, 0);
+    }
+    k += BK;
+    a_off += a_step;
+    qq += BK;
+    while (qq >= p.Q) {
+      qq -= p.Q;
+      if (++pp == p.P) { pp = 0; ++n; }
+    }
+  };
+  auto store_tile = [&](int buf) {
+    float* As = lds + buf * BUF;
+    float* Bs = As + BK * BM + pix * BNS + j;
+    *reinterpret_cast<f32x4*>(As + pix * BM + j * 4) = ra;
+#pragma unroll
+    for (int i = 0; i < NE; ++i) Bs[16 * i] = rb[i];
+  };
+
+  f32x16 acc[3];
+#pragma unroll
+  for (int c = 0; c < 3; ++c)
+#pragma unroll
+    for (int e = 0; e < 16; ++e) acc[c][e] = 0.f;
+
+  const int l31 = lane & 31, lh = lane >> 5;
+  auto compute = [&](int buf) {
+    const float* As = lds + buf * BUF + lh * BM + wm * 32 + l31;
+    const float* Bs = lds + buf * BUF + BK * BM + lh * BNS + wn * 96 + l31;
+#pragma unroll
+    for (int kk = 0; kk < BK / 2; ++kk) {
+      const float af = As[kk * 2 * BM];
+      float bf[3];
+#pragma unroll
+      for (int c = 0; c < 3; ++c) bf[c] = Bs[kk * 2 * BNS + c * 32];
+#pragma unroll
+      for (int c = 0; c < 3; ++c) acc[c] = __builtin_amdgcn_mfma_f32_32x32x2f32(af, bf[c], acc[c], 0, 0, 0);
+    }
+  };
+
+  const int nk = (k_end - k_begin + BK - 1) / BK;
+  if (nk > 0) {
+    load_tile();
+    store_tile(0);
+    __syncthreads();
+    int cur = 0;
+    for (int kt = 0; kt < nk; ++kt) {
+      const bool more = kt + 1 < nk;
+      if (more) load_tile();
+      compute(cur);
+      if (more) store_tile(cur ^ 1);
+      __syncthreads();
+      cur ^= 1;
+    }
+  }
+
+  const int nout = p.R * p.RUN;
+  float* out = p.y + (long)split * p.Nc * nout;
+#pragma unroll
+  for (int c = 0; c < 3; ++c) {
+    const int col = n0 + wn * 96 + c * 32 + l31;
+    const int r = col / RUNP, f = col - r * RUNP;
+    const bool cok = col < ncol && f < p.RUN;
+#pragma unroll
+    for (int e = 0; e < 16; ++e) {
+      const int row = m0 + wm * 32 + (e & 3) + 8 * (e >> 2) + lh * 4;
+      if (cok && row < p.Nc) out[(long)row * nout + r * p.RUN + f] = acc[c][e];
+    }
+  }
+}
+
+int runs_pad(int run) { return (run + 7) / 8 * 8; }
+
+bool runs_check(const nnl_conv_geom_t* g) {
+  if (!g || g->N <= 0 || g->H <= 0 || g->W <= 0 || g->C <= 0 || g->K <= 0 || g->R <= 0 || g->S <= 0 || g->stride <= 0 || g->pad < 0) return false;
+  if (g->C >= 4 || g->S * g->C > 64 || g->K % 4 != 0 || g->R > 4096 || g->pad > 4096 || g->stride > 4096) return false;
+  if (g->H + 2L * g->pad < g->R || g->W + 2L * g->pad < g->S) return false;
+  const long P = (g->H + 2L * g->pad - g->R) / g->stride + 1, Q = (g->W + 2L * g->pad - g->S) / g->stride + 1;
+  if (P != g->P || Q != g->Q || P <= 0 || Q <= 0) return false;
+  const long lim = (1L << 31) - (1L << 20);
+  if (((long)g->N * g->H + 2L * g->pad + g->R) * (g->W + 2L * g->pad + g->S) * g->C * 4 >= lim) return false;
+  if ((long)g->N * P * Q * g->K * 4 >= lim || (long)g->N * P * Q >= (1L << 30) - 4096) return false;
+  if ((long)g->K * g->R * runs_pad(g->S * g->C) * 4 >= lim) return false;
+  return true;
+}
+
+RunsParams runs_params(const nnl_conv_geom_t* g) {
+  RunsParams p{};
+  p.H = g->H; p.W = g->W; p.C = g->C; p.P = g->P; p.Q = g->Q; p.R = g->R; p.stride = g->stride; p.pad = g->pad;
+  p.RUN = g->S * g->C;
+  p.M = g->N * g->P * g->Q; p.Nc = g->K;
+  p.splits = 1;
+  return p;
+}
+
+struct RunsWgradPlan { int grid_m, grid_n, splits, k_per_split; };
+RunsWgradPlan runs_wgrad_plan(const nnl_conv_geom_t* g) {
+  RunsWgradPlan pl{};
+  const long Kp = (long)g->N * g->P * g->Q;
+  pl.grid_m = (int)nnl_cdiv(g->K, 64);
+  pl.grid_n = (int)nnl_cdiv((long)g->R * runs_pad(g->S * g->C), 192);
+  long sp = 1024 / ((long)pl.grid_m * pl.grid_n);
+  if (sp > Kp / 256) sp = Kp / 256;
+  if (sp < 1) sp = 1;
+  pl.k_per_split = (int)(nnl_cdiv(nnl_cdiv(Kp, sp), 16) * 16);
+  pl.splits = (int)nnl_cdiv(Kp, pl.k_per_split);
+  return pl;
+}
+
+template <int RUNP>
+int launch_runs_fwd(const RunsParams& p, hipStream_t s) {
+  NNL_ROUTE("runs_fwd<%d>", RUNP);
+  hipLaunchKernelGGL(conv_runs_fwd_kernel<RUNP>, dim3(p.grid_m * p.grid_n), dim3(256), 0, s, p);
+  NNL_CHECK_LAUNCH();
+  return NNL_OK;
+}
+
+template <int RUNP>
+int launch_runs_wgrad(const RunsParams& p, hipStream_t s) {
+  NNL_ROUTE("runs_wgrad<%d>%s@splits=%d", RUNP, p.splits > 1 ? ":splitk" : "", p.splits);
+  hipLaunchKernelGGL(conv_runs_wgrad_kernel<RUNP>, dim3(p.grid_m * p.grid_n * p.splits), dim3(256), 0, s, p);
+  NNL_CHECK_LAUNCH();
+  return NNL_OK;
+}
+
+#define NNL_RUNS_DISPATCH(launch, runp, p, s)          \
+  switch (runp) {                                      \
+    case 8: return launch<8>(p, s);                    \
+    case 16: return launch<16>(p, s);                  \
+    case 24: return launch<24>(p, s);                  \
+    case 32: return launch<32>(p, s);                  \
+    case 40: return launch<40>(p, s);                  \
+    case 48: return launch<48>(p, s);                  \
+    case 56: return launch<56>(p, s);                  \
+    default: return launch<64>(p, s);                  \
+  }
+int dispatch_runs_fwd(const RunsParams& p, hipStream_t s) { NNL_RUNS_DISPATCH(launch_runs_fwd, runs_pad(p.RUN), p, s) }
+int dispatch_runs_wgrad(const RunsParams& p, hipStream_t s) { NNL_RUNS_DISPATCH(launch_runs_wgrad, runs_pad(p.RUN), p, s) }
+
+}
+
+extern "C" int nnl_conv2d_runs_ok(const nnl_conv_geom_t* g) { return runs_check(g) ? 1 : 0; }
+
+extern "C" size_t nnl_conv2d_runs_workspace_bytes(const nnl_conv_geom_t* g, int wgrad) {
+  if (!runs_check(g)) return 0;
+  if (!wgrad) return (size_t)g->K * g->R * runs_pad(g->S * g->C) * sizeof(float);
+  const RunsWgradPlan pl = runs_wgrad_plan(g);
+  return pl.splits > 1 ? (size_t)pl.splits * g->K * g->R * g->S * g->C * sizeof(float) : 0;
+}
+
+extern "C" int nnl_conv2d_runs_fwd(const float* x, const float* w, const float* bias, float* y, const nnl_conv_geom_t* g, int relu,
+                                   void* workspace, size_t workspace_bytes, float* bn_partials, const float* bn_pivot, int32_t* bn_rows,
+                                   void* stream) {
+  if (bn_rows) *bn_rows = 0;
+  if (!runs_check(g)) return nnl_set_error(NNL_ERR_UNSUPPORTED, "conv2d_runs_fwd: geometry outside nnl_conv2d_runs_ok");
+  NNL_CHECK_ARG(x && w && y, "conv2d_runs_fwd: null pointer");
+  NNL_CHECK_ARG(relu == 0 || relu == 1, "conv2d_runs_fwd: relu must be 0 or 1");
+  const size_t need = nnl_conv2d_runs_workspace_bytes(g, 0);
+  if (workspace == nullptr || workspace_bytes < need)
+    return nnl_set_error(NNL_ERR_WORKSPACE, "conv2d_runs_fwd: workspace %zu B < required %zu B", workspace_bytes, need);
+  hipStream_t s = (hipStream_t)stream;
+  RunsParams p = runs_params(g);
+  const int runp = runs_pad(p.RUN);
+  NnlProfScope prof(NNL_PROF_CONV_FWD, s, 2.0 * p.M * (double)p.Nc * g->R * p.RUN);
+  float* wp = (float*)workspace;
+  NNL_ROUTE("runs_repack");
+  hipLaunchKernelGGL(conv_runs_repack_kernel, dim3((unsigned)nnl_cdiv((long)g->K * g->R * runp, 256)), dim3(256), 0, s, w, wp, g->K * g->R,
+                     p.RUN, runp);
+  NNL_CHECK_LAUNCH();
+  p.a = x; p.b = wp; p.y = y; p.bias = bias; p.add = nullptr; p.relu = relu;
+  p.a_bytes = (unsigned)((long)g->N * g->H * g->W * g->C * 4); p.b_bytes = (unsigned)need;
+  p.grid_m = (int)nnl_cdiv(p.M, 64); p.grid_n = (int)nnl_cdiv(p.Nc, 64);
+  const bool stats = bn_partials && bn_pivot && bn_rows;
+  p.bn_part = stats ? bn_partials : nullptr; p.bn_pivot = bn_pivot;
+  const int st = dispatch_runs_fwd(p, s);
+  if (st == NNL_OK && stats) *bn_rows = p.grid_m;
+  return st;
+}
+
+extern "C" int nnl_conv2d_runs_wgrad(const float* x, const float* dy, float* dw, const nnl_conv_geom_t* g, void* workspace,
+                                     size_t workspace_bytes, void* stream) {
+  if (!runs_check(g)) return nnl_set_error(NNL_ERR_UNSUPPORTED, "conv2d_runs_wgrad: geometry outside nnl_conv2d_runs_ok");
+  NNL_CHECK_ARG(x && dy && dw, "conv2d_runs_wgrad: null pointer");
+  const size_t need = nnl_conv2d_runs_workspace_bytes(g, 1);
+  if (need > 0 && (workspace == nullptr || workspace_bytes < need))
+    return nnl_set_error(NNL_ERR_WORKSPACE, "conv2d_runs_wgrad: workspace %zu B < required %zu B", workspace_bytes, need);
+  hipStream_t s = (hipStream_t)stream;
+  const RunsWgradPlan pl = runs_wgrad_plan(g);
+  RunsParams p = runs_params(g);
+  NnlProfScope prof(NNL_PROF_CONV_WGRAD, s, 2.0 * p.M * (double)p.Nc * g->R * p.RUN);
+  p.a = dy; p.b = x; p.y = pl.splits > 1 ? (float*)workspace : dw;
+  p.a_bytes = (unsigned)((long)p.M * p.Nc * 4); p.b_bytes = (unsigned)((long)g->N * g->H * g->W * g->C * 4);
+  p.grid_m = pl.grid_m; p.grid_n = pl.grid_n; p.splits = pl.splits; p.k_per_split = pl.k_per_split;
+  const int st = dispatch_runs_wgrad(p, s);
+  if (st != NNL_OK || pl.splits == 1) return st;
+  return nnl_internal_splitk_reduce((const float*)workspace, dw, (long)g->K * g->R * p.RUN / 4, pl.splits, s);
+}
diff --git a/neuralnetworklibrary_amd/csrc/igemm.h b/neuralnetworklibrary_amd/csrc/igemm.h
--- a/neuralnetworklibrary_amd/csrc/igemm.h
+++ b/neuralnetworklibrary_amd/csrc/igemm.h
@@ -38,6 +38,8 @@
 int nnl_internal_gemm_tn(const float* a, const float* b, float* y, int Mc, int Nc, long Kp, void* ws, size_t ws_bytes,
                          hipStream_t s);
 
+int nnl_internal_splitk_reduce(const float* slabs, float* out, long n4, int splits, hipStream_t s);
+
 __device__ __forceinline__ int nnl_xcd_remap(int bid, int nblk) {
   const int q = nblk >> 3, r = nblk & 7;
   const int xcd = bid & 7, idx = bid >> 3;
diff --git a/neuralnetworklibrary_amd/csrc/igemm_taps.h b/neuralnetworklibrary_amd/csrc/igemm_taps.h
--- a/neuralnetworklibrary_amd/csrc/igemm_taps.h
+++ b/neuralnetworklibrary_amd/csrc/igemm_taps.h
@@ -421,22 +421,7 @@
   }
   if constexpr (EPI == 0 && BM == 64 && BN == 64) {
     if (dense_out && !p.add_up2 && !partial && p.Nc % 4 == 0) {
-      constexpr int LDT = 68;
-      float* tl = &lds[0][0];
-#pragma unroll
-      for (int e = 0; e < 16; ++e) tl[(wm * 32 + (e & 3) + 8 * (e >> 2) + row_h) * LDT + wn * 32 + col_l] = acc[0][0][e];
-      __syncthreads();
-      float fs1[4] = {0.f, 0.f, 0.f, 0.f}, fs2[4] = {0.f, 0.f, 0.f, 0.f};
-#pragma unroll
-      for (int k4 = 0; k4 < 4; ++k4) {
-        const int idx4 = tid + k4 * 256, rl = idx4 >> 4, c4 = n0 + (idx4 & 15) * 4;
-        const int row = m0 + rl;
-        if (row >= p.M || c4 >= p.Nc) continue;
-        f32x4 v = *reinterpret_cast<const f32x4*>(tl + rl * LDT + (idx4 & 15) * 4);
-        const long o = (long)row * p.Nc + c4;
-        finish_piece<true>(p, v, c4, o, fs1, fs2);
-      }
-      bn_partials_write(p, fs1, fs2, &lds[0][0], tid, tile_m, n0);
+      tile64_finish_rows<true>(p, acc[0][0], &lds[0][0], tid, wm, wn, tile_m, m0, n0);
       return;
     }
   }
diff --git a/neuralnetworklibrary_amd/csrc/split_tile.h b/neuralnetworklibrary_amd/csrc/split_tile.h
--- a/neuralnetworklibrary_amd/csrc/split_tile.h
+++ b/neuralnetworklibrary_amd/csrc/split_tile.h
@@ -106,3 +106,24 @@
     p.bn_part[((long)tile_m * p.Nc + n0 + tid) * 2 + 1] = b;
   }
 }
+
+template <bool SIG, class Params>
+__device__ __forceinline__ void tile64_finish_rows(const Params& p, const f32x16& acc, float* tl, int tid, int wm, int wn, int tile_m, int m0,
+                                                   int n0) {
+  constexpr int LDT = 68;
+  const int lane = tid & 63, col_l = lane & 31, row_h = (lane >> 5) * 4;
+#pragma unroll
+  for (int e = 0; e < 16; ++e) tl[(wm * 32 + (e & 3) + 8 * (e >> 2) + row_h) * LDT + wn * 32 + col_l] = acc[e];
+  __syncthreads();
+  float fs1[4] = {0.f, 0.f, 0.f, 0.f}, fs2[4] = {0.f, 0.f, 0.f, 0.f};
+#pragma unroll
+  for (int k4 = 0; k4 < 4; ++k4) {
+    const int idx4 = tid + k4 * 256, rl = idx4 >> 4, c4 = n0 + (idx4 & 15) * 4;
+    const int row = m0 + rl;
+    if (row >= p.M || c4 >= p.Nc) continue;
+    f32x4 v = *reinterpret_cast<const f32x4*>(tl + rl * LDT + (idx4 & 15) * 4);
+    const long o = (long)row * p.Nc + c4;
+    finish_piece<SIG>(p, v, c4, o, fs1, fs2);
+  }
+  bn_partials_write(p, fs1, fs2, tl, tid, tile_m, n0);
+}
diff --git a/neuralnetworklibrary_amd/ops.py b/neuralnetworklibrary_amd/ops.py
--- a/neuralnetworklibrary_amd/ops.py
+++ b/neuralnetworklibrary_amd/ops.py
@@ -490,9 +490,19 @@
 _ConvState = collections.namedtuple('_ConvState', 'g relu has_bias c_in w_layout slot give_slot grad_dst uses')
 
 
-def _conv_operands(x, weight, bias, stride, pad):
-    xn = _pad_c4(to_nhwc(_f32c(x) if x.dim() != 4 else x.float()))
-    wn = _pad_c4(to_nhwc(weight.float()))
+def _runs_ok(x, weight, stride, pad):
+    if x.dim() != 4 or weight.dim() != 4 or x.shape[1] >= 4 or x.shape[1] != weight.shape[1]:
+        return False
+    (N, C, H, W), (K, _, R, S) = x.shape, weight.shape
+    if H + 2 * pad < R or W + 2 * pad < S:
+        return False
+    return bool(lib.nnl_conv2d_runs_ok(_geom(N, H, W, C, K, R, S, stride, pad)))
+
+
+def _conv_operands(x, weight, bias, stride, pad, runs=False):
+    xn, wn = to_nhwc(_f32c(x) if x.dim() != 4 else x.float()), to_nhwc(weight.float())
+    if not runs:
+        xn, wn = _pad_c4(xn), _pad_c4(wn)
     N, H, W, C = xn.shape
     K, R, S, _ = wn.shape
     g = _geom(N, H, W, C, K, R, S, stride, pad)
@@ -603,9 +613,14 @@
         dwn = dst.permute(0, 2, 3, 1)
     else:
         dwn = torch.empty((g4.K, g4.R, g4.S, g4.C), dtype=torch.float32, device=dy4.device)
-    wsb = int(lib.nnl_conv2d_wgrad_workspace_bytes(g4))
-    ws = _workspace(wsb, dy4.device, floor=True)
-    check(lib.nnl_conv2d_wgrad(ptr(xn), ptr(dy4), ptr(dwn), g4, ptr(ws), wsb, stream()))
+    if g4.C < 4:
+        wsb = int(lib.nnl_conv2d_runs_workspace_bytes(g4, 1))
+        ws = _workspace(wsb, dy4.device, floor=True)
+        check(lib.nnl_conv2d_runs_wgrad(ptr(xn), ptr(dy4), ptr(dwn), g4, ptr(ws), wsb, stream()))
+    else:
+        wsb = int(lib.nnl_conv2d_wgrad_workspace_bytes(g4))
+        ws = _workspace(wsb, dy4.device, floor=True)
+        check(lib.nnl_conv2d_wgrad(ptr(xn), ptr(dy4), ptr(dwn), g4, ptr(ws), wsb, stream()))
     dw = from_nhwc(dwn[:K, :, :, :st.c_in])
     wshape, wstride = st.w_layout
     if (g4.R == 1 and g4.S == 1 and wshape == tuple(dw.shape) and wstride != tuple(dw.stride()) and dw.is_contiguous(memory_format=torch.channels_last)
@@ -628,17 +643,24 @@
     @staticmethod
     def forward(ctx, x, weight, bias, stride, pad, relu, slot=None, bn_pivot=None, give_slot=None):
         require_cuda(x, weight, bias)
-        xn, wn, b, g, y = _conv_operands(x, weight, bias, stride, pad)
+        runs = relu in (0, 1) and not ctx.needs_input_grad[0] and slot is None and give_slot is None and _runs_ok(x, weight, stride, pad)
+        xn, wn, b, g, y = _conv_operands(x, weight, bias, stride, pad, runs)
         N, K = g.N, g.K
         ctx.st = _conv_state(x, weight, bias, g, relu, slot, give_slot)
-        wsb = int(lib.nnl_conv2d_fwd_workspace_bytes(g))
-        ws = _workspace(wsb, x.device)
         part, rows = None, _lib.i32(0)
         if bn_pivot is not None:
             part = torch.empty(((N * g.P * g.Q + 63) // 64) * K * 2, dtype=torch.float32, device=x.device)
-        u = (_OPEN or _CLOSED).wino(wn.data_ptr(), 0, g)
-        check(lib.nnl_conv2d_fwd_pre(ptr(xn), ptr(wn), ptr(b), ptr(y), g, int(relu), ptr(ws), wsb, ptr(_tile_counters(x.device) if wsb else None),
-                                     ptr(part), ptr(bn_pivot), ctypes.byref(rows) if part is not None else None, ptr(u), stream()))
+        if runs:
+            wsb = int(lib.nnl_conv2d_runs_workspace_bytes(g, 0))
+            ws = _workspace(wsb, x.device)
+            check(lib.nnl_conv2d_runs_fwd(ptr(xn), ptr(wn), ptr(b), ptr(y), g, int(relu), ptr(ws), wsb, ptr(part), ptr(bn_pivot),
+                                          ctypes.byref(rows) if part is not None else None, stream()))
+        else:
+            wsb = int(lib.nnl_conv2d_fwd_workspace_bytes(g))
+            ws = _workspace(wsb, x.device)
+            u = (_OPEN or _CLOSED).wino(wn.data_ptr(), 0, g)
+            check(lib.nnl_conv2d_fwd_pre(ptr(xn), ptr(wn), ptr(b), ptr(y), g, int(relu), ptr(ws), wsb, ptr(_tile_counters(x.device) if wsb else None),
+                                         ptr(part), ptr(bn_pivot), ctypes.byref(rows) if part is not None else None, ptr(u), stream()))
         if part is None or rows.value == 0:
             part = torch.empty(0, dtype=torch.float32, device=x.device)
         else:
@@ -997,7 +1019,8 @@
 class _BNReLUMaxPool(torch.autograd.Function):
 
     @staticmethod
-    def forward(ctx, x, gamma, beta, running_mean, running_var, training, momentum, eps, nbt, ksize, stride, pad):
+    def forward(ctx, x, gamma, beta, running_mean, running_var, training, momentum, eps, nbt, ksize, stride, pad, ext_stats=None,
+                pivot_out=None):
         require_cuda(x, gamma, beta)
         xn = to_nhwc(x.float())
         N, H, W, C = xn.shape
@@ -1008,10 +1031,14 @@
         stats = torch.empty(4, C, dtype=torch.float32, device=dev)
         wsb = int(lib.nnl_bn_workspace_bytes(N * H * W, C))
         ws = _workspace(wsb, dev)
-        check(lib.nnl_bn_relu_maxpool_fwd(ptr(xn), ptr(gamma), ptr(beta), ptr(y), ptr(idx), ptr(stats[0]), ptr(stats[1]),
-                                          ptr(stats[2]), ptr(stats[3]), ptr(running_mean), ptr(running_var), N, H, W, C, P, Q,
-                                          ksize, stride, pad, float(eps), float(momentum), int(training), ptr(nbt), ptr(ws), wsb,
-                                          stream()))
+        part, pivot, n_part = None, None, 0
+        if ext_stats is not None and ext_stats[0].numel() > 0:
+            part, pivot = ext_stats
+            n_part = part.numel() // (2 * C)
+        check(lib.nnl_bn_relu_maxpool_fwd_pre(ptr(xn), ptr(gamma), ptr(beta), ptr(y), ptr(idx), ptr(stats[0]), ptr(stats[1]),
+                                              ptr(stats[2]), ptr(stats[3]), ptr(running_mean), ptr(running_var), N, H, W, C, P, Q,
+                                              ksize, stride, pad, float(eps), float(momentum), int(training), ptr(nbt), ptr(ws), wsb,
+                                              ptr(part), ptr(pivot), n_part, ptr(pivot_out), stream()))
         ctx.save_for_backward(xn, idx, gamma, beta, stats, y)
         ctx.cfg = (N, H, W, C, P, Q, ksize, stride, pad, training)
         return from_nhwc(y)
@@ -1029,7 +1056,7 @@
         check(lib.nnl_bn_relu_maxpool_bwd(ptr(dyn), ptr(y), ptr(idx), ptr(xn), ptr(gamma), ptr(beta), ptr(stats[0]), ptr(stats[1]),
                                           ptr(stats[2]), ptr(stats[3]), ptr(dx), ptr(dgamma), ptr(dbeta), N, H, W, C, P, Q, ksize, stride, pad,
                                           int(training), ptr(ws), wsb, stream()))
-        return (from_nhwc(dx), dgamma, dbeta) + (None,) * 9
+        return (from_nhwc(dx), dgamma, dbeta) + (None,) * 11
 
 
 def conv_bn_relu_maxpool(conv, bn, pool, x):
@@ -1042,9 +1069,26 @@
             and bool(lib.nnl_bn_relu_maxpool_supported(bn.num_features)))
     if not fuse:
         return pool(conv_bn_act(conv, bn, x, relu=True))
-    y = conv(x)
     training, momentum, nbt, rmean, rvar = _bn_mode(bn)
-    return _BNReLUMaxPool.apply(y, bn.weight, bn.bias, rmean, rvar, training, momentum, bn.eps, nbt, k, s, p)
+    stats = (getattr(conv, 'nnl_hip_conv', False) and bn.training and bn.track_running_stats and bn.running_mean is not None
+             and conv.bias is None and not getattr(conv, 'fuse_relu', False) and torch.is_grad_enabled()
+             and not x.requires_grad and conv.stride[0] == conv.stride[1] and conv.padding[0] == conv.padding[1]
+             and conv.dilation == (1, 1) and conv.groups == 1 and conv.padding_mode == 'zeros'
+             and os.environ.get('NNL_BN_EPI_STATS', '1') != '0' and _runs_ok(x, conv.weight, conv.stride[0], conv.padding[0]))
+    pivot = getattr(bn, '_nnl_pivot', None) if stats else None
+    if stats and (pivot is None or pivot.device != x.device or pivot.numel() != bn.num_features):
+        if torch.cuda.is_current_stream_capturing():
+            stats = False
+        else:
+            pivot = torch.empty(bn.num_features, dtype=torch.float32, device=x.device)
+            object.__setattr__(bn, '_nnl_pivot', pivot)
+            y = conv(x)
+            return _BNReLUMaxPool.apply(y, bn.weight, bn.bias, rmean, rvar, training, momentum, bn.eps, nbt, k, s, p, None, pivot)
+    if not stats:
+        y = conv(x)
+        return _BNReLUMaxPool.apply(y, bn.weight, bn.bias, rmean, rvar, training, momentum, bn.eps, nbt, k, s, p)
+    y, part = conv2d_with_bn_stats(x, conv.weight, None, conv.stride[0], conv.padding[0], pivot)
+    return _BNReLUMaxPool.apply(y, bn.weight, bn.bias, rmean, rvar, training, momentum, bn.eps, nbt, k, s, p, (part, pivot), pivot)
 
 
 def maxpool2d(x, ksize=3, stride=2, pad=1, ceil_mode=False):
```
